# PRBonn/LiDiff

Hardware: NVIDIA B200
Metric: denoising_steps_per_sec_180k_pts_T50 (higher is better)
Workload: dtype fp16x3 split tensor-core MMA, fp32 accumulate (fp32 CUDA cores for the Cin=3 stem), fp64 DPM update

## Files before the change

### include/lidiff_b200.h

```cpp
#ifndef LIDIFF_B200_H_
#define LIDIFF_B200_H_

#include <stdint.h>
#include <stddef.h>

#ifdef __cplusplus
extern "C" {
#endif

#define LB2_OK            0
#define LB2_ERR_ARG      -1
#define LB2_ERR_CUDA     -2
#define LB2_ERR_UNSUP    -3

#define LB2_KEY_EMPTY 0xFFFFFFFFFFFFFFFFull

int         lb2_create(int device, void** handle);
void        lb2_destroy(void* handle);
const char* lb2_last_error(void* handle);
int         lb2_version(void);
int64_t     lb2_launch_count(void* handle);
#define LB2_OPT_TC_PAIR       0
#define LB2_OPT_TC_N256       1
#define LB2_OPT_TC_SMALL      2
#define LB2_OPT_TC_PERSISTENT 3
#define LB2_OPT_TC_FULL_LAG   4
#define LB2_OPT_TC_NSPLIT     5
#define LB2_OPT_COUNT         6
int         lb2_set_option(void* handle, int option, int value);
int         lb2_get_option(void* handle, int option);
int         lb2_read_status(void* handle, void* stream);

typedef struct {
    uint64_t* keys;
    int32_t*  vals;
    int32_t   cap_table;
} lb2_grid;

int lb2_quantize(void* h, void* stream, const float* x, int64_t n_elem, float resolution, int div_mode,
                 float* out_coord);

size_t lb2_unique_scratch_bytes(int64_t n_cap);
int lb2_unique_build(void* h, void* stream,
                     const float* in_f, const int32_t* in_i, const int32_t* d_nin, int32_t n_cap,
                     int32_t ts_floor, lb2_grid grid,
                     int32_t* out_coords, int32_t* inverse, int32_t* d_nout, void* scratch);

int lb2_voxel_mean(void* h, void* stream, const float* feats, const int32_t* inverse, int32_t n,
                   int32_t c, const int32_t* d_m, int32_t m_cap, float* out, int32_t* counts);

int lb2_kernel_map(void* h, void* stream, lb2_grid grid_in, const int32_t* out_coords,
                   const int32_t* d_nout, int32_t nout_cap, int32_t ks, int32_t step,
                   int32_t* nbr, int64_t nbr_stride, uint64_t* pair_count, uint32_t* row_mask);

int lb2_kernel_map_self(void* h, void* stream, lb2_grid grid, const int32_t* coords, const int32_t* d_n, int32_t n_cap,
                        int32_t step, int32_t* nbr, int64_t nbr_stride, uint64_t* pair_count, uint32_t* row_mask);

size_t lb2_row_order_scratch_bytes(int32_t n_cap);
int lb2_row_order(void* h, void* stream, const uint32_t* row_mask, const int32_t* d_n, int32_t n_cap,
                  int32_t kvol, int32_t* perm, void* scratch, const int32_t* coords, int32_t coord_shift);

int lb2_tile_order(void* h, void* stream, const uint32_t* row_mask, const int32_t* row_perm, const int32_t* d_n, int32_t n_cap,
                   int32_t* order128, int32_t* order256, void* scratch);

typedef struct {
    const float*   in1;
    const float*   in2;
    const float*   residual;
    float*         out;
    const float*   gate_table;
    const int32_t* gate_idx;
    float*         out_gated;
    const float*   pre_add;
    const void*    in1_h;
    const void*    in2_h;
    void*          out_h;
    void*          out_gated_h;
    const void*    residual_h;
} lb2_conv_io;

typedef struct {
    int32_t        c1, c2, cout, kvol;
    const float*   weight;
    const void*    weight_packed;
    const float*   scale;
    const float*   shift;
    int32_t        relu;
    const int32_t* nbr;
    int64_t        nbr_stride;
    const int32_t* d_mout;
    int32_t        mout_cap;
    const int32_t* row_perm;
    const uint32_t* row_mask;
    int32_t        npass;
    lb2_conv_io    io[2];
    const int32_t* tile_order128;
    const int32_t* tile_order256;
} lb2_conv_desc;

#define LB2_ALGO_AUTO  0
#define LB2_ALGO_FFMA  1
#define LB2_ALGO_TC    2
#define LB2_ALGO_TC_TILE 3
int lb2_spconv_forward(void* h, void* stream, const lb2_conv_desc* d, int algo);

typedef struct {
    int32_t        c1, c2, cout, kvol;
    const void*    weight_packed;
    const int32_t* pair_in;
    const int32_t* pair_out;
    const int32_t* koff;
    const int32_t* tile_off;
    int32_t        npass;
    const float*   in1[2];
    const float*   in2[2];
    const void*    in1_h[2];
    const void*    in2_h[2];
    float*         out[2];
    const int32_t* d_zero_rows;
    int32_t        zero_rows_cap;
} lb2_scatter_desc;
size_t lb2_pair_list_scratch_bytes(void);
int lb2_pair_list(void* h, void* stream, const int32_t* nbr, int64_t nbr_stride, const int32_t* d_nout,
                  int32_t nout_cap, int32_t kvol, int32_t skip_k, int32_t* pair_in, int32_t* pair_out,
                  int32_t* koff, int32_t* tile_off, void* scratch);
int lb2_spconv_scatter_supported(int32_t c1, int32_t c2, int32_t cout, int32_t kvol);
int lb2_spconv_scatter(void* h, void* stream, const lb2_scatter_desc* d);

size_t lb2_packed_weight_bytes(int32_t kvol, int32_t cin, int32_t cout);
int lb2_pack_weights(void* h, void* stream, const float* weight, int32_t kvol, int32_t cin, int32_t cout,
                     void* packed);

int lb2_nn_match(void* h, void* stream, const int32_t* q_coords, const int32_t* d_nq, int32_t nq_cap,
                 const int32_t* k_coords, const int32_t* d_nk, int32_t nk_cap, int32_t batch_scale,
                 int32_t* idx);

int lb2_nn_match_grid(void* h, void* stream, const int32_t* q_coords, const int32_t* d_nq, int32_t nq_cap,
                      const int32_t* k_coords, const int32_t* d_nk, int32_t nk_cap, lb2_grid key_grid,
                      int32_t key_stride, int32_t max_ring, int32_t* idx);

size_t lb2_nn_table_bytes(void);
int lb2_nn_table_build(void* h, void* stream, const int32_t* k_coords, const int32_t* d_nk, int32_t nk_cap, void* table);
int lb2_nn_match_table(void* h, void* stream, const int32_t* q_coords, const int32_t* d_nq, int32_t nq_cap,
                       const int32_t* k_coords, const int32_t* d_nk, int32_t nk_cap, const void* table,
                       int32_t key_stride, int32_t max_ring, int32_t* idx);

size_t lb2_nn_tree_bytes(int32_t nk_cap);
int lb2_nn_tree_build(void* h, void* stream, const int32_t* k_coords, const int32_t* d_nk, int32_t nk_cap, void* tree);
int lb2_nn_match_tree(void* h, void* stream, const int32_t* q_coords, const int32_t* d_nq, int32_t nq_cap,
                      const void* tree, int32_t nk_cap, const int32_t* k_coords, const int32_t* hint_of,
                      const int32_t* hint_idx, int32_t* idx);

int lb2_linear(void* h, void* stream, const float* x, int64_t ldx, const float* w, const float* b,
               const float* addend, int64_t ld_addend, int32_t m_cap, const int32_t* d_m,
               int32_t n_in, int32_t n_out, int32_t act, float* y, int64_t ldy,
               const float* prebias, int32_t pre_act);

int lb2_head_mlp(void* h, void* stream, const float* x, int64_t ldx, int64_t x_pass_stride, const float* w0, const float* b0,
                 const float* w1, const float* b1, int32_t m_cap, const int32_t* d_m, int32_t n_in, int32_t n_hid,
                 int32_t n_out, int32_t out_act, int32_t npass, float* y, int64_t ldy, int64_t y_pass_stride);

int lb2_gate_mul(void* h, void* stream, const float* x, const float* table, const int32_t* idx,
                 const int32_t* d_m, int32_t m_cap, int32_t c, float* out, void* out_h);

int lb2_gather_rows(void* h, void* stream, const float* src, const int32_t* idx, int32_t n, int32_t c,
                    float* out);

typedef struct {
    double c_sample, c_x0, c_noise, sigma_s, alpha_s, inv_r0;
    float  guidance_w, resolution;
    int32_t second_order, div_mode, f64_state;
} lb2_dpm_coef;
int lb2_guidance_dpm_step(void* h, void* stream, const float* eps_c, const float* eps_u,
                          const int32_t* inverse, const float* x_t, const double* x_init,
                          const float* noise, double* x0_state, int64_t n_points, lb2_dpm_coef coef,
                          float* eps_out, float* x_next, float* coord_next ,
                          const float* batch_col );

int lb2_farthest_point_sample(void* h, void* stream, const double* pts, int32_t n, int32_t n_samples,
                              int32_t* out_idx, double* dist_scratch);


size_t lb2_cloud_nn_scratch_bytes(int64_t nq, int64_t nr);
int lb2_cloud_nn_distance(void* h, void* stream, const double* query, int64_t nq, const double* ref, int64_t nr,
                          void* scratch, double* dist);

typedef struct {
    int64_t n_a, n_b;
    int64_t occ_a, occ_b, occ_ab;
    double  jsd_3d, jsd_bev;
} lb2_voxel_hist_result;
size_t lb2_voxel_hist_scratch_bytes(int64_t na, int64_t nb);
int lb2_voxel_hist_compare(void* h, void* stream, const double* a, int64_t na, const double* b, int64_t nb,
                           const double* edges, int32_t bins, void* scratch, lb2_voxel_hist_result* out);

int lb2_threshold_counts(void* h, void* stream, const double* d, int64_t n, const double* thr, int32_t nthr, int64_t* counts);

#ifdef __cplusplus
}
#endif
#endif
```

### lidiff_b200/_lib.py

```python
from __future__ import annotations

import ctypes as C
import os
import threading

import torch

_SO = os.path.join(os.path.dirname(os.path.abspath(__file__)), "_C", "liblidiff_b200.so")

ALGO_AUTO, ALGO_FFMA, ALGO_TC, ALGO_TC_TILE = 0, 1, 2, 3
OPT_TC_PAIR, OPT_TC_N256, OPT_TC_SMALL, OPT_TC_PERSISTENT, OPT_TC_FULL_LAG, OPT_TC_NSPLIT = range(6)


class Grid(C.Structure):
    _fields_ = [("keys", C.c_void_p), ("vals", C.c_void_p), ("cap_table", C.c_int32)]


class ConvIO(C.Structure):
    _fields_ = [("in1", C.c_void_p), ("in2", C.c_void_p), ("residual", C.c_void_p), ("out", C.c_void_p),
                ("gate_table", C.c_void_p), ("gate_idx", C.c_void_p), ("out_gated", C.c_void_p), ("pre_add", C.c_void_p),
                ("in1_h", C.c_void_p), ("in2_h", C.c_void_p), ("out_h", C.c_void_p), ("out_gated_h", C.c_void_p),
                ("residual_h", C.c_void_p)]


class ConvDesc(C.Structure):
    _fields_ = [("c1", C.c_int32), ("c2", C.c_int32), ("cout", C.c_int32), ("kvol", C.c_int32),
                ("weight", C.c_void_p), ("weight_packed", C.c_void_p),
                ("scale", C.c_void_p), ("shift", C.c_void_p), ("relu", C.c_int32),
                ("nbr", C.c_void_p), ("nbr_stride", C.c_int64),
                ("d_mout", C.c_void_p), ("mout_cap", C.c_int32), ("row_perm", C.c_void_p), ("row_mask", C.c_void_p),
                ("npass", C.c_int32),
                ("io", ConvIO * 2),
                ("tile_order128", C.c_void_p), ("tile_order256", C.c_void_p)]


class ScatterDesc(C.Structure):
    _fields_ = [("c1", C.c_int32), ("c2", C.c_int32), ("cout", C.c_int32), ("kvol", C.c_int32),
                ("weight_packed", C.c_void_p), ("pair_in", C.c_void_p), ("pair_out", C.c_void_p),
                ("koff", C.c_void_p), ("tile_off", C.c_void_p), ("npass", C.c_int32),
                ("in1", C.c_void_p * 2), ("in2", C.c_void_p * 2), ("in1_h", C.c_void_p * 2), ("in2_h", C.c_void_p * 2),
                ("out", C.c_void_p * 2),
                ("d_zero_rows", C.c_void_p), ("zero_rows_cap", C.c_int32)]


class VoxelHistResult(C.Structure):
    _fields_ = [("n_a", C.c_int64), ("n_b", C.c_int64), ("occ_a", C.c_int64), ("occ_b", C.c_int64), ("occ_ab", C.c_int64),
                ("jsd_3d", C.c_double), ("jsd_bev", C.c_double)]


class DpmCoef(C.Structure):
    _fields_ = [("c_sample", C.c_double), ("c_x0", C.c_double), ("c_noise", C.c_double),
                ("sigma_s", C.c_double), ("alpha_s", C.c_double), ("inv_r0", C.c_double),
                ("guidance_w", C.c_float), ("resolution", C.c_float),
                ("second_order", C.c_int32), ("div_mode", C.c_int32), ("f64_state", C.c_int32)]


EXPORTS = [
    "lb2_create", "lb2_destroy", "lb2_last_error", "lb2_version", "lb2_launch_count", "lb2_read_status",
    "lb2_set_option", "lb2_get_option", "lb2_tile_order",
    "lb2_quantize", "lb2_unique_scratch_bytes", "lb2_unique_build", "lb2_voxel_mean", "lb2_kernel_map",
    "lb2_spconv_forward", "lb2_packed_weight_bytes", "lb2_pack_weights", "lb2_nn_match", "lb2_linear",
    "lb2_gate_mul", "lb2_gather_rows", "lb2_head_mlp", "lb2_kernel_map_self", "lb2_guidance_dpm_step", "lb2_farthest_point_sample",
    "lb2_row_order", "lb2_row_order_scratch_bytes", "lb2_nn_match_grid",
    "lb2_nn_table_bytes", "lb2_nn_table_build", "lb2_nn_match_table",
    "lb2_nn_tree_bytes", "lb2_nn_tree_build", "lb2_nn_match_tree",
    "lb2_pair_list", "lb2_pair_list_scratch_bytes", "lb2_spconv_scatter", "lb2_spconv_scatter_supported",
    "lb2_cloud_nn_scratch_bytes", "lb2_cloud_nn_distance", "lb2_voxel_hist_scratch_bytes", "lb2_voxel_hist_compare",
    "lb2_threshold_counts",
]


def _ptr(t):
    if t is None:
        return None
    if isinstance(t, int):
        return t
    return t.data_ptr()


class Lib:

    def __init__(self, path: str = _SO):
        if not os.path.exists(path):
            raise RuntimeError(f"lidiff_b200: CUDA library not built ({path}); run `python -c 'import __graft_entry__ as g; g.build()'` "
                               "or lidiff_b200/csrc/build.sh — there is no CPU fallback")
        self.path = path
        self.dll = C.CDLL(path)
        d = self.dll
        d.lb2_create.argtypes = [C.c_int, C.POINTER(C.c_void_p)]
        d.lb2_destroy.argtypes = [C.c_void_p]
        d.lb2_destroy.restype = None
        d.lb2_last_error.argtypes = [C.c_void_p]
        d.lb2_last_error.restype = C.c_char_p
        d.lb2_launch_count.argtypes = [C.c_void_p]
        d.lb2_launch_count.restype = C.c_int64
        d.lb2_read_status.argtypes = [C.c_void_p, C.c_void_p]
        d.lb2_set_option.argtypes = [C.c_void_p, C.c_int, C.c_int]
        d.lb2_get_option.argtypes = [C.c_void_p, C.c_int]
        d.lb2_unique_scratch_bytes.argtypes = [C.c_int64]
        d.lb2_unique_scratch_bytes.restype = C.c_size_t
        d.lb2_packed_weight_bytes.argtypes = [C.c_int32] * 3
        d.lb2_packed_weight_bytes.restype = C.c_size_t
        vp, i32, i64, f32 = C.c_void_p, C.c_int32, C.c_int64, C.c_float
        d.lb2_quantize.argtypes = [vp, vp, vp, i64, f32, C.c_int, vp]
        d.lb2_unique_build.argtypes = [vp, vp, vp, vp, vp, i32, i32, Grid, vp, vp, vp, vp]
        d.lb2_voxel_mean.argtypes = [vp, vp, vp, vp, i32, i32, vp, i32, vp, vp]
        d.lb2_kernel_map.argtypes = [vp, vp, Grid, vp, vp, i32, i32, i32, vp, i64, vp, vp]
        d.lb2_kernel_map_self.argtypes = [vp, vp, Grid, vp, vp, i32, i32, vp, i64, vp, vp]
        d.lb2_row_order.argtypes = [vp, vp, vp, vp, i32, i32, vp, vp, vp, i32]
        d.lb2_tile_order.argtypes = [vp, vp, vp, vp, vp, i32, vp, vp, vp]
        d.lb2_row_order_scratch_bytes.restype = C.c_size_t
        d.lb2_row_order_scratch_bytes.argtypes = [i32]
        d.lb2_spconv_forward.argtypes = [vp, vp, C.POINTER(ConvDesc), C.c_int]
        d.lb2_pack_weights.argtypes = [vp, vp, vp, i32, i32, i32, vp]
        d.lb2_nn_match.argtypes = [vp, vp, vp, vp, i32, vp, vp, i32, i32, vp]
        d.lb2_pair_list.argtypes = [vp, vp, vp, i64, vp, i32, i32, i32, vp, vp, vp, vp, vp]
        d.lb2_pair_list_scratch_bytes.restype = C.c_size_t
        d.lb2_spconv_scatter.argtypes = [vp, vp, C.POINTER(ScatterDesc)]
        d.lb2_spconv_scatter_supported.argtypes = [i32, i32, i32, i32]
        d.lb2_nn_table_bytes.restype = C.c_size_t
        d.lb2_nn_tree_bytes.restype = C.c_size_t
        d.lb2_nn_tree_bytes.argtypes = [i32]
        d.lb2_nn_tree_build.argtypes = [vp, vp, vp, vp, i32, vp]
        d.lb2_nn_match_tree.argtypes = [vp, vp, vp, vp, i32, vp, i32, vp, vp, vp, vp]
        d.lb2_nn_table_build.argtypes = [vp, vp, vp, vp, i32, vp]
        d.lb2_nn_match_table.argtypes = [vp, vp, vp, vp, i32, vp, vp, i32, vp, i32, i32, vp]
        d.lb2_nn_match_grid.argtypes = [vp, vp, vp, vp, i32, vp, vp, i32, Grid, i32, i32, vp]
        d.lb2_linear.argtypes = [vp, vp, vp, i64, vp, vp, vp, i64, i32, vp, i32, i32, i32, vp, i64,
                                 vp, i32]
        d.lb2_gate_mul.argtypes = [vp, vp, vp, vp, vp, vp, i32, i32, vp, vp]
        d.lb2_gather_rows.argtypes = [vp, vp, vp, vp, i32, i32, vp]
        d.lb2_head_mlp.argtypes = [vp, vp, vp, i64, i64, vp, vp, vp, vp, i32, vp, i32, i32, i32, i32, i32, vp, i64, i64]
        d.lb2_guidance_dpm_step.argtypes = [vp, vp, vp, vp, vp, vp, vp, vp, vp, i64, DpmCoef, vp, vp, vp, vp]
        d.lb2_farthest_point_sample.argtypes = [vp, vp, vp, i32, i32, vp, vp]
        d.lb2_cloud_nn_scratch_bytes.argtypes = [i64, i64]
        d.lb2_cloud_nn_scratch_bytes.restype = C.c_size_t
        d.lb2_cloud_nn_distance.argtypes = [vp, vp, vp, i64, vp, i64, vp, vp]
        d.lb2_voxel_hist_scratch_bytes.argtypes = [i64, i64]
        d.lb2_voxel_hist_scratch_bytes.restype = C.c_size_t
        d.lb2_voxel_hist_compare.argtypes = [vp, vp, vp, i64, vp, i64, vp, i32, vp, vp]
        d.lb2_threshold_counts.argtypes = [vp, vp, vp, i64, vp, i32, vp]
        self._handles = {}
        self._lock = threading.Lock()

    def missing_symbols(self):
        return [s for s in EXPORTS if not hasattr(self.dll, s)]

    def handle(self, device) -> "Handle":
        dev = torch.device(device)
        if dev.type != "cuda":
            raise RuntimeError("lidiff_b200 runs on CUDA (B200, sm_100a) only; no CPU fallback")
        idx = dev.index if dev.index is not None else torch.cuda.current_device()
        with self._lock:
            if idx not in self._handles:
                hp = C.c_void_p()
                rc = self.dll.lb2_create(idx, C.byref(hp))
                if rc != 0:
                    raise RuntimeError(f"lb2_create(device={idx}) failed with {rc} (needs an sm_100 GPU)")
                self._handles[idx] = Handle(self, hp, idx)
            return self._handles[idx]


class Handle:
    def __init__(self, lib: Lib, hp, device_index: int):
        self.lib, self.dll, self.hp, self.device_index = lib, lib.dll, hp, device_index
        self.device = torch.device("cuda", device_index)

    def _stream(self):
        return torch.cuda.current_stream(self.device).cuda_stream

    def _check(self, rc, what):
        if rc != 0:
            msg = self.dll.lb2_last_error(self.hp)
            raise RuntimeError(f"{what} failed ({rc}): {msg.decode() if msg else ''}")

    def launch_count(self) -> int:
        return int(self.dll.lb2_launch_count(self.hp))

    def read_status(self) -> int:
        return int(self.dll.lb2_read_status(self.hp, self._stream()))

    def set_option(self, option: int, value: int):
        self._check(self.dll.lb2_set_option(self.hp, int(option), int(value)), "set_option")

    def get_option(self, option: int) -> int:
        return int(self.dll.lb2_get_option(self.hp, int(option)))

    def new_grid(self, n_cap: int):
        cap = 1 << max(4, (2 * n_cap - 1).bit_length())
        keys = torch.empty(cap, dtype=torch.int64, device=self.device)
        vals = torch.empty(2 * cap, dtype=torch.int32, device=self.device)
        return (keys, vals, cap)

    @staticmethod
    def _grid(g):
        return Grid(g[0].data_ptr(), g[1].data_ptr(), g[2])

    def unique_scratch(self, n_cap: int) -> torch.Tensor:
        nbytes = int(self.dll.lb2_unique_scratch_bytes(n_cap))
        return torch.empty(nbytes, dtype=torch.uint8, device=self.device)

    def quantize(self, x, resolution, div_mode, out):
        self._check(self.dll.lb2_quantize(self.hp, self._stream(), _ptr(x), x.numel(), float(resolution), int(div_mode), _ptr(out)), "lb2_quantize")

    def unique_build(self, in_f, in_i, d_nin, n_cap, ts_floor, grid, out_coords, inverse, d_nout, scratch):
        self._check(self.dll.lb2_unique_build(self.hp, self._stream(), _ptr(in_f), _ptr(in_i), _ptr(d_nin), int(n_cap), int(ts_floor),
                                              self._grid(grid), _ptr(out_coords), _ptr(inverse), _ptr(d_nout), _ptr(scratch)), "lb2_unique_build")

    def voxel_mean(self, feats, inverse, n, c, d_m, m_cap, out, counts):
        self._check(self.dll.lb2_voxel_mean(self.hp, self._stream(), _ptr(feats), _ptr(inverse), int(n), int(c), _ptr(d_m), int(m_cap),
                                            _ptr(out), _ptr(counts)), "lb2_voxel_mean")

    def kernel_map(self, grid_in, out_coords, d_nout, nout_cap, ks, step, nbr, nbr_stride, pair_count=None, row_mask=None):
        self._check(self.dll.lb2_kernel_map(self.hp, self._stream(), self._grid(grid_in), _ptr(out_coords), _ptr(d_nout), int(nout_cap),
                                            int(ks), int(step), _ptr(nbr), int(nbr_stride), _ptr(pair_count), _ptr(row_mask)), "lb2_kernel_map")

    def kernel_map_self(self, grid, coords, d_n, n_cap, step, nbr, nbr_stride, pair_count=None, row_mask=None):
        self._check(self.dll.lb2_kernel_map_self(self.hp, self._stream(), self._grid(grid), _ptr(coords), _ptr(d_n), int(n_cap), int(step),
                                                 _ptr(nbr), int(nbr_stride), _ptr(pair_count), _ptr(row_mask)), "lb2_kernel_map_self")

    def row_order_scratch_bytes(self, n_cap) -> int:
        return int(self.dll.lb2_row_order_scratch_bytes(int(n_cap)))

    def row_order(self, row_mask, d_n, n_cap, kvol, perm, scratch, coords=None, coord_shift=0):
        self._check(self.dll.lb2_row_order(self.hp, self._stream(), _ptr(row_mask), _ptr(d_n), int(n_cap), int(kvol), _ptr(perm), _ptr(scratch),
                                           _ptr(coords), int(coord_shift)), "lb2_row_order")

    def tile_order(self, row_mask, row_perm, d_n, n_cap, order128, order256, scratch):
        self._check(self.dll.lb2_tile_order(self.hp, self._stream(), _ptr(row_mask), _ptr(row_perm), _ptr(d_n), int(n_cap), _ptr(order128),
                                            _ptr(order256), _ptr(scratch)), "lb2_tile_order")

    def spconv(self, desc: ConvDesc, algo: int = ALGO_AUTO):
        self._check(self.dll.lb2_spconv_forward(self.hp, self._stream(), C.byref(desc), int(algo)), "lb2_spconv_forward")

    def pair_list(self, nbr, nbr_stride, d_nout, nout_cap, kvol, skip_k, pair_in, pair_out, koff, tile_off, scratch):
        self._check(self.dll.lb2_pair_list(self.hp, self._stream(), _ptr(nbr), int(nbr_stride), _ptr(d_nout), int(nout_cap), int(kvol), int(skip_k),
                                           _ptr(pair_in), _ptr(pair_out), _ptr(koff), _ptr(tile_off), _ptr(scratch)), "lb2_pair_list")

    def scatter_supported(self, c1, c2, cout, kvol) -> bool:
        return bool(self.dll.lb2_spconv_scatter_supported(int(c1), int(c2), int(cout), int(kvol)))

    def spconv_scatter(self, desc: "ScatterDesc"):
        self._check(self.dll.lb2_spconv_scatter(self.hp, self._stream(), C.byref(desc)), "lb2_spconv_scatter")

    def packed_weight_bytes(self, kvol, cin, cout) -> int:
        return int(self.dll.lb2_packed_weight_bytes(kvol, cin, cout))

    def pack_weights(self, w: torch.Tensor):
        kvol, cin, cout = w.shape
        nbytes = self.packed_weight_bytes(kvol, cin, cout)
        if nbytes == 0:
            return None
        out = torch.empty(nbytes, dtype=torch.uint8, device=self.device)
        self._check(self.dll.lb2_pack_weights(self.hp, self._stream(), _ptr(w), kvol, cin, cout, _ptr(out)), "lb2_pack_weights")
        return out

    def nn_match(self, q, d_nq, nq_cap, k, d_nk, nk_cap, batch_scale, idx):
        self._check(self.dll.lb2_nn_match(self.hp, self._stream(), _ptr(q), _ptr(d_nq), int(nq_cap), _ptr(k), _ptr(d_nk), int(nk_cap),
                                          int(batch_scale), _ptr(idx)), "lb2_nn_match")

    def nn_match_grid(self, q, d_nq, nq_cap, k, d_nk, nk_cap, key_grid, key_stride, max_ring, idx):
        self._check(self.dll.lb2_nn_match_grid(self.hp, self._stream(), _ptr(q), _ptr(d_nq), int(nq_cap), _ptr(k), _ptr(d_nk), int(nk_cap),
                                               self._grid(key_grid), int(key_stride), int(max_ring), _ptr(idx)), "lb2_nn_match_grid")

    def nn_table(self, k, d_nk, nk_cap):
        t = torch.empty(int(self.dll.lb2_nn_table_bytes()), dtype=torch.uint8, device=self.device)
        self._check(self.dll.lb2_nn_table_build(self.hp, self._stream(), _ptr(k), _ptr(d_nk), int(nk_cap), _ptr(t)), "lb2_nn_table_build")
        return t

    def nn_tree(self, k, d_nk, nk_cap, out=None):
        nbytes = int(self.dll.lb2_nn_tree_bytes(int(nk_cap)))
        t = out if (out is not None and out.numel() == nbytes) else torch.empty(nbytes, dtype=torch.uint8, device=self.device)
        self._check(self.dll.lb2_nn_tree_build(self.hp, self._stream(), _ptr(k), _ptr(d_nk), int(nk_cap), _ptr(t)), "lb2_nn_tree_build")
        return t

    def nn_match_tree(self, q, d_nq, nq_cap, tree, nk_cap, idx, k=None, hint_of=None, hint_idx=None):
        self._check(self.dll.lb2_nn_match_tree(self.hp, self._stream(), _ptr(q), _ptr(d_nq), int(nq_cap), _ptr(tree), int(nk_cap),
                                               _ptr(k), _ptr(hint_of), _ptr(hint_idx), _ptr(idx)), "lb2_nn_match_tree")

    def nn_match_table(self, q, d_nq, nq_cap, k, d_nk, nk_cap, table, key_stride, max_ring, idx):
        self._check(self.dll.lb2_nn_match_table(self.hp, self._stream(), _ptr(q), _ptr(d_nq), int(nq_cap), _ptr(k), _ptr(d_nk), int(nk_cap),
                                                _ptr(table), int(key_stride), int(max_ring), _ptr(idx)), "lb2_nn_match_table")

    def linear(self, x, ldx, w, b, addend, ld_add, m_cap, d_m, n_in, n_out, act, y, ldy, prebias=None, pre_act=0):
        self._check(self.dll.lb2_linear(self.hp, self._stream(), _ptr(x), int(ldx), _ptr(w), _ptr(b), _ptr(addend), int(ld_add), int(m_cap),
                                        _ptr(d_m), int(n_in), int(n_out), int(act), _ptr(y), int(ldy), _ptr(prebias), int(pre_act)), "lb2_linear")

    def head_mlp(self, x, ldx, x_pass_stride, w0, b0, w1, b1, m_cap, d_m, n_in, n_hid, n_out, out_act, npass, y, ldy, y_pass_stride):
        self._check(self.dll.lb2_head_mlp(self.hp, self._stream(), _ptr(x), int(ldx), int(x_pass_stride), _ptr(w0), _ptr(b0), _ptr(w1), _ptr(b1),
                                          int(m_cap), _ptr(d_m), int(n_in), int(n_hid), int(n_out), int(out_act), int(npass), _ptr(y), int(ldy),
                                          int(y_pass_stride)), "lb2_head_mlp")

    def gate_mul(self, x, table, idx, d_m, m_cap, c, out, out_h=None):
        self._check(self.dll.lb2_gate_mul(self.hp, self._stream(), _ptr(x), _ptr(table), _ptr(idx), _ptr(d_m), int(m_cap), int(c), _ptr(out),
                                          _ptr(out_h)), "lb2_gate_mul")

    def gather_rows(self, src, idx, n, c, out):
        self._check(self.dll.lb2_gather_rows(self.hp, self._stream(), _ptr(src), _ptr(idx), int(n), int(c), _ptr(out)), "lb2_gather_rows")

    def guidance_dpm_step(self, eps_c, eps_u, inverse, x_t, x_init, noise, x0_state, n_points, coef: DpmCoef,
                          eps_out, x_next, coord_next, batch_col=None):
        self._check(self.dll.lb2_guidance_dpm_step(self.hp, self._stream(), _ptr(eps_c), _ptr(eps_u), _ptr(inverse), _ptr(x_t), _ptr(x_init),
                                                   _ptr(noise), _ptr(x0_state), int(n_points), coef, _ptr(eps_out), _ptr(x_next),
                                                   _ptr(coord_next), _ptr(batch_col)), "lb2_guidance_dpm_step")

    def farthest_point_sample(self, pts, n, n_samples, out_idx, dist):
        self._check(self.dll.lb2_farthest_point_sample(self.hp, self._stream(), _ptr(pts), int(n), int(n_samples), _ptr(out_idx), _ptr(dist)),
                    "lb2_farthest_point_sample")

    def cloud_nn_scratch_bytes(self, nq, nr) -> int:
        return int(self.dll.lb2_cloud_nn_scratch_bytes(int(nq), int(nr)))

    def cloud_nn_distance(self, query, nq, ref, nr, scratch, dist):
        self._check(self.dll.lb2_cloud_nn_distance(self.hp, self._stream(), _ptr(query), int(nq), _ptr(ref), int(nr), _ptr(scratch),
                                                   _ptr(dist)), "lb2_cloud_nn_distance")

    def voxel_hist_scratch_bytes(self, na, nb) -> int:
        return int(self.dll.lb2_voxel_hist_scratch_bytes(int(na), int(nb)))

    def voxel_hist_compare(self, a, na, b, nb, edges, bins, scratch, out):
        self._check(self.dll.lb2_voxel_hist_compare(self.hp, self._stream(), _ptr(a), int(na), _ptr(b), int(nb), _ptr(edges), int(bins),
                                                    _ptr(scratch), _ptr(out)), "lb2_voxel_hist_compare")

    def threshold_counts(self, d, n, thr, nthr, counts):
        self._check(self.dll.lb2_threshold_counts(self.hp, self._stream(), _ptr(d), int(n), _ptr(thr), int(nthr), _ptr(counts)),
                    "lb2_threshold_counts")


_LIB = None


def get_lib() -> Lib:
    global _LIB
    if _LIB is None:
        _LIB = Lib()
    return _LIB


def get_handle(device) -> Handle:
    return get_lib().handle(device)
```

### lidiff_b200/csrc/coords.cu

```cuda
#include "common.cuh"
#include <stdlib.h>
#include <limits.h>
#include <algorithm>

extern "C" int lb2_version(void) { return 100; }

extern "C" int lb2_create(int device, void** handle) {
    if (!handle) return LB2_ERR_ARG;
    *handle = nullptr;
    int n = 0;
    if (cudaGetDeviceCount(&n) != cudaSuccess || n <= 0 || device < 0 || device >= n) return LB2_ERR_CUDA;
    if (cudaSetDevice(device) != cudaSuccess) return LB2_ERR_CUDA;
    cudaDeviceProp prop;
    if (cudaGetDeviceProperties(&prop, device) != cudaSuccess) return LB2_ERR_CUDA;
    if (prop.major != 10) return LB2_ERR_UNSUP;
    Lb2Handle* h = new Lb2Handle();
    h->device = device; h->num_sms = prop.multiProcessorCount; h->launches = 0; h->err[0] = 0; h->configured = 0;
    {
        auto env = [](const char* name, int dflt) { const char* e = getenv(name); return (e && e[0]) ? atoi(e) : dflt; };
        h->opt[LB2_OPT_TC_PAIR] = env("LB2_TC_PAIR", 2);
        h->opt[LB2_OPT_TC_N256] = env("LB2_TC_N256", 1);
        h->opt[LB2_OPT_TC_SMALL] = env("LB2_TC_SMALL", 1);
        h->opt[LB2_OPT_TC_PERSISTENT] = env("LB2_TC_PERSISTENT", 1);
        const char* lag = getenv("LB2_TC_LAG");
        h->opt[LB2_OPT_TC_FULL_LAG] = (lag && lag[0] == 'f') ? 1 : 0;
        h->opt[LB2_OPT_TC_NSPLIT] = env("LB2_TC_NSPLIT", 0);
    }
    if (cudaMalloc(&h->d_status, sizeof(int32_t)) != cudaSuccess) { delete h; return LB2_ERR_CUDA; }
    cudaMemset(h->d_status, 0, sizeof(int32_t));
    *handle = h;
    return LB2_OK;
}

extern "C" void lb2_destroy(void* handle) {
    Lb2Handle* h = (Lb2Handle*)handle;
    if (!h) return;
    cudaFree(h->d_status);
    delete h;
}

extern "C" int lb2_set_option(void* handle, int option, int value) {
    Lb2Handle* h = (Lb2Handle*)handle;
    LB2_REQUIRE(h, h && option >= 0 && option < LB2_OPT_COUNT, "set_option");
    h->opt[option] = value;
    return LB2_OK;
}

extern "C" int lb2_get_option(void* handle, int option) {
    Lb2Handle* h = (Lb2Handle*)handle;
    if (!h || option < 0 || option >= LB2_OPT_COUNT) return LB2_ERR_ARG;
    return h->opt[option];
}

extern "C" const char* lb2_last_error(void* handle) {
    return handle ? ((Lb2Handle*)handle)->err : "null handle";
}

extern "C" int64_t lb2_launch_count(void* handle) { return handle ? ((Lb2Handle*)handle)->launches : -1; }

extern "C" int lb2_read_status(void* handle, void* stream) {
    Lb2Handle* h = (Lb2Handle*)handle;
    if (!h) return LB2_ERR_ARG;
    int32_t v = 0;
    cudaStream_t s = (cudaStream_t)stream;
    if (cudaMemcpyAsync(&v, h->d_status, sizeof(v), cudaMemcpyDeviceToHost, s) != cudaSuccess) return LB2_ERR_CUDA;
    if (cudaMemsetAsync(h->d_status, 0, sizeof(v), s) != cudaSuccess) return LB2_ERR_CUDA;
    if (cudaStreamSynchronize(s) != cudaSuccess) return LB2_ERR_CUDA;
    return v;
}

__global__ void k_quantize(const float* __restrict__ x, long long n, float res, float inv_res, int div_mode,
                           float* __restrict__ out) {
    long long i = (long long)blockIdx.x * blockDim.x + threadIdx.x;
    if (i >= n) return;
    float v = x[i];
    float q = div_mode == 0 ? __fdiv_rn(v, res) : __fmul_rn(v, inv_res);
    out[i] = rintf(q);
}

extern "C" int lb2_quantize(void* handle, void* stream, const float* x, int64_t n_elem, float resolution,
                            int div_mode, float* out_coord) {
    Lb2Handle* h = (Lb2Handle*)handle;
    LB2_REQUIRE(h, h && x && out_coord && resolution > 0.f, "quantize");
    if (n_elem == 0) return LB2_OK;
    float inv = 1.0f / resolution;
    k_quantize<<<cdiv(n_elem, 256), 256, 0, (cudaStream_t)stream>>>(x, n_elem, resolution, inv, div_mode, out_coord);
    LB2_POST_LAUNCH(h, "k_quantize");
    return LB2_OK;
}

#define SCAN_THREADS 512
#define SCAN_ITEMS   4
#define SCAN_TILE    (SCAN_THREADS * SCAN_ITEMS)

struct UniqueScratch {
    int* slot_of;
    int* rank;
    int* bsum;
};

extern "C" size_t lb2_unique_scratch_bytes(int64_t n_cap) {
    size_t a = ((size_t)n_cap * sizeof(int) + 255) / 256 * 256;
    return 2 * a + SCAN_TILE * sizeof(int) + 256;
}

static UniqueScratch carve(void* scratch, int64_t n_cap) {
    size_t a = ((size_t)n_cap * sizeof(int) + 255) / 256 * 256;
    char* p = (char*)scratch;
    UniqueScratch s;
    s.slot_of = (int*)p; s.rank = (int*)(p + a); s.bsum = (int*)(p + 2 * a);
    return s;
}

__global__ void k_grid_clear(unsigned long long* keys, int* vals, int cap) {
    int i = blockIdx.x * blockDim.x + threadIdx.x;
    if (i < cap) { keys[i] = LB2_KEY_EMPTY; vals[i] = INT_MAX; vals[cap + i] = -1; }
}

__device__ __forceinline__ int4 load_row(const float* __restrict__ in_f, const int* __restrict__ in_i, int i, int ts) {
    int4 c;
    if (in_f) {
        float4 f = __ldg(reinterpret_cast<const float4*>(in_f) + i);
        c = make_int4((int)floorf(f.x), (int)floorf(f.y), (int)floorf(f.z), (int)floorf(f.w));
    } else {
        c = __ldg(reinterpret_cast<const int4*>(in_i) + i);
    }
    if (ts > 0) { c.y = floor_to_multiple(c.y, ts); c.z = floor_to_multiple(c.z, ts); c.w = floor_to_multiple(c.w, ts); }
    return c;
}

__global__ void k_grid_insert(const float* __restrict__ in_f, const int* __restrict__ in_i,
                              const int* __restrict__ d_n, int n_cap, int ts,
                              unsigned long long* keys, int* vals, unsigned mask,
                              int* __restrict__ slot_of, int* status) {
    int i = blockIdx.x * blockDim.x + threadIdx.x;
    int n = d_n ? min(*d_n, n_cap) : n_cap;
    if (i >= n) return;
    int4 c = load_row(in_f, in_i, i, ts);
    unsigned long long key;
    if (!lb2_pack_key(c.x, c.y, c.z, c.w, key)) atomicOr(status, 1);
    unsigned slot = lb2_hash(key) & mask;
    while (true) {
        unsigned long long prev = atomicCAS(keys + slot, (unsigned long long)LB2_KEY_EMPTY, key);
        if (prev == LB2_KEY_EMPTY || prev == key) break;
        slot = (slot + 1) & mask;
    }
    atomicMin(vals + slot, i);
    slot_of[i] = (int)slot;
}

__global__ void __launch_bounds__(SCAN_THREADS) k_scan_local(const int* __restrict__ slot_of, const int* __restrict__ vals,
                                                             const int* __restrict__ d_n, int n_cap,
                                                             int* __restrict__ rank, int* __restrict__ bsum) {
    __shared__ int warp_tot[SCAN_THREADS / 32];
    int n = d_n ? min(*d_n, n_cap) : n_cap;
    int base = blockIdx.x * SCAN_TILE + threadIdx.x * SCAN_ITEMS;
    int f[SCAN_ITEMS], tsum = 0;
#pragma unroll
    for (int j = 0; j < SCAN_ITEMS; ++j) {
        int i = base + j;
        f[j] = (i < n) ? (vals[slot_of[i]] == i) : 0;
        tsum += f[j];
    }
    int lane = threadIdx.x & 31, w = threadIdx.x >> 5;
    int incl = tsum;
#pragma unroll
    for (int d = 1; d < 32; d <<= 1) { int v = __shfl_up_sync(0xffffffffu, incl, d); if (lane >= d) incl += v; }
    if (lane == 31) warp_tot[w] = incl;
    __syncthreads();
    if (w == 0) {
        int v = (lane < SCAN_THREADS / 32) ? warp_tot[lane] : 0, inc2 = v;
#pragma unroll
        for (int d = 1; d < 32; d <<= 1) { int u = __shfl_up_sync(0xffffffffu, inc2, d); if (lane >= d) inc2 += u; }
        if (lane < SCAN_THREADS / 32) warp_tot[lane] = inc2 - v;
        if (lane == SCAN_THREADS / 32 - 1) bsum[blockIdx.x] = inc2;
    }
    __syncthreads();
    int excl = warp_tot[w] + incl - tsum;
#pragma unroll
    for (int j = 0; j < SCAN_ITEMS; ++j) {
        int i = base + j;
        if (i < n) rank[i] = f[j] ? excl : -1;
        excl += f[j];
    }
}

__global__ void __launch_bounds__(SCAN_THREADS) k_scan_bsum(int* __restrict__ bsum, int nblocks, int* __restrict__ d_total) {
    __shared__ int warp_tot[SCAN_THREADS / 32];
    int base = threadIdx.x * SCAN_ITEMS;
    int v[SCAN_ITEMS], tsum = 0;
#pragma unroll
    for (int j = 0; j < SCAN_ITEMS; ++j) { v[j] = (base + j < nblocks) ? bsum[base + j] : 0; tsum += v[j]; }
    int lane = threadIdx.x & 31, w = threadIdx.x >> 5;
    int incl = tsum;
#pragma unroll
    for (int d = 1; d < 32; d <<= 1) { int u = __shfl_up_sync(0xffffffffu, incl, d); if (lane >= d) incl += u; }
    if (lane == 31) warp_tot[w] = incl;
    __syncthreads();
    if (w == 0) {
        int x = (lane < SCAN_THREADS / 32) ? warp_tot[lane] : 0, inc2 = x;
#pragma unroll
        for (int d = 1; d < 32; d <<= 1) { int u = __shfl_up_sync(0xffffffffu, inc2, d); if (lane >= d) inc2 += u; }
        if (lane < SCAN_THREADS / 32) warp_tot[lane] = inc2 - x;
        if (lane == SCAN_THREADS / 32 - 1) *d_total = inc2;
    }
    __syncthreads();
    int excl = warp_tot[w] + incl - tsum;
#pragma unroll
    for (int j = 0; j < SCAN_ITEMS; ++j) { if (base + j < nblocks) bsum[base + j] = excl; excl += v[j]; }
}

__global__ void k_unique_emit(const float* __restrict__ in_f, const int* __restrict__ in_i,
                              const int* __restrict__ d_n, int n_cap, int ts,
                              const int* __restrict__ slot_of, const int* __restrict__ rank,
                              const int* __restrict__ bsum, int* __restrict__ vals, int cap,
                              int4* __restrict__ out_coords) {
    int i = blockIdx.x * blockDim.x + threadIdx.x;
    int n = d_n ? min(*d_n, n_cap) : n_cap;
    if (i >= n) return;
    int r = rank[i];
    if (r < 0) return;
    r += bsum[i / SCAN_TILE];
    vals[cap + slot_of[i]] = r;
    out_coords[r] = load_row(in_f, in_i, i, ts);
}

__global__ void k_unique_inverse(const int* __restrict__ d_n, int n_cap, const int* __restrict__ slot_of,
                                 const int* __restrict__ vals, int cap, int* __restrict__ inverse) {
    int i = blockIdx.x * blockDim.x + threadIdx.x;
    int n = d_n ? min(*d_n, n_cap) : n_cap;
    if (i < n) inverse[i] = vals[cap + slot_of[i]];
}

extern "C" int lb2_unique_build(void* handle, void* stream, const float* in_f, const int32_t* in_i,
                                const int32_t* d_nin, int32_t n_cap, int32_t ts_floor, lb2_grid grid,
                                int32_t* out_coords, int32_t* inverse, int32_t* d_nout, void* scratch) {
    Lb2Handle* h = (Lb2Handle*)handle;
    LB2_REQUIRE(h, h != nullptr, "handle");
    LB2_REQUIRE(h, (in_f != nullptr) != (in_i != nullptr), "exactly one of in_f / in_i");
    LB2_REQUIRE(h, grid.keys && grid.vals && out_coords && d_nout && scratch, "null buffer");
    LB2_REQUIRE(h, n_cap > 0 && n_cap <= SCAN_TILE * SCAN_TILE, "n_cap out of range (max 4M rows)");
    LB2_REQUIRE(h, grid.cap_table >= 2 && (grid.cap_table & (grid.cap_table - 1)) == 0, "cap_table must be a power of two");
    LB2_REQUIRE(h, (long long)grid.cap_table >= 2LL * n_cap, "cap_table must be >= 2 * n_cap");
    LB2_REQUIRE(h, ts_floor >= 0, "ts_floor");
    cudaStream_t s = (cudaStream_t)stream;
    UniqueScratch sc = carve(scratch, n_cap);
    unsigned long long* keys = (unsigned long long*)grid.keys;
    int cap = grid.cap_table;
    unsigned mask = (unsigned)cap - 1u;
    int nblk = (int)cdiv(n_cap, SCAN_TILE);

    k_grid_clear<<<cdiv(cap, 256), 256, 0, s>>>(keys, grid.vals, cap);
    LB2_POST_LAUNCH(h, "k_grid_clear");
    k_grid_insert<<<cdiv(n_cap, 256), 256, 0, s>>>(in_f, in_i, d_nin, n_cap, ts_floor, keys, grid.vals, mask, sc.slot_of, h->d_status);
    LB2_POST_LAUNCH(h, "k_grid_insert");
    k_scan_local<<<nblk, SCAN_THREADS, 0, s>>>(sc.slot_of, grid.vals, d_nin, n_cap, sc.rank, sc.bsum);
    LB2_POST_LAUNCH(h, "k_scan_local");
    k_scan_bsum<<<1, SCAN_THREADS, 0, s>>>(sc.bsum, nblk, d_nout);
    LB2_POST_LAUNCH(h, "k_scan_bsum");
    k_unique_emit<<<cdiv(n_cap, 256), 256, 0, s>>>(in_f, in_i, d_nin, n_cap, ts_floor, sc.slot_of, sc.rank, sc.bsum,
                                                  grid.vals, cap, (int4*)out_coords);
    LB2_POST_LAUNCH(h, "k_unique_emit");
    if (inverse) {
        k_unique_inverse<<<cdiv(n_cap, 256), 256, 0, s>>>(d_nin, n_cap, sc.slot_of, grid.vals, cap, inverse);
        LB2_POST_LAUNCH(h, "k_unique_inverse");
    }
    return LB2_OK;
}

__global__ void k_voxel_accum(const float* __restrict__ feats, const int* __restrict__ inverse, int n, int c,
                              float* __restrict__ out, int* __restrict__ counts) {
    long long t = (long long)blockIdx.x * blockDim.x + threadIdx.x;
    if (t >= (long long)n * c) return;
    int i = (int)(t / c), j = (int)(t % c);
    int r = inverse[i];
    atomicAdd(out + (long long)r * c + j, feats[t]);
    if (j == 0) atomicAdd(counts + r, 1);
}

__global__ void k_voxel_div(float* __restrict__ out, const int* __restrict__ counts, const int* __restrict__ d_m,
                            int m_cap, int c) {
    long long t = (long long)blockIdx.x * blockDim.x + threadIdx.x;
    int m = d_m ? min(*d_m, m_cap) : m_cap;
    if (t >= (long long)m * c) return;
    out[t] = __fdiv_rn(out[t], (float)counts[t / c]);
}

extern "C" int lb2_voxel_mean(void* handle, void* stream, const float* feats, const int32_t* inverse, int32_t n,
                              int32_t c, const int32_t* d_m, int32_t m_cap, float* out, int32_t* counts) {
    Lb2Handle* h = (Lb2Handle*)handle;
    LB2_REQUIRE(h, h && feats && inverse && out && counts && n > 0 && c > 0 && m_cap > 0, "voxel_mean");
    cudaStream_t s = (cudaStream_t)stream;
    if (cudaMemsetAsync(out, 0, (size_t)m_cap * c * sizeof(float), s) != cudaSuccess ||
        cudaMemsetAsync(counts, 0, (size_t)m_cap * sizeof(int), s) != cudaSuccess)
        return lb2_fail(h, LB2_ERR_CUDA, "voxel_mean memset%s", "");
    k_voxel_accum<<<cdiv((long long)n * c, 256), 256, 0, s>>>(feats, inverse, n, c, out, counts);
    LB2_POST_LAUNCH(h, "k_voxel_accum");
    k_voxel_div<<<cdiv((long long)m_cap * c, 256), 256, 0, s>>>(out, counts, d_m, m_cap, c);
    LB2_POST_LAUNCH(h, "k_voxel_div");
    return LB2_OK;
}

template <int KS>
__global__ void __launch_bounds__(128) k_kernel_map(const unsigned long long* __restrict__ keys, const int* __restrict__ rows, unsigned mask,
                                                    const int4* __restrict__ out_coords, const int* __restrict__ d_n, int n_cap,
                                                    int step, int* __restrict__ nbr, long long nbr_stride,
                                                    unsigned long long* __restrict__ pair_count, unsigned* __restrict__ row_mask) {
    constexpr int KV = KS * KS * KS;
    const int o = blockIdx.x * blockDim.x + threadIdx.x;
    const int n = d_n ? min(*d_n, n_cap) : n_cap;
    unsigned found = 0;
    if (o < n) {
        const int4 c = __ldg(out_coords + o);
        constexpr int cen = (KS & 1) ? KS / 2 : 0;
        int res[KV];
        unsigned long long key[KV], got[KV];
        unsigned slot[KV];
#pragma unroll
        for (int k = 0; k < KV; ++k) {
            const int kx = k % KS, ky = (k / KS) % KS, kz = k / (KS * KS);
            const int x = c.y + (kx - cen) * step, y = c.z + (ky - cen) * step, z = c.w + (kz - cen) * step;
            const bool ok = lb2_pack_key(c.x, x, y, z, key[k]);
            slot[k] = ok ? (lb2_hash(key[k]) & mask) : 0u;
            got[k] = ok ? __ldg(keys + slot[k]) : LB2_KEY_EMPTY;
            if (!ok) key[k] = ~LB2_KEY_EMPTY;
        }
#pragma unroll
        for (int k = 0; k < KV; ++k) {
            if (got[k] == key[k]) res[k] = __ldg(rows + slot[k]);
            else if (got[k] == LB2_KEY_EMPTY) res[k] = -1;
            else {
                unsigned sl = (slot[k] + 1) & mask;
                res[k] = -1;
                while (true) {
                    const unsigned long long kk = __ldg(keys + sl);
                    if (kk == key[k]) { res[k] = __ldg(rows + sl); break; }
                    if (kk == LB2_KEY_EMPTY) break;
                    sl = (sl + 1) & mask;
                }
            }
        }
#pragma unroll
        for (int k = 0; k < KV; ++k) {
            nbr[(long long)k * nbr_stride + o] = res[k];
            if (res[k] >= 0) found |= 1u << k;
        }
    } else if (o < n_cap) {
#pragma unroll
        for (int k = 0; k < KV; ++k) nbr[(long long)k * nbr_stride + o] = -1;
    }
    if (row_mask && o < n_cap) row_mask[o] = found;
    if (pair_count) {
        int cnt = __popc(found);
#pragma unroll
        for (int d = 16; d > 0; d >>= 1) cnt += __shfl_xor_sync(0xffffffffu, cnt, d);
        if ((threadIdx.x & 31) == 0 && cnt) atomicAdd(pair_count, (unsigned long long)cnt);
    }
}

extern "C" int lb2_kernel_map(void* handle, void* stream, lb2_grid grid_in, const int32_t* out_coords,
                              const int32_t* d_nout, int32_t nout_cap, int32_t ks, int32_t step,
                              int32_t* nbr, int64_t nbr_stride, uint64_t* pair_count, uint32_t* row_mask) {
    Lb2Handle* h = (Lb2Handle*)handle;
    LB2_REQUIRE(h, h && grid_in.keys && grid_in.vals && out_coords && nbr, "kernel_map null");
    LB2_REQUIRE(h, ks >= 1 && ks <= 3 && step != 0 && nout_cap > 0 && nbr_stride >= nout_cap, "kernel_map args");
    const unsigned long long* gk = (const unsigned long long*)grid_in.keys;
    const int* gr = grid_in.vals + grid_in.cap_table;
    const unsigned gm = (unsigned)grid_in.cap_table - 1u;
    const unsigned blocks = cdiv(nout_cap, 128);
    cudaStream_t s = (cudaStream_t)stream;
    if (ks == 3) k_kernel_map<3><<<blocks, 128, 0, s>>>(gk, gr, gm, (const int4*)out_coords, d_nout, nout_cap, step, nbr, nbr_stride, (unsigned long long*)pair_count, row_mask);
    else if (ks == 2) k_kernel_map<2><<<blocks, 128, 0, s>>>(gk, gr, gm, (const int4*)out_coords, d_nout, nout_cap, step, nbr, nbr_stride, (unsigned long long*)pair_count, row_mask);
    else k_kernel_map<1><<<blocks, 128, 0, s>>>(gk, gr, gm, (const int4*)out_coords, d_nout, nout_cap, step, nbr, nbr_stride, (unsigned long long*)pair_count, row_mask);
    LB2_POST_LAUNCH(h, "k_kernel_map");
    return LB2_OK;
}

__global__ void __launch_bounds__(128) k_kernel_map_self(const unsigned long long* __restrict__ keys, const int* __restrict__ rows, unsigned mask,
                                                         const int4* __restrict__ coords, const int* __restrict__ d_n, int n_cap, int step,
                                                         int* __restrict__ nbr, long long nbr_stride,
                                                         unsigned long long* __restrict__ pair_count, unsigned* __restrict__ row_mask) {
    constexpr int HALF = 13;
    const int o = blockIdx.x * blockDim.x + threadIdx.x;
    const int n = d_n ? min(*d_n, n_cap) : n_cap;
    unsigned found = 0;
    if (o < n) {
        const int4 c = __ldg(coords + o);
        int res[HALF];
        unsigned long long key[HALF], got[HALF];
        unsigned slot[HALF];
#pragma unroll
        for (int k = 0; k < HALF; ++k) {
            const int kx = k % 3, ky = (k / 3) % 3, kz = k / 9;
            const int x = c.y + (kx - 1) * step, y = c.z + (ky - 1) * step, z = c.w + (kz - 1) * step;
            const bool ok = lb2_pack_key(c.x, x, y, z, key[k]);
            slot[k] = ok ? (lb2_hash(key[k]) & mask) : 0u;
            got[k] = ok ? __ldg(keys + slot[k]) : LB2_KEY_EMPTY;
            if (!ok) key[k] = ~LB2_KEY_EMPTY;
        }
#pragma unroll
        for (int k = 0; k < HALF; ++k) {
            if (got[k] == key[k]) res[k] = __ldg(rows + slot[k]);
            else if (got[k] == LB2_KEY_EMPTY) res[k] = -1;
            else {
                unsigned sl = (slot[k] + 1) & mask;
                res[k] = -1;
                while (true) {
                    const unsigned long long kk = __ldg(keys + sl);
                    if (kk == key[k]) { res[k] = __ldg(rows + sl); break; }
                    if (kk == LB2_KEY_EMPTY) break;
                    sl = (sl + 1) & mask;
                }
            }
        }
#pragma unroll
        for (int k = 0; k < HALF; ++k) {
            nbr[(long long)k * nbr_stride + o] = res[k];
            if (res[k] >= 0) {
                found |= 1u << k;
                nbr[(long long)(26 - k) * nbr_stride + res[k]] = o;
                if (row_mask) atomicOr(row_mask + res[k], 1u << (26 - k));
            }
        }
        nbr[(long long)HALF * nbr_stride + o] = o;
        if (row_mask) atomicOr(row_mask + o, found | (1u << HALF));
    } else if (o < n_cap) {
#pragma unroll
        for (int k = 0; k <= HALF; ++k) nbr[(long long)k * nbr_stride + o] = -1;
    }
    if (pair_count) {
        int cnt = (o < n) ? 2 * __popc(found) + 1 : 0;
#pragma unroll
        for (int d = 16; d > 0; d >>= 1) cnt += __shfl_xor_sync(0xffffffffu, cnt, d);
        if ((threadIdx.x & 31) == 0 && cnt) atomicAdd(pair_count, (unsigned long long)cnt);
    }
}

extern "C" int lb2_kernel_map_self(void* handle, void* stream, lb2_grid grid, const int32_t* coords, const int32_t* d_n, int32_t n_cap,
                                   int32_t step, int32_t* nbr, int64_t nbr_stride, uint64_t* pair_count, uint32_t* row_mask) {
    Lb2Handle* h = (Lb2Handle*)handle;
    LB2_REQUIRE(h, h && grid.keys && grid.vals && coords && nbr, "kernel_map_self null");
    LB2_REQUIRE(h, step > 0 && n_cap > 0 && nbr_stride >= n_cap, "kernel_map_self args");
    cudaStream_t s = (cudaStream_t)stream;
    cudaError_t e = cudaMemsetAsync(nbr + 14 * nbr_stride, 0xff, (size_t)13 * nbr_stride * sizeof(int32_t), s);
    if (e == cudaSuccess && row_mask) e = cudaMemsetAsync(row_mask, 0, (size_t)n_cap * sizeof(uint32_t), s);
    if (e != cudaSuccess) return lb2_fail(h, LB2_ERR_CUDA, "kernel_map_self memset: %s", cudaGetErrorString(e));
    k_kernel_map_self<<<cdiv(n_cap, 128), 128, 0, s>>>((const unsigned long long*)grid.keys, grid.vals + grid.cap_table, (unsigned)grid.cap_table - 1u,
                                                       (const int4*)coords, d_n, n_cap, step, nbr, nbr_stride, (unsigned long long*)pair_count, row_mask);
    LB2_POST_LAUNCH(h, "k_kernel_map_self");
    return LB2_OK;
}

#define RO_BINS 256
#define RS_BITS 9
#define RS_BINS (1 << RS_BITS)
#define RS_CHUNK 2048
#define RS_WARPS 8

__device__ __forceinline__ unsigned ro_key27(unsigned mask) {
    const unsigned extras = mask & ~(1u << 13);
    const unsigned k26 = ((mask >> 14) << 13) | (mask & 0x1fffu);
    return ((__popc(extras) >= 2) ? (1u << 26) : 0u) | k26;
}

__device__ __forceinline__ unsigned ro_part9(unsigned v) {
    v &= 0x1ffu;
    v = (v | (v << 16)) & 0x030000ffu;
    v = (v | (v << 8)) & 0x0300f00fu;
    v = (v | (v << 4)) & 0x030c30c3u;
    v = (v | (v << 2)) & 0x09249249u;
    return v;
}
__device__ __forceinline__ unsigned ro_morton(const int4 c, int shift) {
    return ro_part9((unsigned)(c.y >> shift)) | (ro_part9((unsigned)(c.z >> shift)) << 1) | (ro_part9((unsigned)(c.w >> shift)) << 2);
}

struct RsSrc {
    const unsigned* keys;
    const unsigned* mask;
    const int4* coords;
    const int* vals;
    const unsigned long long* keys64;
    int mode, coord_shift, key_shift;
};
__device__ __forceinline__ unsigned rs_key(const RsSrc& s, int i) {
    switch (s.mode) {
        case 0: return s.keys[i];
        case 1: return ro_key27(s.mask[i]);
        case 2: return ro_morton(s.coords[i], s.coord_shift);
        case 4: return (unsigned)(s.keys64[s.vals ? s.vals[i] : i] >> s.key_shift);
        default: return ro_key27(s.mask[s.vals[i]]);
    }
}

__global__ void __launch_bounds__(256) k_rs_hist(const RsSrc src, const int* __restrict__ d_n, int n_cap, int shift, int* __restrict__ hist,
                                                 int* __restrict__ total) {
    __shared__ int sh[RS_BINS];
    for (int i = threadIdx.x; i < RS_BINS; i += blockDim.x) sh[i] = 0;
    __syncthreads();
    const int n = d_n ? min(*d_n, n_cap) : n_cap;
    const int lo = blockIdx.x * RS_CHUNK, hi = min(lo + RS_CHUNK, n);
    for (int i = lo + threadIdx.x; i < hi; i += blockDim.x) atomicAdd(&sh[(rs_key(src, i) >> shift) & (RS_BINS - 1)], 1);
    __syncthreads();
    for (int i = threadIdx.x; i < RS_BINS; i += blockDim.x) {
        hist[blockIdx.x * RS_BINS + i] = sh[i];
        if (sh[i]) atomicAdd(total + i, sh[i]);
    }
}

__global__ void __launch_bounds__(32 * RS_WARPS) k_rs_scatter(const RsSrc src, const int* __restrict__ d_n, int n_cap,
                                                              int shift, const int* __restrict__ hist, const int* __restrict__ total,
                                                              unsigned* __restrict__ keys_out, int* __restrict__ vals_out) {
    const int* __restrict__ vals_in = src.vals;
    __shared__ int cnt[RS_WARPS][RS_BINS];
    __shared__ int first[RS_BINS];
    const int warp = threadIdx.x >> 5, lane = threadIdx.x & 31;
    for (int i = threadIdx.x; i < RS_WARPS * RS_BINS; i += blockDim.x) (&cnt[0][0])[i] = 0;
    {
        const int t = threadIdx.x;
        const int t0 = total[2 * t], t1 = total[2 * t + 1];
        first[t] = t0 + t1;
        __syncthreads();
        for (int d = 1; d < RS_BINS / 2; d <<= 1) {
            const int u = (t >= d) ? first[t - d] : 0;
            __syncthreads();
            first[t] += u;
            __syncthreads();
        }
        const int excl = first[t] - (t0 + t1);
        int p0 = 0, p1 = 0;
#pragma unroll 8
        for (int b = 0; b < (int)blockIdx.x; ++b) {
            const int2 v = *reinterpret_cast<const int2*>(hist + b * RS_BINS + 2 * t);
            p0 += v.x; p1 += v.y;
        }
        __syncthreads();
        first[2 * t] = excl + p0;
        first[2 * t + 1] = excl + t0 + p1;
    }
    __syncthreads();
    const int n = d_n ? min(*d_n, n_cap) : n_cap;
    const int w0 = blockIdx.x * RS_CHUNK + warp * (RS_CHUNK / RS_WARPS);
    for (int g = 0; g < RS_CHUNK / RS_WARPS / 32; ++g) {
        const int i = w0 + g * 32 + lane;
        if (i < n) atomicAdd(&cnt[warp][(rs_key(src, i) >> shift) & (RS_BINS - 1)], 1);
    }
    __syncthreads();
    for (int bin = threadIdx.x; bin < RS_BINS; bin += blockDim.x) {
        int run = first[bin];
        for (int w = 0; w < RS_WARPS; ++w) { const int v = cnt[w][bin]; cnt[w][bin] = run; run += v; }
    }
    __syncthreads();
    for (int g = 0; g < RS_CHUNK / RS_WARPS / 32; ++g) {
        const int i = w0 + g * 32 + lane;
        const bool ok = i < n;
        const unsigned active = __ballot_sync(0xffffffffu, ok);
        if (ok) {
            const unsigned key = rs_key(src, i);
            const int val = vals_in ? vals_in[i] : i;
            const int d = (key >> shift) & (RS_BINS - 1);
            const unsigned peers = __match_any_sync(active, d);
            const int rank = __popc(peers & ((1u << lane) - 1u));
            const int pos = cnt[warp][d] + rank;
            __syncwarp(active);
            if (rank == 0) cnt[warp][d] += __popc(peers);
            __syncwarp(active);
            if (keys_out) keys_out[pos] = key;
            vals_out[pos] = val;
        }
    }
}

__device__ __forceinline__ int ro_bucket(unsigned mask, int kvol) {
    (void)kvol;
    return (int)(mask & 0xffu);
}

__global__ void k_ro_hist(const unsigned* __restrict__ mask, const int* __restrict__ d_n, int n_cap, int kvol, int* __restrict__ bins) {
    __shared__ int sh[RO_BINS];
    for (int i = threadIdx.x; i < RO_BINS; i += blockDim.x) sh[i] = 0;
    __syncthreads();
    const int n = d_n ? min(*d_n, n_cap) : n_cap;
    for (int i = blockIdx.x * blockDim.x + threadIdx.x; i < n; i += gridDim.x * blockDim.x) atomicAdd(&sh[ro_bucket(mask[i], kvol)], 1);
    __syncthreads();
    for (int i = threadIdx.x; i < RO_BINS; i += blockDim.x) if (sh[i]) atomicAdd(&bins[i], sh[i]);
}

__global__ void k_ro_scan(int* __restrict__ bins) {
    __shared__ int sh[RO_BINS];
    const int t = threadIdx.x;
    const int v = bins[t];
    sh[t] = v;
    __syncthreads();
    for (int d = 1; d < RO_BINS; d <<= 1) {
        const int u = (t >= d) ? sh[t - d] : 0;
        __syncthreads();
        sh[t] += u;
        __syncthreads();
    }
    bins[t] = sh[t] - v;
}

__global__ void k_ro_scatter(const unsigned* __restrict__ mask, const int* __restrict__ d_n, int n_cap, int kvol,
                             int* __restrict__ cursor, int* __restrict__ perm) {
    __shared__ int cnt[RO_BINS];
    __shared__ int base[RO_BINS];
    for (int i = threadIdx.x; i < RO_BINS; i += blockDim.x) cnt[i] = 0;
    __syncthreads();
    const int n = d_n ? min(*d_n, n_cap) : n_cap;
    const int i = blockIdx.x * blockDim.x + threadIdx.x;
    int b = -1, local = 0;
    if (i < n) { b = ro_bucket(mask[i], kvol); local = atomicAdd(&cnt[b], 1); }
    __syncthreads();
    for (int j = threadIdx.x; j < RO_BINS; j += blockDim.x) if (cnt[j]) base[j] = atomicAdd(&cursor[j], cnt[j]);
    __syncthreads();
    if (i < n) perm[base[b] + local] = i;
}

static int rs_blocks(int n_cap) { return cdiv(n_cap, RS_CHUNK); }

extern "C" size_t lb2_row_order_scratch_bytes(int32_t n_cap) {
    return ((size_t)RS_BINS * (rs_blocks(n_cap) + 6) + 3 * (size_t)n_cap) * sizeof(int);
}

extern "C" int lb2_row_order(void* handle, void* stream, const uint32_t* row_mask, const int32_t* d_n, int32_t n_cap,
                             int32_t kvol, int32_t* perm, void* scratch, const int32_t* coords, int32_t coord_shift) {
    Lb2Handle* h = (Lb2Handle*)handle;
    LB2_REQUIRE(h, h && row_mask && perm && scratch && n_cap > 0 && (kvol == 27 || (kvol >= 1 && kvol <= 8)), "row_order");
    LB2_REQUIRE(h, coord_shift >= 0 && coord_shift < 24, "row_order coord_shift");
    cudaStream_t s = (cudaStream_t)stream;
    if (kvol == 27) {
        const int nblk = rs_blocks(n_cap);
        int* hist = (int*)scratch;
        int* total = hist + (size_t)RS_BINS * nblk;
        unsigned* keys_a = (unsigned*)(total + 6 * RS_BINS);
        if (cudaMemsetAsync(total, 0, 6 * RS_BINS * sizeof(int), s) != cudaSuccess) return lb2_fail(h, LB2_ERR_CUDA, "row_order memset%s", "");
        unsigned* keys_b = keys_a + n_cap;
        int* vals_a = (int*)(keys_b + n_cap);
        const int npass = coords ? 6 : 3;
        for (int pass = 0; pass < npass; ++pass) {
            const int mp = coords ? pass - 3 : pass;
            const bool to_perm = coords ? (pass & 1) : !(pass & 1);
            RsSrc src;
            src.mask = row_mask; src.coords = (const int4*)coords; src.coord_shift = coord_shift;
            src.keys = (pass & 1) ? keys_a : keys_b;
            src.vals = (pass == 0) ? nullptr : (to_perm ? vals_a : perm);
            src.mode = (pass == 0) ? (coords ? 2 : 1) : ((coords && pass == 3) ? 3 : 0);
            unsigned* kout = (pass == npass - 1 || (coords && pass == 2)) ? nullptr : ((pass & 1) ? keys_b : keys_a);
            int* vout = to_perm ? perm : vals_a;
            const int shift = (mp >= 0 ? mp : pass) * RS_BITS;
            k_rs_hist<<<nblk, 256, 0, s>>>(src, d_n, n_cap, shift, hist, total + pass * RS_BINS);
            LB2_POST_LAUNCH(h, "k_rs_hist");
            k_rs_scatter<<<nblk, 32 * RS_WARPS, 0, s>>>(src, d_n, n_cap, shift, hist, total + pass * RS_BINS, kout, vout);
            LB2_POST_LAUNCH(h, "k_rs_scatter");
        }
        return LB2_OK;
    }
    int* bins = (int*)scratch;
    if (cudaMemsetAsync(bins, 0, RO_BINS * sizeof(int), s) != cudaSuccess) return lb2_fail(h, LB2_ERR_CUDA, "row_order memset%s", "");
    k_ro_hist<<<std::min<unsigned>(cdiv(n_cap, 256), 1024u), 256, 0, s>>>(row_mask, d_n, n_cap, kvol, bins);
    LB2_POST_LAUNCH(h, "k_ro_hist");
    k_ro_scan<<<1, RO_BINS, 0, s>>>(bins);
    LB2_POST_LAUNCH(h, "k_ro_scan");
    k_ro_scatter<<<cdiv(n_cap, 256), 256, 0, s>>>(row_mask, d_n, n_cap, kvol, bins, perm);
    LB2_POST_LAUNCH(h, "k_ro_scatter");
    return LB2_OK;
}

size_t lb2_sort_keys64_scratch_bytes(int n) {
    return ((size_t)RS_BINS * (rs_blocks(n) + 8) + (size_t)n) * sizeof(int);
}

int lb2_sort_keys64(Lb2Handle* h, cudaStream_t s, const unsigned long long* keys, int n, int key_bits, int* perm, void* scratch) {
    if (n <= 0) return LB2_OK;
    const int nblk = rs_blocks(n);
    const int npass = key_bits <= RS_BITS ? 1 : (key_bits + RS_BITS - 1) / RS_BITS;
    int* hist = (int*)scratch;
    int* total = hist + (size_t)RS_BINS * nblk;
    int* tmp = total + 8 * RS_BINS;
    if (cudaMemsetAsync(total, 0, (size_t)npass * RS_BINS * sizeof(int), s) != cudaSuccess) return lb2_fail(h, LB2_ERR_CUDA, "sort_keys64 memset%s", "");
    const int* vin = nullptr;
    for (int pass = 0; pass < npass; ++pass) {
        int* vout = ((npass - 1 - pass) & 1) ? tmp : perm;
        RsSrc src;
        src.keys = nullptr; src.mask = nullptr; src.coords = nullptr; src.vals = vin; src.keys64 = keys;
        src.mode = 4; src.coord_shift = 0; src.key_shift = pass * RS_BITS;
        k_rs_hist<<<nblk, 256, 0, s>>>(src, nullptr, n, 0, hist, total + pass * RS_BINS);
        LB2_POST_LAUNCH(h, "k_rs_hist");
        k_rs_scatter<<<nblk, 32 * RS_WARPS, 0, s>>>(src, nullptr, n, 0, hist, total + pass * RS_BINS, nullptr, vout);
        LB2_POST_LAUNCH(h, "k_rs_scatter");
        vin = vout;
    }
    return LB2_OK;
}

#define NT_LEAF 4
#define NT_HDR 16

static int nt_nleaf(int nk_cap) { int n = 1; while (n * NT_LEAF < nk_cap) n <<= 1; return n; }
static size_t nt_sort_ints(int nk_cap) { return (size_t)RS_BINS * (rs_blocks(nk_cap) + 3) + 4 * (size_t)nk_cap; }

extern "C" size_t lb2_nn_tree_bytes(int32_t nk_cap) {
    return (NT_HDR + (size_t)2 * nt_nleaf(nk_cap) * 8 + 5 * (size_t)nt_nleaf(nk_cap) * NT_LEAF + nt_sort_ints(nk_cap)) * sizeof(int) + 64;
}

__global__ void k_nt_init(int* __restrict__ hdr, int nleaf, int nk_cap) {
    if (threadIdx.x < 3) { hdr[threadIdx.x] = 0x7fffffff; hdr[3 + threadIdx.x] = (int)0x80000000; }
    if (threadIdx.x == 0) { hdr[6] = 0; hdr[7] = nleaf; hdr[8] = nk_cap; }
}

__global__ void k_nt_minmax(const int4* __restrict__ keys, const int* __restrict__ d_nk, int nk_cap, int* __restrict__ hdr) {
    const int nk = d_nk ? min(*d_nk, nk_cap) : nk_cap;
    int lo[3] = {0x7fffffff, 0x7fffffff, 0x7fffffff}, hi[3] = {(int)0x80000000, (int)0x80000000, (int)0x80000000};
    for (int i = blockIdx.x * blockDim.x + threadIdx.x; i < nk; i += gridDim.x * blockDim.x) {
        const int4 c = __ldg(keys + i);
        lo[0] = min(lo[0], c.y); lo[1] = min(lo[1], c.z); lo[2] = min(lo[2], c.w);
        hi[0] = max(hi[0], c.y); hi[1] = max(hi[1], c.z); hi[2] = max(hi[2], c.w);
    }
#pragma unroll
    for (int a = 0; a < 3; ++a) {
#pragma unroll
        for (int o = 16; o > 0; o >>= 1) { lo[a] = min(lo[a], __shfl_xor_sync(0xffffffffu, lo[a], o)); hi[a] = max(hi[a], __shfl_xor_sync(0xffffffffu, hi[a], o)); }
        if ((threadIdx.x & 31) == 0) { atomicMin(hdr + a, lo[a]); atomicMax(hdr + 3 + a, hi[a]); }
    }
}

__device__ __forceinline__ unsigned nt_spread9(unsigned v) {
    unsigned r = 0;
#pragma unroll
    for (int b = 0; b < 9; ++b) r |= ((v >> b) & 1u) << (3 * b);
    return r;
}

__global__ void k_nt_morton(const int4* __restrict__ keys, const int* __restrict__ d_nk, int nk_cap, const int* __restrict__ hdr,
                            unsigned* __restrict__ codes) {
    const int nk = d_nk ? min(*d_nk, nk_cap) : nk_cap;
    const int i = blockIdx.x * blockDim.x + threadIdx.x;
    if (i >= nk) return;
    long long ext = 0;
#pragma unroll
    for (int a = 0; a < 3; ++a) ext = max(ext, (long long)hdr[3 + a] - (long long)hdr[a]);
    int shift = 0;
    while ((ext >> shift) > 511) ++shift;
    const int4 c = __ldg(keys + i);
    const unsigned x = (unsigned)(((long long)c.y - hdr[0]) >> shift), y = (unsigned)(((long long)c.z - hdr[1]) >> shift),
                   z = (unsigned)(((long long)c.w - hdr[2]) >> shift);
    codes[i] = nt_spread9(x) | (nt_spread9(y) << 1) | (nt_spread9(z) << 2);
}

__global__ void k_nt_gather(const int4* __restrict__ keys, const int* __restrict__ d_nk, int nk_cap, const int* __restrict__ order,
                            int slots, int4* __restrict__ skeys, int* __restrict__ sbatch) {
    const int nk = d_nk ? min(*d_nk, nk_cap) : nk_cap;
    const int i = blockIdx.x * blockDim.x + threadIdx.x;
    if (i >= slots) return;
    if (i >= nk) { skeys[i] = make_int4(0, 0, 0, -1); sbatch[i] = 0; return; }
    const int j = order[i];
    const int4 c = __ldg(keys + j);
    skeys[i] = make_int4(c.y, c.z, c.w, j);
    sbatch[i] = c.x;
}

__global__ void k_nt_leaves(const int4* __restrict__ skeys, const int* __restrict__ sbatch, const int* __restrict__ d_nk, int nk_cap,
                            int nleaf, int* __restrict__ nodes) {
    const int nk = d_nk ? min(*d_nk, nk_cap) : nk_cap;
    const int l = blockIdx.x * blockDim.x + threadIdx.x;
    if (l >= nleaf) return;
    int v[8] = {0x7fffffff, 0x7fffffff, 0x7fffffff, (int)0x80000000, (int)0x80000000, (int)0x80000000, 0x7fffffff, (int)0x80000000};
    for (int t = 0; t < NT_LEAF; ++t) {
        const int i = l * NT_LEAF + t;
        if (i >= nk) break;
        const int4 c = skeys[i];
        const int b = sbatch[i];
        v[0] = min(v[0], c.x); v[1] = min(v[1], c.y); v[2] = min(v[2], c.z);
        v[3] = max(v[3], c.x); v[4] = max(v[4], c.y); v[5] = max(v[5], c.z);
        v[6] = min(v[6], b); v[7] = max(v[7], b);
    }
    int* n = nodes + (size_t)(nleaf + l) * 8;
#pragma unroll
    for (int a = 0; a < 8; ++a) n[a] = v[a];
}

__global__ void __launch_bounds__(1024) k_nt_internal(int nleaf, int* __restrict__ nodes) {
    for (int first = nleaf >> 1; first >= 1; first >>= 1) {
        for (int i = first + threadIdx.x; i < 2 * first; i += blockDim.x) {
            const int* a = nodes + (size_t)(2 * i) * 8;
            const int* b = a + 8;
            int* n = nodes + (size_t)i * 8;
#pragma unroll
            for (int c = 0; c < 3; ++c) { n[c] = min(a[c], b[c]); n[3 + c] = max(a[3 + c], b[3 + c]); }
            n[6] = min(a[6], b[6]); n[7] = max(a[7], b[7]);
        }
        __syncthreads();
    }
}

extern "C" int lb2_nn_tree_build(void* handle, void* stream, const int32_t* k_coords, const int32_t* d_nk, int32_t nk_cap, void* tree) {
    Lb2Handle* h = (Lb2Handle*)handle;
    LB2_REQUIRE(h, h && k_coords && tree && nk_cap > 0, "nn_tree_build");
    cudaStream_t s = (cudaStream_t)stream;
    const int nleaf = nt_nleaf(nk_cap);
    int* hdr = (int*)tree;
    int* nodes = hdr + NT_HDR;
    int4* skeys = (int4*)(nodes + (size_t)2 * nleaf * 8);
    const int slots = nleaf * NT_LEAF;
    int* sbatch = (int*)(skeys + slots);
    int* hist = sbatch + slots;
    const int nblk = rs_blocks(nk_cap);
    int* total = hist + (size_t)RS_BINS * nblk;
    unsigned* codes = (unsigned*)(total + 3 * RS_BINS);
    unsigned* keys_b = codes + nk_cap;
    int* vals_a = (int*)(keys_b + nk_cap);
    int* vals_b = vals_a + nk_cap;
    k_nt_init<<<1, 32, 0, s>>>(hdr, nleaf, nk_cap);
    LB2_POST_LAUNCH(h, "k_nt_init");
    k_nt_minmax<<<std::min<unsigned>(cdiv(nk_cap, 256), 256u), 256, 0, s>>>((const int4*)k_coords, d_nk, nk_cap, hdr);
    LB2_POST_LAUNCH(h, "k_nt_minmax");
    k_nt_morton<<<cdiv(nk_cap, 256), 256, 0, s>>>((const int4*)k_coords, d_nk, nk_cap, hdr, codes);
    LB2_POST_LAUNCH(h, "k_nt_morton");
    if (cudaMemsetAsync(total, 0, 3 * RS_BINS * sizeof(int), s) != cudaSuccess) return lb2_fail(h, LB2_ERR_CUDA, "nn_tree memset%s", "");
    const unsigned* kin[3] = {codes, keys_b, codes};
    const int* vin[3] = {nullptr, vals_a, vals_b};
    unsigned* kout[3] = {keys_b, codes, nullptr};
    int* vout[3] = {vals_a, vals_b, vals_a};
    for (int pass = 0; pass < 3; ++pass) {
        RsSrc src;
        src.keys = kin[pass]; src.mask = nullptr; src.coords = nullptr; src.vals = vin[pass]; src.mode = 0; src.coord_shift = 0;
        k_rs_hist<<<nblk, 256, 0, s>>>(src, d_nk, nk_cap, pass * RS_BITS, hist, total + pass * RS_BINS);
        LB2_POST_LAUNCH(h, "k_rs_hist");
        k_rs_scatter<<<nblk, 32 * RS_WARPS, 0, s>>>(src, d_nk, nk_cap, pass * RS_BITS, hist, total + pass * RS_BINS, kout[pass], vout[pass]);
        LB2_POST_LAUNCH(h, "k_rs_scatter");
    }
    k_nt_gather<<<cdiv(slots, 256), 256, 0, s>>>((const int4*)k_coords, d_nk, nk_cap, vals_a, slots, skeys, sbatch);
    LB2_POST_LAUNCH(h, "k_nt_gather");
    k_nt_leaves<<<cdiv(nleaf, 256), 256, 0, s>>>(skeys, sbatch, d_nk, nk_cap, nleaf, nodes);
    LB2_POST_LAUNCH(h, "k_nt_leaves");
    k_nt_internal<<<1, 1024, 0, s>>>(nleaf, nodes);
    LB2_POST_LAUNCH(h, "k_nt_internal");
    return LB2_OK;
}

__global__ void __launch_bounds__(256) k_tile_masks(const unsigned* __restrict__ mask, const int* __restrict__ perm, const int* __restrict__ d_n,
                                                    int n_cap, unsigned* __restrict__ tmask) {
    const int n = d_n ? min(*d_n, n_cap) : n_cap;
    const int nt = (n + 127) >> 7;
    const int warp = (blockIdx.x * blockDim.x + threadIdx.x) >> 5, lane = threadIdx.x & 31;
    if (warp >= nt) return;
    unsigned m = 0;
#pragma unroll
    for (int q = 0; q < 4; ++q) {
        const int slot = warp * 128 + q * 32 + lane;
        if (slot < n) m |= __ldg(mask + (perm ? __ldg(perm + slot) : slot));
    }
    m = __reduce_or_sync(0xffffffffu, m);
    if (lane == 0) tmask[warp] = m;
}

__global__ void __launch_bounds__(1024) k_tile_sort(const unsigned* __restrict__ tmask, const int* __restrict__ d_n, int n_cap,
                                                    int* __restrict__ order128, int* __restrict__ order256) {
    __shared__ int bins[2][33];
    const int n = d_n ? min(*d_n, n_cap) : n_cap;
    const int nt128 = (n + 127) >> 7, nt256 = (n + 255) >> 8;
    const int cap128 = (n_cap + 127) >> 7, cap256 = (n_cap + 255) >> 8;
    if (threadIdx.x < 66) (&bins[0][0])[threadIdx.x] = 0;
    __syncthreads();
    for (int t = threadIdx.x; t < nt128; t += blockDim.x) atomicAdd(&bins[0][32 - __popc(tmask[t])], 1);
    for (int u = threadIdx.x; u < nt256; u += blockDim.x) {
        const unsigned m = tmask[2 * u] | ((2 * u + 1 < nt128) ? tmask[2 * u + 1] : 0u);
        atomicAdd(&bins[1][32 - __popc(m)], 1);
    }
    __syncthreads();
    if (threadIdx.x < 2) {
        int run = 0;
        for (int b = 0; b < 33; ++b) { const int v = bins[threadIdx.x][b]; bins[threadIdx.x][b] = run; run += v; }
    }
    __syncthreads();
    for (int t = threadIdx.x; t < nt128; t += blockDim.x) order128[atomicAdd(&bins[0][32 - __popc(tmask[t])], 1)] = t;
    for (int u = threadIdx.x; u < nt256; u += blockDim.x) {
        const unsigned m = tmask[2 * u] | ((2 * u + 1 < nt128) ? tmask[2 * u + 1] : 0u);
        order256[atomicAdd(&bins[1][32 - __popc(m)], 1)] = u;
    }
    for (int t = nt128 + threadIdx.x; t < cap128; t += blockDim.x) order128[t] = -1;
    for (int u = nt256 + threadIdx.x; u < cap256; u += blockDim.x) order256[u] = -1;
}

extern "C" int lb2_tile_order(void* handle, void* stream, const uint32_t* row_mask, const int32_t* row_perm, const int32_t* d_n, int32_t n_cap,
                              int32_t* order128, int32_t* order256, void* scratch) {
    Lb2Handle* h = (Lb2Handle*)handle;
    LB2_REQUIRE(h, h && row_mask && order128 && order256 && scratch && n_cap > 0, "tile_order");
    cudaStream_t s = (cudaStream_t)stream;
    const int cap128 = cdiv(n_cap, 128);
    k_tile_masks<<<cdiv(cap128, 8), 256, 0, s>>>(row_mask, row_perm, d_n, n_cap, (unsigned*)scratch);
    LB2_POST_LAUNCH(h, "k_tile_masks");
    k_tile_sort<<<1, 1024, 0, s>>>((const unsigned*)scratch, d_n, n_cap, order128, order256);
    LB2_POST_LAUNCH(h, "k_tile_sort");
    return LB2_OK;
}
```

### lidiff_b200/csrc/spconv_ffma.cu

```cuda
#include "common.cuh"
#include "tc_common.cuh"

#define FF_BM 64
#define FF_BN 64
#define FF_BK 16
#define FF_THREADS 256

struct FfmaParams {
    int c1, c2, cout, kvol;
    const float* W;
    const float* scale;
    const float* shift;
    int relu;
    const int* nbr;
    long long nbr_stride;
    const int* d_mout;
    int mout_cap;
    const int* row_perm;
    lb2_conv_io io[2];
};

__global__ void __launch_bounds__(FF_THREADS) k_spconv_ffma(const FfmaParams p) {
    __shared__ int   idx_s[FF_BM];
    __shared__ int   row_s[FF_BM];
    __shared__ float As[FF_BK][FF_BM + 4];
    __shared__ float Bs[FF_BK][FF_BN + 4];

    const int M = p.d_mout ? min(*p.d_mout, p.mout_cap) : p.mout_cap;
    const int m0 = blockIdx.x * FF_BM;
    if (m0 >= M) return;
    const int n0 = blockIdx.y * FF_BN;
    const lb2_conv_io io = p.io[blockIdx.z];
    const int ctot = p.c1 + p.c2;
    const int t = threadIdx.x;
    const int ty = t >> 4, tx = t & 15;
    const int ar = t >> 2, ac = (t & 3) * 4;
    const int bk = t >> 4, bn = (t & 15) * 4;
    const bool vecA1 = (p.c1 % 4 == 0), vecA2 = (p.c2 % 4 == 0);
    const bool vecB = (p.cout % 4 == 0);

    float acc[4][4];
#pragma unroll
    for (int i = 0; i < 4; ++i)
#pragma unroll
        for (int j = 0; j < 4; ++j) acc[i][j] = 0.f;

    if (t < FF_BM) row_s[t] = (m0 + t < M) ? (p.row_perm ? __ldg(p.row_perm + m0 + t) : m0 + t) : -1;
    __syncthreads();
    for (int k = 0; k < p.kvol; ++k) {
        int my = -1;
        if (t < FF_BM) {
            const int row = row_s[t];
            if (row >= 0) my = p.nbr ? __ldg(p.nbr + (long long)k * p.nbr_stride + row) : row;
            idx_s[t] = my;
        }
        if (!__syncthreads_or(my >= 0)) continue;
        const float* Wk = p.W + (long long)k * ctot * p.cout;

        for (int c0 = 0; c0 < ctot; c0 += FF_BK) {
            {
                const int src = idx_s[ar];
                const int c = c0 + ac;
                float v[4] = {0.f, 0.f, 0.f, 0.f};
                if (src >= 0) {
                    if (c < p.c1) {
                        const float* rp = io.in1 + (long long)src * p.c1;
                        if (vecA1 && c + 3 < p.c1) {
                            float4 f = __ldg(reinterpret_cast<const float4*>(rp + c));
                            v[0] = f.x; v[1] = f.y; v[2] = f.z; v[3] = f.w;
                        } else {
#pragma unroll
                            for (int j = 0; j < 4; ++j) {
                                int cj = c + j;
                                if (cj < p.c1) v[j] = __ldg(rp + cj);
                                else if (cj < ctot) v[j] = __ldg(io.in2 + (long long)src * p.c2 + (cj - p.c1));
                            }
                        }
                    } else if (c < ctot) {
                        const float* rp = io.in2 + (long long)src * p.c2;
                        const int cc = c - p.c1;
                        if (vecA2 && cc + 3 < p.c2) {
                            float4 f = __ldg(reinterpret_cast<const float4*>(rp + cc));
                            v[0] = f.x; v[1] = f.y; v[2] = f.z; v[3] = f.w;
                        } else {
#pragma unroll
                            for (int j = 0; j < 4; ++j) if (cc + j < p.c2) v[j] = __ldg(rp + cc + j);
                        }
                    }
                }
#pragma unroll
                for (int j = 0; j < 4; ++j) As[ac + j][ar] = v[j];
            }
            {
                const int c = c0 + bk, n = n0 + bn;
                float v[4] = {0.f, 0.f, 0.f, 0.f};
                if (c < ctot) {
                    const float* wp = Wk + (long long)c * p.cout + n;
                    if (vecB && n + 3 < p.cout) {
                        float4 f = __ldg(reinterpret_cast<const float4*>(wp));
                        v[0] = f.x; v[1] = f.y; v[2] = f.z; v[3] = f.w;
                    } else {
#pragma unroll
                        for (int j = 0; j < 4; ++j) if (n + j < p.cout) v[j] = __ldg(wp + j);
                    }
                }
                *reinterpret_cast<float4*>(&Bs[bk][bn]) = make_float4(v[0], v[1], v[2], v[3]);
            }
            __syncthreads();
#pragma unroll
            for (int kk = 0; kk < FF_BK; ++kk) {
                const float4 a = *reinterpret_cast<const float4*>(&As[kk][ty * 4]);
                const float4 b = *reinterpret_cast<const float4*>(&Bs[kk][tx * 4]);
                const float av[4] = {a.x, a.y, a.z, a.w}, bv[4] = {b.x, b.y, b.z, b.w};
#pragma unroll
                for (int i = 0; i < 4; ++i)
#pragma unroll
                    for (int j = 0; j < 4; ++j) acc[i][j] = fmaf(av[i], bv[j], acc[i][j]);
            }
            __syncthreads();
        }
    }

#pragma unroll
    for (int i = 0; i < 4; ++i) {
        const int row = row_s[ty * 4 + i];
        if (row < 0) continue;
        const long long ro = (long long)row * p.cout;
        const float* gate_row = nullptr;
        if (io.gate_table) gate_row = io.gate_table + (long long)(io.gate_idx ? __ldg(io.gate_idx + row) : 0) * p.cout;
        float yv[4] = {0.f, 0.f, 0.f, 0.f}, gv[4] = {0.f, 0.f, 0.f, 0.f};
#pragma unroll
        for (int j = 0; j < 4; ++j) {
            const int col = n0 + tx * 4 + j;
            if (col >= p.cout) continue;
            float y = acc[i][j];
            if (io.pre_add) y += __ldg(io.pre_add + ro + col);
            if (p.scale) y = fmaf(y, __ldg(p.scale + col), __ldg(p.shift + col));
            if (io.residual) y += __ldg(io.residual + ro + col);
            else if (io.residual_h) {
                const __half* rp = reinterpret_cast<const __half*>(io.residual_h) + 2 * ro + col;
                y += __half2float(__ldg(rp)) + __half2float(__ldg(rp + p.cout));
            }
            if (p.relu) y = fmaxf(y, 0.f);
            yv[j] = y;
            gv[j] = gate_row ? y * __ldg(gate_row + col) : y;
            if (io.out) io.out[ro + col] = y;
            if (io.out_gated) io.out_gated[ro + col] = gv[j];
        }
        if (n0 + tx * 4 + 3 < p.cout) {
            if (io.out_h) tc::store_split4(io.out_h, row, p.cout, n0 + tx * 4, yv);
            if (io.out_gated_h) tc::store_split4(io.out_gated_h, row, p.cout, n0 + tx * 4, gv);
        }
    }
}

int lb2_spconv_ffma_launch(Lb2Handle* h, cudaStream_t s, const lb2_conv_desc* d) {
    FfmaParams p;
    p.c1 = d->c1; p.c2 = d->c2; p.cout = d->cout; p.kvol = d->kvol;
    p.W = d->weight; p.scale = d->scale; p.shift = d->shift; p.relu = d->relu;
    p.nbr = d->nbr; p.nbr_stride = d->nbr_stride; p.d_mout = d->d_mout; p.mout_cap = d->mout_cap; p.row_perm = d->row_perm;
    p.io[0] = d->io[0]; p.io[1] = d->io[d->npass > 1 ? 1 : 0];
    dim3 grid(cdiv(d->mout_cap, FF_BM), cdiv(d->cout, FF_BN), d->npass);
    k_spconv_ffma<<<grid, FF_THREADS, 0, s>>>(p);
    LB2_POST_LAUNCH(h, "k_spconv_ffma");
    return LB2_OK;
}
```

### lidiff_b200/csrc/spconv_scatter.cu

```cuda
#include "common.cuh"
#include <algorithm>
#include "tc_common.cuh"

namespace sc {
using namespace tc;

constexpr int THREADS = 320;
constexpr int MAX_STAGES = 4;
constexpr int MAX_KVOL = 27;
constexpr int SLAB_PITCH = 36;
constexpr int SLAB_BYTES = BM * SLAB_PITCH * 4;

struct Params {
    int c1, c2, cout, kvol, nchunks, stages, npass;
    const unsigned char* wpacked;
    const int* pair_in;
    const int* pair_out;
    const int* koff;
    const int* tile_off;
    const float* in1[2];
    const float* in2[2];
    const void* in1_h[2];
    const void* in2_h[2];
    float* out[2];
    int acc_stride, tmem_cols;
};

__global__ void __launch_bounds__(THREADS, 1) k_spconv_scatter(const Params p) {
    extern __shared__ unsigned char smem_raw[];
    __shared__ int s_koff[MAX_KVOL + 1];
    __shared__ int s_toff[MAX_KVOL + 1];
    const int warp = threadIdx.x >> 5, lane = threadIdx.x & 31;
    const int ctot = p.c1 + p.c2;
    if (threadIdx.x <= p.kvol) { s_koff[threadIdx.x] = p.koff[threadIdx.x]; s_toff[threadIdx.x] = p.tile_off[threadIdx.x]; }

    const uint32_t raw = smem_u32(smem_raw);
    const uint32_t base = (raw + 1023u) & ~1023u;
    unsigned char* gen = smem_raw + (base - raw);
    const uint32_t b_tile = (uint32_t)p.cout * 128u;
    const uint32_t w_bytes = (uint32_t)p.nchunks * 2u * b_tile;
    const uint32_t a_stage = 2u * A_TILE;
    unsigned char* a_gen = gen + w_bytes;
    const uint32_t a_base = base + w_bytes;
    float* slab = reinterpret_cast<float*>(a_gen + (size_t)p.stages * a_stage);
    uint64_t* bars = reinterpret_cast<uint64_t*>(reinterpret_cast<unsigned char*>(slab) + SLAB_BYTES);
    uint32_t* misc = reinterpret_cast<uint32_t*>(bars + 2 * MAX_STAGES + 6);
    const uint32_t bar0 = smem_u32(bars);
    auto full_a = [&](int s) { return bar0 + 8u * s; };
    auto empty_a = [&](int s) { return bar0 + 8u * (MAX_STAGES + s); };
    const uint32_t w_full = bar0 + 8u * (2 * MAX_STAGES), w_empty = bar0 + 8u * (2 * MAX_STAGES + 1);
    auto acc_full = [&](int b) { return bar0 + 8u * (2 * MAX_STAGES + 2 + b); };
    auto acc_empty = [&](int b) { return bar0 + 8u * (2 * MAX_STAGES + 4 + b); };

    if (threadIdx.x == 0) {
        for (int s = 0; s < p.stages; ++s) { mbar_init(full_a(s), 128); mbar_init(empty_a(s), 1); }
        mbar_init(w_full, 1); mbar_init(w_empty, 1);
        for (int b = 0; b < 2; ++b) { mbar_init(acc_full(b), 1); mbar_init(acc_empty(b), 128); }
        asm volatile("fence.mbarrier_init.release.cluster;" ::: "memory");
    }
    if (warp == 4) {
        asm volatile("tcgen05.alloc.cta_group::1.sync.aligned.shared::cta.b32 [%0], %1;" ::"r"(smem_u32(&misc[0])), "r"((uint32_t)p.tmem_cols) : "memory");
        asm volatile("tcgen05.relinquish_alloc_permit.cta_group::1.sync.aligned;" ::: "memory");
    }
    tc_fence_before();
    __syncthreads();
    tc_fence_after();
    const uint32_t tmem_d = misc[0];

    const int tiles_per_pass = s_toff[p.kvol];
    const long long total = (long long)tiles_per_pass * p.npass;
    const int t_begin = (int)(total * blockIdx.x / gridDim.x), t_end = (int)(total * (blockIdx.x + 1) / gridDim.x);

    auto decode = [&](int T, int& pass, int& k, int& pbase, int& cnt) {
        pass = T / tiles_per_pass;
        const int t = T - pass * tiles_per_pass;
        k = 0;
        while (k + 1 < p.kvol && s_toff[k + 1] <= t) ++k;
        pbase = s_koff[k] + (t - s_toff[k]) * BM;
        cnt = min(BM, s_koff[k + 1] - pbase);
    };

    if (warp < 4) {
        const int sub = threadIdx.x & 7, rbase = threadIdx.x >> 3;
        const int D = p.stages - 1;
        int it = 0, arrived = 0;
        bool any_h = false;
        for (int T = t_begin; T < t_end; ++T) {
            int pass, k, pbase, cnt;
            decode(T, pass, k, pbase, cnt);
            const bool use_h = (p.in1_h[pass] != nullptr) && (p.c2 == 0 || p.in2_h[pass] != nullptr);
            any_h |= use_h;
            int src[8];
#pragma unroll
            for (int j = 0; j < 8; ++j) { const int r = rbase + 16 * j; src[j] = r < cnt ? __ldg(p.pair_in + pbase + r) : -1; }
            for (int c = 0; c < p.nchunks; ++c, ++it) {
                const int s = it % p.stages;
                mbar_wait(empty_a(s), ((it / p.stages) & 1) ^ 1);
                unsigned char* a_hi = a_gen + (size_t)s * a_stage;
                const uint32_t a_hi_u = a_base + (uint32_t)s * a_stage;
                const int ch = c * KC + sub * 8;
                if (ch < ctot) {
                    const bool first = ch < p.c1;
                    const int cw = first ? p.c1 : p.c2;
                    const int co = first ? ch : ch - p.c1;
                    if (use_h) produce_a_split(reinterpret_cast<const __half*>(first ? p.in1_h[pass] : p.in2_h[pass]), cw, co, src, a_hi_u, a_hi_u + A_TILE, rbase, sub);
                    else produce_a_f32(first ? p.in1[pass] : p.in2[pass], cw, co, src, a_hi, a_hi + A_TILE, rbase, sub);
                }
                cp_async_commit();
                if (it >= D) {
                    cp_async_wait_dyn(D);
                    fence_proxy_async();
                    mbar_arrive(full_a(arrived % p.stages));
                    ++arrived;
                }
            }
        }
        cp_async_wait<0>();
        fence_proxy_async();
        for (; arrived < it; ++arrived) mbar_arrive(full_a(arrived % p.stages));
        (void)any_h;
    } else if (warp == 4) {
        if (lane == 0) {
            const uint32_t idesc = make_idesc(p.cout);
            int it = 0, j = 0, wrun = -1, cur_k = -1, cur_pass = -1;
            for (int T = t_begin; T < t_end; ++T, ++j) {
                int pass, k, pbase, cnt;
                decode(T, pass, k, pbase, cnt);
                if (k != cur_k || pass != cur_pass) {
                    ++wrun; cur_k = k; cur_pass = pass;
                    mbar_wait(w_full, wrun & 1);
                    tc_fence_after();
                }
                const int buf = j & 1;
                if (j >= 2) { mbar_wait(acc_empty(buf), ((j >> 1) - 1) & 1); tc_fence_after(); }
                const uint32_t tmem_acc = tmem_d + (uint32_t)(buf * p.acc_stride);
                for (int c = 0; c < p.nchunks; ++c, ++it) {
                    const int s = it % p.stages;
                    mbar_wait(full_a(s), (it / p.stages) & 1);
                    tc_fence_after();
                    const uint32_t a_hi = a_base + (uint32_t)s * a_stage, a_lo = a_hi + A_TILE;
                    const uint32_t b_hi = base + (uint32_t)c * 2u * b_tile, b_lo = b_hi + b_tile;
                    const int ksteps = min(KC, ctot - c * KC) >> 4;
                    for (int ks = 0; ks < ksteps; ++ks) {
                        const uint64_t dah = make_desc(a_hi + ks * 32), dal = make_desc(a_lo + ks * 32);
                        const uint64_t dbh = make_desc(b_hi + ks * 32), dbl = make_desc(b_lo + ks * 32);
                        umma(tmem_acc, dah, dbh, idesc, (c | ks) ? 1u : 0u);
                        umma(tmem_acc, dal, dbh, idesc, 1);
                        umma(tmem_acc, dah, dbl, idesc, 1);
                    }
                    umma_commit(empty_a(s));
                }
                umma_commit(acc_full(buf));
                bool run_ends = (T + 1 == t_end);
                if (!run_ends) {
                    int p2, k2, pb2, c2;
                    decode(T + 1, p2, k2, pb2, c2);
                    run_ends = (k2 != k) || (p2 != pass);
                }
                if (run_ends) umma_commit(w_empty);
            }
        }
        __syncwarp();
    } else if (warp == 5) {
        if (lane == 0) {
            int wrun = -1, cur_k = -1, cur_pass = -1;
            for (int T = t_begin; T < t_end; ++T) {
                int pass, k, pbase, cnt;
                decode(T, pass, k, pbase, cnt);
                if (k == cur_k && pass == cur_pass) continue;
                ++wrun; cur_k = k; cur_pass = pass;
                if (wrun >= 1) mbar_wait(w_empty, (wrun - 1) & 1);
                const unsigned char* src = p.wpacked + PACK_HEADER + (size_t)k * w_bytes;
                mbar_expect_tx(w_full, w_bytes);
                for (int c = 0; c < p.nchunks; ++c) bulk_g2s(base + (uint32_t)c * 2u * b_tile, src + (size_t)c * 2u * b_tile, 2u * b_tile, w_full);
            }
        }
        __syncwarp();
    } else {
        const int q4 = warp & 3;
        const float out_scale = __ldg(reinterpret_cast<const float*>(p.wpacked) + 1);
        const uint32_t lane_base = (uint32_t)(q4 * 32) << 16;
        float* myslab = slab + (size_t)q4 * 32 * SLAB_PITCH;
        int j = 0;
        for (int T = t_begin; T < t_end; ++T, ++j) {
            int pass, k, pbase, cnt;
            decode(T, pass, k, pbase, cnt);
            const int r = q4 * 32 + lane;
            const int orow = r < cnt ? __ldg(p.pair_out + pbase + r) : -1;
            const int buf = j & 1;
            mbar_wait(acc_full(buf), (j >> 1) & 1);
            tc_fence_after();
            for (int c0 = 0; c0 < p.cout; c0 += 32) {
                uint32_t v[32];
                tmem_ld32(tmem_d + lane_base + (uint32_t)(buf * p.acc_stride + c0), v);
                tmem_ld_wait();
                __syncwarp();
                float* srow = myslab + lane * SLAB_PITCH;
#pragma unroll
                for (int q = 0; q < 8; ++q)
                    *reinterpret_cast<float4*>(srow + q * 4) = make_float4(__uint_as_float(v[q * 4]) * out_scale, __uint_as_float(v[q * 4 + 1]) * out_scale,
                                                                           __uint_as_float(v[q * 4 + 2]) * out_scale, __uint_as_float(v[q * 4 + 3]) * out_scale);
                __syncwarp();
#pragma unroll
                for (int e = lane; e < 256; e += 32) {
                    const int rr = e >> 3, c4 = (e & 7) * 4;
                    const int dst_row = __shfl_sync(0xffffffffu, orow, rr);
                    if (dst_row >= 0) {
                        const float4 a4 = *reinterpret_cast<const float4*>(myslab + rr * SLAB_PITCH + c4);
                        asm volatile("red.global.add.v4.f32 [%0], {%1, %2, %3, %4};" ::"l"(p.out[pass] + (long long)dst_row * p.cout + c0 + c4),
                                     "f"(a4.x), "f"(a4.y), "f"(a4.z), "f"(a4.w) : "memory");
                    }
                }
            }
            tc_fence_before();
            mbar_arrive(acc_empty(buf));
        }
    }
    tc_fence_before();
    __syncthreads();
    if (warp == 4) asm volatile("tcgen05.dealloc.cta_group::1.sync.aligned.b32 %0, %1;" ::"r"(tmem_d), "r"((uint32_t)p.tmem_cols) : "memory");
}

__global__ void k_pair_count(const int* __restrict__ nbr, long long nbr_stride, const int* __restrict__ d_n, int n_cap, int skip_k,
                             int* __restrict__ cnt) {
    const int k = blockIdx.y;
    if (k == skip_k) return;
    const int n = d_n ? min(*d_n, n_cap) : n_cap;
    const int o = blockIdx.x * blockDim.x + threadIdx.x;
    const bool hit = o < n && nbr[(long long)k * nbr_stride + o] >= 0;
    const unsigned m = __ballot_sync(0xffffffffu, hit);
    if ((threadIdx.x & 31) == 0 && m) atomicAdd(cnt + k, __popc(m));
}

__global__ void k_pair_scan(const int* __restrict__ cnt, int kvol, int* __restrict__ koff, int* __restrict__ tile_off, int* __restrict__ cursor) {
    if (threadIdx.x == 0) {
        int a = 0, t = 0;
        for (int k = 0; k < kvol; ++k) { koff[k] = a; tile_off[k] = t; cursor[k] = 0; a += cnt[k]; t += (cnt[k] + tc::BM - 1) / tc::BM; }
        koff[kvol] = a; tile_off[kvol] = t;
    }
}

__global__ void k_pair_fill(const int* __restrict__ nbr, long long nbr_stride, const int* __restrict__ d_n, int n_cap, int skip_k,
                            const int* __restrict__ koff, int* __restrict__ cursor, int* __restrict__ pair_in, int* __restrict__ pair_out) {
    const int k = blockIdx.y;
    if (k == skip_k) return;
    const int n = d_n ? min(*d_n, n_cap) : n_cap;
    const int o = blockIdx.x * blockDim.x + threadIdx.x;
    const int v = o < n ? nbr[(long long)k * nbr_stride + o] : -1;
    const unsigned m = __ballot_sync(0xffffffffu, v >= 0);
    if (!m) return;
    const int lane = threadIdx.x & 31;
    int basep = 0;
    if (lane == __ffs(m) - 1) basep = atomicAdd(cursor + k, __popc(m));
    basep = __shfl_sync(0xffffffffu, basep, __ffs(m) - 1);
    if (v >= 0) {
        const int pos = koff[k] + basep + __popc(m & ((1u << lane) - 1));
        pair_in[pos] = v;
        pair_out[pos] = o;
    }
}

__global__ void k_zero_rows(float* __restrict__ buf, const int* __restrict__ d_n, int n_cap, int c) {
    const long long t = (long long)blockIdx.x * blockDim.x + threadIdx.x;
    const int n = d_n ? min(*d_n, n_cap) : n_cap;
    if (t < (long long)n * c / 4) reinterpret_cast<float4*>(buf)[t] = make_float4(0.f, 0.f, 0.f, 0.f);
}

static size_t smem_bytes(int cin, int cout, int stages) {
    const int nchunks = (cin + tc::KC - 1) / tc::KC;
    return 1024 + (size_t)nchunks * 2 * cout * 128 + (size_t)stages * 2 * tc::A_TILE + SLAB_BYTES + (2 * MAX_STAGES + 6) * 8 + 64;
}

static bool shape_ok(int c1, int c2, int cout, int kvol) {
    const int ctot = c1 + c2;
    if (kvol < 1 || kvol > MAX_KVOL || ctot % 16 || ctot < 16) return false;
    if (c2 > 0 && (c1 % 8 || c2 % 8)) return false;
    if (cout % 32 || cout < 32 || cout > 128) return false;
    return smem_bytes(ctot, cout, 2) <= 227 * 1024 - 256;
}

}

extern "C" size_t lb2_pair_list_scratch_bytes(void) { return 2 * 32 * sizeof(int); }

extern "C" int lb2_pair_list(void* handle, void* stream, const int32_t* nbr, int64_t nbr_stride, const int32_t* d_nout,
                             int32_t nout_cap, int32_t kvol, int32_t skip_k, int32_t* pair_in, int32_t* pair_out,
                             int32_t* koff, int32_t* tile_off, void* scratch) {
    Lb2Handle* h = (Lb2Handle*)handle;
    LB2_REQUIRE(h, h && nbr && pair_in && pair_out && koff && tile_off && scratch && nout_cap > 0 && kvol >= 1 && kvol <= sc::MAX_KVOL, "pair_list");
    cudaStream_t s = (cudaStream_t)stream;
    int* cnt = (int*)scratch;
    int* cursor = cnt + 32;
    if (cudaMemsetAsync(cnt, 0, 64 * sizeof(int), s) != cudaSuccess) return lb2_fail(h, LB2_ERR_CUDA, "pair_list memset%s", "");
    dim3 grid(cdiv(nout_cap, 256), kvol);
    sc::k_pair_count<<<grid, 256, 0, s>>>(nbr, nbr_stride, d_nout, nout_cap, skip_k, cnt);
    LB2_POST_LAUNCH(h, "k_pair_count");
    sc::k_pair_scan<<<1, 32, 0, s>>>(cnt, kvol, koff, tile_off, cursor);
    LB2_POST_LAUNCH(h, "k_pair_scan");
    sc::k_pair_fill<<<grid, 256, 0, s>>>(nbr, nbr_stride, d_nout, nout_cap, skip_k, koff, cursor, pair_in, pair_out);
    LB2_POST_LAUNCH(h, "k_pair_fill");
    return LB2_OK;
}

extern "C" int lb2_spconv_scatter_supported(int32_t c1, int32_t c2, int32_t cout, int32_t kvol) { return sc::shape_ok(c1, c2, cout, kvol) ? 1 : 0; }

extern "C" int lb2_spconv_scatter(void* handle, void* stream, const lb2_scatter_desc* d) {
    Lb2Handle* h = (Lb2Handle*)handle;
    LB2_REQUIRE(h, h && d && d->weight_packed && d->pair_in && d->pair_out && d->koff && d->tile_off, "spconv_scatter null");
    LB2_REQUIRE(h, d->npass == 1 || d->npass == 2, "npass");
    if (!sc::shape_ok(d->c1, d->c2, d->cout, d->kvol)) return lb2_fail(h, LB2_ERR_UNSUP, "spconv_scatter: shape not supported%s", "");
    cudaStream_t s = (cudaStream_t)stream;
    sc::Params p;
    p.c1 = d->c1; p.c2 = d->c2; p.cout = d->cout; p.kvol = d->kvol; p.npass = d->npass;
    p.nchunks = (d->c1 + d->c2 + tc::KC - 1) / tc::KC;
    p.wpacked = (const unsigned char*)d->weight_packed;
    p.pair_in = d->pair_in; p.pair_out = d->pair_out; p.koff = d->koff; p.tile_off = d->tile_off;
    for (int i = 0; i < 2; ++i) {
        const int j = d->npass > 1 ? i : 0;
        LB2_REQUIRE(h, d->in1[j] && d->out[j] && ((d->c2 > 0) == (d->in2[j] != nullptr)), "spconv_scatter io");
        p.in1[i] = d->in1[j]; p.in2[i] = d->in2[j]; p.out[i] = d->out[j];
        p.in1_h[i] = d->in1_h[j]; p.in2_h[i] = d->in2_h[j];
    }
    int stages = sc::MAX_STAGES;
    while (stages > 2 && sc::smem_bytes(d->c1 + d->c2, d->cout, stages) > 227 * 1024 - 256) --stages;
    p.stages = stages;
    const int half = d->cout <= 32 ? 32 : d->cout <= 64 ? 64 : 128;
    p.acc_stride = half; p.tmem_cols = 2 * half;
    if (d->zero_rows_cap > 0) {
        for (int i = 0; i < d->npass; ++i) {
            sc::k_zero_rows<<<cdiv((long long)d->zero_rows_cap * d->cout / 4, 256), 256, 0, s>>>(d->out[i], d->d_zero_rows, d->zero_rows_cap, d->cout);
            LB2_POST_LAUNCH(h, "k_zero_rows");
        }
    }
    {
        cudaError_t e = lb2_configure_smem(h, LB2_K_SCATTER, sc::k_spconv_scatter, (int)(227 * 1024 - 256));
        if (e != cudaSuccess) return lb2_fail(h, LB2_ERR_CUDA, "k_spconv_scatter smem attribute: %s", cudaGetErrorString(e));
    }
    sc::k_spconv_scatter<<<h->num_sms, sc::THREADS, sc::smem_bytes(d->c1 + d->c2, d->cout, stages), s>>>(p);
    LB2_POST_LAUNCH(h, "k_spconv_scatter");
    return LB2_OK;
}
```

### lidiff_b200/csrc/spconv_tc.cu

```cuda
#include "common.cuh"
#include <algorithm>
#include <stdlib.h>
#include "tc_common.cuh"

namespace tc {

constexpr int NUM_PRODUCER = 128;
constexpr int THREADS = 320;
constexpr int DRAIN_WARP0 = 6;
constexpr int STEP_BUDGET = 64;
constexpr int MAX_KVOL = 27;
constexpr int MAX_STAGES = 4;

struct Params {
    int c1, c2, cout, kvol;
    const unsigned char* wpacked;
    const float* scale;
    const float* shift;
    int relu;
    const int* nbr;
    long long nbr_stride;
    const int* d_mout;
    int mout_cap;
    const int* row_perm;
    int stages, nchunks, tmem_cols, tot_col, group;
    int nbuf, acc_stride;
    int ncta;
    lb2_conv_io io[2];
};

__global__ void __launch_bounds__(THREADS, 1) k_spconv_tc(const Params p) {
    extern __shared__ unsigned char smem_raw[];
    const int M = p.d_mout ? min(*p.d_mout, p.mout_cap) : p.mout_cap;
    const int m0 = blockIdx.x * BM;
    if (m0 >= M) return;
    const lb2_conv_io io = p.io[blockIdx.y];
    const int n0 = blockIdx.z * p.ncta;
    const int warp = threadIdx.x >> 5, lane = threadIdx.x & 31;
    const int ctot = p.c1 + p.c2;

    const uint32_t raw = smem_u32(smem_raw);
    const uint32_t base = (raw + 1023u) & ~1023u;
    unsigned char* gen = smem_raw + (base - raw);
    const uint32_t b_tile = (uint32_t)p.ncta * 128u;
    const uint32_t b_full = (uint32_t)p.cout * 128u;
    const float out_scale = __ldg(reinterpret_cast<const float*>(p.wpacked) + 1);
    const uint32_t stage_bytes = 2u * A_TILE + 2u * b_tile;
    unsigned char* tail = gen + (size_t)p.stages * stage_bytes;
    int* idx_s = reinterpret_cast<int*>(tail);
    uint64_t* bars = reinterpret_cast<uint64_t*>(tail + MAX_KVOL * BM * sizeof(int));
    uint32_t* misc = reinterpret_cast<uint32_t*>(bars + 3 * MAX_STAGES + 4);
    int* row_s = reinterpret_cast<int*>(misc + 4);
    const uint32_t bar0 = smem_u32(bars);
    auto full_a = [&](int s) { return bar0 + 8u * s; };
    auto full_b = [&](int s) { return bar0 + 8u * (MAX_STAGES + s); };
    auto empty = [&](int s) { return bar0 + 8u * (2 * MAX_STAGES + s); };
    auto acc_full = [&](int b) { return bar0 + 8u * (3 * MAX_STAGES + b); };
    auto acc_empty = [&](int b) { return bar0 + 8u * (3 * MAX_STAGES + 2 + b); };

    if (threadIdx.x == 0) {
        for (int s = 0; s < p.stages; ++s) { mbar_init(full_a(s), NUM_PRODUCER); mbar_init(full_b(s), 1); mbar_init(empty(s), 1); }
        for (int b = 0; b < 2; ++b) { mbar_init(acc_full(b), 1); mbar_init(acc_empty(b), 128); }
        misc[1] = 0;
        asm volatile("fence.mbarrier_init.release.cluster;" ::: "memory");
    }
    if (warp == 4) {
        asm volatile("tcgen05.alloc.cta_group::1.sync.aligned.shared::cta.b32 [%0], %1;" ::"r"(smem_u32(&misc[0])), "r"((uint32_t)p.tmem_cols) : "memory");
        asm volatile("tcgen05.relinquish_alloc_permit.cta_group::1.sync.aligned;" ::: "memory");
    }
    __syncthreads();
    if (threadIdx.x < BM) {
        const int slot = m0 + threadIdx.x;
        const int row = (slot < M) ? (p.row_perm ? __ldg(p.row_perm + slot) : slot) : -1;
        row_s[threadIdx.x] = row;
        uint32_t mymask = 0;
        for (int k0 = 0; k0 < p.kvol; k0 += 9) {
            int v[9];
#pragma unroll
            for (int q = 0; q < 9; ++q) {
                const int k = k0 + q;
                v[q] = -1;
                if (k < p.kvol && row >= 0) v[q] = p.nbr ? __ldg(p.nbr + (long long)k * p.nbr_stride + row) : row;
            }
#pragma unroll
            for (int q = 0; q < 9; ++q) {
                const int k = k0 + q;
                if (k < p.kvol) {
                    idx_s[k * BM + threadIdx.x] = v[q];
                    if (__any_sync(0xffffffffu, v[q] >= 0)) mymask |= 1u << k;
                }
            }
        }
        if (lane == 0 && mymask) atomicOr(&misc[1], mymask);
    }
    tc_fence_before();
    __syncthreads();
    tc_fence_after();
    const uint32_t tmem_d = misc[0];
    const uint32_t kmask = misc[1];
    const int n_off = __popc(kmask);
    const int n_groups = (n_off + p.group - 1) / p.group;

    if (warp < 4) {
        const int sub = threadIdx.x & 7;
        const int rbase = threadIdx.x >> 3;
        const bool use_h = (io.in1_h != nullptr) && (p.c2 == 0 || io.in2_h != nullptr);
        const int D = p.stages - 1;
        int it = 0, arrived = 0;
        for (uint32_t km = kmask; km; km &= km - 1) {
            const int k = __ffs(km) - 1;
            const int* idxk = idx_s + k * BM;
            int src[8];
#pragma unroll
            for (int j = 0; j < 8; ++j) src[j] = idxk[rbase + 16 * j];
            for (int c = 0; c < p.nchunks; ++c, ++it) {
                const int s = it % p.stages;
                mbar_wait(empty(s), ((it / p.stages) & 1) ^ 1);
                unsigned char* a_hi = gen + (size_t)s * stage_bytes;
                const uint32_t a_hi_u = base + (uint32_t)s * stage_bytes;
                const int ch = c * KC + sub * 8;
                if (ch < ctot) {
                    const bool first = ch < p.c1;
                    const int cw = first ? p.c1 : p.c2;
                    const int co = first ? ch : ch - p.c1;
                    if (use_h) produce_a_split(reinterpret_cast<const __half*>(first ? io.in1_h : io.in2_h), cw, co, src, a_hi_u, a_hi_u + A_TILE, rbase, sub);
                    else produce_a_f32(first ? io.in1 : io.in2, cw, co, src, a_hi, a_hi + A_TILE, rbase, sub);
                }
                if (use_h) {
                    cp_async_commit();
                    if (it >= D) {
                        cp_async_wait_dyn(D);
                        fence_proxy_async();
                        mbar_arrive(full_a(arrived % p.stages));
                        ++arrived;
                    }
                } else {
                    fence_proxy_async();
                    mbar_arrive(full_a(s));
                }
            }
        }
        if (use_h) {
            cp_async_wait<0>();
            fence_proxy_async();
            for (; arrived < it; ++arrived) mbar_arrive(full_a(arrived % p.stages));
        }
    } else if (warp == 4) {
        if (lane == 0) {
            const uint32_t idesc = make_idesc(p.ncta);
            int it = 0, in_group = 0, group_idx = 0, off_idx = 0;
            for (uint32_t km = kmask; km; km &= km - 1, ++off_idx) {
                const int buf = group_idx % p.nbuf;
                const uint32_t tmem_acc = tmem_d + (uint32_t)(buf * p.acc_stride);
                if (in_group == 0 && group_idx >= p.nbuf) {
                    mbar_wait(acc_empty(buf), ((group_idx / p.nbuf) - 1) & 1);
                    tc_fence_after();
                }
                for (int c = 0; c < p.nchunks; ++c, ++it) {
                    const int s = it % p.stages;
                    const uint32_t par = (it / p.stages) & 1;
                    mbar_wait(full_b(s), par);
                    mbar_wait(full_a(s), par);
                    tc_fence_after();
                    const uint32_t a_hi = base + (uint32_t)s * stage_bytes, a_lo = a_hi + A_TILE;
                    const uint32_t b_hi = a_lo + A_TILE, b_lo = b_hi + b_tile;
                    const int ksteps = min(KC, ctot - c * KC) >> 4;
                    for (int ks = 0; ks < ksteps; ++ks) {
                        const uint64_t dah = make_desc(a_hi + ks * 32), dal = make_desc(a_lo + ks * 32);
                        const uint64_t dbh = make_desc(b_hi + ks * 32), dbl = make_desc(b_lo + ks * 32);
                        umma(tmem_acc, dah, dbh, idesc, (in_group | c | ks) ? 1u : 0u);
                        umma(tmem_acc, dal, dbh, idesc, 1);
                        umma(tmem_acc, dah, dbl, idesc, 1);
                    }
                    umma_commit(empty(s));
                }
                if (++in_group == p.group || off_idx == n_off - 1) {
                    umma_commit(acc_full(buf));
                    in_group = 0;
                    ++group_idx;
                }
            }
        }
        __syncwarp();
    } else if (warp >= DRAIN_WARP0) {
        const int q4 = warp & 3;
        const uint32_t lane_base = (uint32_t)(q4 * 32) << 16;
        float* stage_c = reinterpret_cast<float*>(gen);
        const int pitch = p.ncta + 4;
        for (int g = 0; g < max(n_groups, 1); ++g) {
            const bool last = g >= n_groups - 1;
            const int buf = g % p.nbuf;
            const uint32_t acc_col = (uint32_t)(buf * p.acc_stride);
            if (n_groups > 0) {
                mbar_wait(acc_full(buf), (g / p.nbuf) & 1);
                tc_fence_after();
            }
            for (int c0 = 0; c0 < p.ncta; c0 += 32) {
                float acc[32];
                if (n_groups > 0) {
                    uint32_t r[32];
                    tmem_ld32(tmem_d + lane_base + acc_col + (uint32_t)c0, r);
                    if (g > 0) {
                        uint32_t t[32];
                        tmem_ld32(tmem_d + lane_base + (uint32_t)(p.tot_col + c0), t);
                        tmem_ld_wait();
#pragma unroll
                        for (int j = 0; j < 32; ++j) acc[j] = __fadd_rn(__uint_as_float(t[j]), __uint_as_float(r[j]));
                    } else {
                        tmem_ld_wait();
#pragma unroll
                        for (int j = 0; j < 32; ++j) acc[j] = __uint_as_float(r[j]);
                    }
                } else {
#pragma unroll
                    for (int j = 0; j < 32; ++j) acc[j] = 0.f;
                }
                if (!last) {
                    uint32_t t[32];
#pragma unroll
                    for (int j = 0; j < 32; ++j) t[j] = __float_as_uint(acc[j]);
                    tmem_st32(tmem_d + lane_base + (uint32_t)(p.tot_col + c0), t);
                } else {
                    float* srow = stage_c + (size_t)(q4 * 32 + lane) * pitch + c0;
#pragma unroll
                    for (int q = 0; q < 8; ++q)
                        *reinterpret_cast<float4*>(srow + q * 4) = make_float4(acc[q * 4] * out_scale, acc[q * 4 + 1] * out_scale,
                                                                               acc[q * 4 + 2] * out_scale, acc[q * 4 + 3] * out_scale);
                }
            }
            if (!last) {
                asm volatile("tcgen05.wait::st.sync.aligned;" ::: "memory");
                tc_fence_before();
                mbar_arrive(acc_empty(buf));
            }
        }
        asm volatile("bar.sync 1, 128;" ::: "memory");
        const int nv = p.ncta >> 2;
        for (int e = lane; e < 32 * nv; e += 32) {
            const int rr = q4 + 4 * (e / nv);
            const int lcol = (e % nv) * 4;
            const int col = n0 + lcol;
            const int orow = row_s[rr];
            if (orow < 0) continue;
            const long long ro = (long long)orow * p.cout;
            const float4 a4 = *reinterpret_cast<const float4*>(stage_c + (size_t)rr * pitch + lcol);
            float y[4] = {a4.x, a4.y, a4.z, a4.w};
            if (io.pre_add) {
                const float4 t4 = __ldg(reinterpret_cast<const float4*>(io.pre_add + ro + col));
                y[0] += t4.x; y[1] += t4.y; y[2] += t4.z; y[3] += t4.w;
            }
            if (p.scale) {
                const float4 s4 = __ldg(reinterpret_cast<const float4*>(p.scale + col));
                const float4 h4 = __ldg(reinterpret_cast<const float4*>(p.shift + col));
                y[0] = fmaf(y[0], s4.x, h4.x); y[1] = fmaf(y[1], s4.y, h4.y); y[2] = fmaf(y[2], s4.z, h4.z); y[3] = fmaf(y[3], s4.w, h4.w);
            }
            if (io.residual || io.residual_h) {
                const float4 t4 = load_residual4(io.residual, io.residual_h, orow, p.cout, col);
                y[0] += t4.x; y[1] += t4.y; y[2] += t4.z; y[3] += t4.w;
            }
            if (p.relu) {
#pragma unroll
                for (int j = 0; j < 4; ++j) y[j] = fmaxf(y[j], 0.f);
            }
            if (io.out) *reinterpret_cast<float4*>(io.out + ro + col) = make_float4(y[0], y[1], y[2], y[3]);
            if (io.out_h) store_split4(io.out_h, orow, p.cout, col, y);
            if (io.out_gated || io.out_gated_h) {
                if (io.gate_table) {
                    const long long g = io.gate_idx ? __ldg(io.gate_idx + orow) : 0;
                    const float4 g4 = __ldg(reinterpret_cast<const float4*>(io.gate_table + g * p.cout + col));
                    y[0] *= g4.x; y[1] *= g4.y; y[2] *= g4.z; y[3] *= g4.w;
                }
                if (io.out_gated) *reinterpret_cast<float4*>(io.out_gated + ro + col) = make_float4(y[0], y[1], y[2], y[3]);
                if (io.out_gated_h) store_split4(io.out_gated_h, orow, p.cout, col, y);
            }
        }
    } else if (warp == 5) {
        if (lane == 0) {
            int it = 0;
            for (uint32_t km = kmask; km; km &= km - 1) {
                const int k = __ffs(km) - 1;
                for (int c = 0; c < p.nchunks; ++c, ++it) {
                    const int s = it % p.stages;
                    mbar_wait(empty(s), ((it / p.stages) & 1) ^ 1);
                    const uint32_t dst = base + (uint32_t)s * stage_bytes + 2u * A_TILE;
                    const unsigned char* src = p.wpacked + PACK_HEADER + ((size_t)k * p.nchunks + c) * (2u * b_full) + (size_t)n0 * 128u;
                    mbar_expect_tx(full_b(s), 2u * b_tile);
                    bulk_g2s(dst, src, b_tile, full_b(s));
                    bulk_g2s(dst + b_tile, src + b_full, b_tile, full_b(s));
                }
            }
        }
        __syncwarp();
    }
    tc_fence_before();
    __syncthreads();
    if (warp == 4) {
        asm volatile("tcgen05.dealloc.cta_group::1.sync.aligned.b32 %0, %1;" ::"r"(tmem_d), "r"((uint32_t)p.tmem_cols) : "memory");
    }
}

__global__ void k_weight_absmax(const float* __restrict__ w, long long n, unsigned* __restrict__ header) {
    long long t = (long long)blockIdx.x * blockDim.x + threadIdx.x;
    float m = 0.f;
    for (; t < n; t += (long long)gridDim.x * blockDim.x) m = fmaxf(m, fabsf(w[t]));
#pragma unroll
    for (int o = 16; o > 0; o >>= 1) m = fmaxf(m, __shfl_xor_sync(0xffffffffu, m, o));
    if ((threadIdx.x & 31) == 0) atomicMax(header, __float_as_uint(m));
}

__device__ __forceinline__ float weight_scale(unsigned max_bits) {
    const float m = __uint_as_float(max_bits);
    if (!(m > 0.f) || !isfinite(m)) return 1.f;
    int e;
    frexpf(m, &e);
    return ldexpf(1.f, 14 - e);
}

__global__ void k_pack_weights(const float* __restrict__ w, int kvol, int cin, int cout, int nchunks, unsigned char* __restrict__ out) {
    const long long total = (long long)kvol * nchunks * cout * KC;
    long long t = (long long)blockIdx.x * blockDim.x + threadIdx.x;
    const float scale = weight_scale(*reinterpret_cast<const unsigned*>(out));
    if (t == 0) reinterpret_cast<float*>(out)[1] = 1.0f / scale;
    if (t >= total) return;
    const int kk = (int)(t % KC);
    const int n = (int)((t / KC) % cout);
    const int c = (int)((t / ((long long)KC * cout)) % nchunks);
    const int k = (int)(t / ((long long)KC * cout * nchunks));
    const int ch = c * KC + kk;
    const float v = ch < cin ? w[((long long)k * cin + ch) * cout + n] * scale : 0.f;
    const __half hi = __float2half_rn(v);
    const __half lo = __float2half_rn(v - __half2float(hi));
    const size_t tile = (size_t)cout * 128;
    unsigned char* blob = out + PACK_HEADER + ((size_t)k * nchunks + c) * 2 * tile;
    const uint32_t off = sw128(n, kk >> 3) + (uint32_t)(kk & 7) * 2u;
    *reinterpret_cast<__half*>(blob + off) = hi;
    *reinterpret_cast<__half*>(blob + tile + off) = lo;
}

static bool shape_ok(int c1, int c2, int cout, int kvol) {
    const int ctot = c1 + c2;
    if (kvol < 1 || kvol > MAX_KVOL) return false;
    if (ctot % 16 != 0 || ctot < 16) return false;
    if (c2 > 0 && (c1 % 8 != 0 || c2 % 8 != 0)) return false;
    if (cout % 32 != 0 || cout < 32 || cout > 256) return false;
    return true;
}

static size_t smem_bytes(int cout, int stages) {
    return 1024 + (size_t)stages * (2 * A_TILE + 2 * (size_t)cout * 128) + MAX_KVOL * BM * sizeof(int) + (3 * MAX_STAGES + 4) * 8 + 16 + BM * sizeof(int);
}

}

bool lb2_spconv_tc_supported(const lb2_conv_desc* d) { return tc::shape_ok(d->c1, d->c2, d->cout, d->kvol); }

extern "C" size_t lb2_packed_weight_bytes(int32_t kvol, int32_t cin, int32_t cout) {
    if (!tc::shape_ok(cin, 0, cout, kvol)) return 0;
    const int nchunks = (cin + tc::KC - 1) / tc::KC;
    return tc::PACK_HEADER + (size_t)kvol * nchunks * 2 * (size_t)cout * 128;
}

extern "C" int lb2_pack_weights(void* handle, void* stream, const float* weight, int32_t kvol, int32_t cin, int32_t cout, void* packed) {
    Lb2Handle* h = (Lb2Handle*)handle;
    LB2_REQUIRE(h, h && weight && packed, "pack_weights null");
    if (!tc::shape_ok(cin, 0, cout, kvol)) return lb2_fail(h, LB2_ERR_UNSUP, "pack_weights: shape not supported by the tensor-core variant%s", "");
    const int nchunks = (cin + tc::KC - 1) / tc::KC;
    const long long total = (long long)kvol * nchunks * cout * tc::KC;
    const long long nw = (long long)kvol * cin * cout;
    if (cudaMemsetAsync(packed, 0, tc::PACK_HEADER, (cudaStream_t)stream) != cudaSuccess) return lb2_fail(h, LB2_ERR_CUDA, "pack_weights memset%s", "");
    tc::k_weight_absmax<<<(unsigned)std::min<long long>(cdiv(nw, 256), 1024), 256, 0, (cudaStream_t)stream>>>(weight, nw, (unsigned*)packed);
    LB2_POST_LAUNCH(h, "k_weight_absmax");
    tc::k_pack_weights<<<cdiv(total, 256), 256, 0, (cudaStream_t)stream>>>(weight, kvol, cin, cout, nchunks, (unsigned char*)packed);
    LB2_POST_LAUNCH(h, "k_pack_weights");
    return LB2_OK;
}


int lb2_spconv_tc2_launch(Lb2Handle* h, cudaStream_t s, const lb2_conv_desc* d, int step_budget);

int lb2_spconv_tc_launch(Lb2Handle* h, cudaStream_t s, const lb2_conv_desc* d, bool persistent) {
    if (persistent && h->opt[LB2_OPT_TC_PERSISTENT]) return lb2_spconv_tc2_launch(h, s, d, tc::STEP_BUDGET);
    tc::Params p;
    p.c1 = d->c1; p.c2 = d->c2; p.cout = d->cout; p.kvol = d->kvol;
    p.wpacked = (const unsigned char*)d->weight_packed;
    p.scale = d->scale; p.shift = d->shift; p.relu = d->relu;
    p.nbr = d->nbr; p.nbr_stride = d->nbr_stride; p.d_mout = d->d_mout; p.mout_cap = d->mout_cap; p.row_perm = d->row_perm;
    p.nchunks = (d->c1 + d->c2 + tc::KC - 1) / tc::KC;
    const int nsplit = (d->cout == 256 && h->opt[LB2_OPT_TC_NSPLIT]) ? 2 : 1;
    p.ncta = d->cout / nsplit;
    int stages = tc::MAX_STAGES;
    while (stages > 1 && tc::smem_bytes(p.ncta, stages) > 227 * 1024) --stages;
    p.stages = stages;
    const int half = p.ncta <= 32 ? 32 : p.ncta <= 64 ? 64 : p.ncta <= 128 ? 128 : 256;
    p.nbuf = half <= 128 ? 2 : 1;
    p.acc_stride = half;
    p.tot_col = p.nbuf * half;
    { int need = (p.nbuf + 1) * half; p.tmem_cols = 32; while (p.tmem_cols < need) p.tmem_cols <<= 1; }
    const int steps_per_offset = 3 * ((d->c1 + d->c2 + 15) / 16);
    p.group = std::max(1, tc::STEP_BUDGET / steps_per_offset);
    p.io[0] = d->io[0]; p.io[1] = d->io[d->npass > 1 ? 1 : 0];
    const size_t smem = tc::smem_bytes(p.ncta, stages);
    {
        cudaError_t e = lb2_configure_smem(h, LB2_K_TC, tc::k_spconv_tc, (int)(227 * 1024));
        if (e != cudaSuccess) return lb2_fail(h, LB2_ERR_CUDA, "k_spconv_tc smem attribute: %s", cudaGetErrorString(e));
    }
    dim3 grid(cdiv(d->mout_cap, tc::BM), d->npass, nsplit);
    tc::k_spconv_tc<<<grid, tc::THREADS, smem, s>>>(p);
    LB2_POST_LAUNCH(h, "k_spconv_tc");
    return LB2_OK;
}
```

### lidiff_b200/engine.py

```python
from __future__ import annotations

import math
import os
from collections import ChainMap

import numpy as np
import torch

from . import _lib
from ._lib import ConvDesc, ConvIO, DpmCoef, ScatterDesc
from .scheduler import DPMSolverMultistepScheduler

GATE_NAMES = ("stage1", "stage2", "stage3", "stage4", "up1", "up2", "up3", "up4")
GATE_LEVEL = (0, 1, 2, 3, 4, 3, 2, 1)
BN_EPS = 1e-5


class ConvLayer:

    def __init__(self, h, sd, pconv, pbn, device):
        W = sd[f"{pconv}.kernel"].detach().to(device=device, dtype=torch.float32)
        if W.dim() == 2:
            W = W[None]
        self.W = W.contiguous()
        self.kvol, self.cin, self.cout = self.W.shape
        self.name = pconv
        if pbn is not None:
            g = lambda k: sd[f"{pbn}.bn.{k}"].detach().to(device=device, dtype=torch.float32)
            scale = g("weight") / torch.sqrt(g("running_var") + BN_EPS)
            self.scale = scale.contiguous()
            self.shift = (g("bias") - g("running_mean") * scale).contiguous()
        else:
            self.scale = self.shift = None
        self.Wp = h.pack_weights(self.W)
        self.Wc = self.Wpc = None
        if self.kvol == 27 and self.Wp is not None and h.scatter_supported(self.cin, 0, self.cout, 27):
            self.Wc = self.W[13:14].contiguous()
            self.Wpc = h.pack_weights(self.Wc)


class Linear:
    def __init__(self, sd, p, device, cols=None):
        w = sd[f"{p}.weight"].detach().to(device=device, dtype=torch.float32)
        self.w = (w if cols is None else w[:, cols[0]:cols[1]]).contiguous()
        self.b = sd[f"{p}.bias"].detach().to(device=device, dtype=torch.float32).contiguous()
        self.n_out, self.n_in = self.w.shape


class Act:
    __slots__ = ("f", "h", "P", "cap", "C")

    def __init__(self, P, cap, C, f, h):
        self.P, self.cap, self.C, self.f, self.h = P, cap, C, f, h


def _ptr(t, p):
    return None if t is None else t[min(p, t.shape[0] - 1)].data_ptr()


def _net_layers(h, sd, device, decoder: bool):
    L = {}

    def add(pconv, pbn):
        L[pconv] = ConvLayer(h, sd, pconv, pbn, device)

    def res(p):
        add(f"{p}.net.0", f"{p}.net.1")
        add(f"{p}.net.3", f"{p}.net.4")
        if f"{p}.downsample.0.kernel" in sd:
            add(f"{p}.downsample.0", f"{p}.downsample.1")

    add("stem.0", "stem.1")
    add("stem.3", "stem.4")
    for n in range(1, 5):
        add(f"stage{n}.0.net.0", f"stage{n}.0.net.1")
        res(f"stage{n}.1")
        res(f"stage{n}.2")
    if decoder:
        for n in range(1, 5):
            add(f"up{n}.0.net.0", f"up{n}.0.net.1")
            res(f"up{n}.1.0")
            res(f"up{n}.1.1")
    return L


class Geometry:

    def __init__(self, h, n_cap: int, with_up: bool = True, levels: int = 5, use_pairs: bool = True):
        dev = h.device
        self.h, self.n_cap, self.levels, self.use_pairs = h, n_cap, levels, use_pairs
        i32 = dict(dtype=torch.int32, device=dev)
        self.C = [torch.zeros((n_cap, 4), **i32) for _ in range(levels)]
        self.d_n = [torch.zeros(1, **i32) for _ in range(levels)]
        self.grid = [h.new_grid(n_cap) for _ in range(levels)]
        self.inv = [torch.zeros(n_cap, **i32) for _ in range(levels)]
        self.nbr3 = [torch.empty((27, n_cap), **i32) for _ in range(levels)]
        self.nbr_dn = [None] + [torch.empty((8, n_cap), **i32) for _ in range(levels - 1)]
        self.nbr_up = [torch.empty((8, n_cap), **i32) for _ in range(levels - 1)] + [None] if with_up else None
        self.scratch = h.unique_scratch(n_cap)
        self.counts = torch.empty(n_cap, **i32)
        self.pairs = torch.zeros(18, dtype=torch.int64, device=dev)
        self.map_id = {}
        self.mask_of = {}
        self.ro_scratch = torch.zeros((h.row_order_scratch_bytes(n_cap) + 3) // 4, **i32)
        self.ro_scratch_late = self.to_scratch_late = None
        self.perm3 = [torch.zeros(n_cap, **i32) for _ in range(levels)]
        self.perm_dn = [None] + [torch.zeros(n_cap, **i32) for _ in range(levels - 1)]
        self.perm_up = [torch.zeros(n_cap, **i32) for _ in range(levels - 1)] + [None] if with_up else None
        self.perm_of = {}
        self.use_tile_order = os.environ.get("LB2_TILE_ORDER", "1") != "0"
        self.map_self = os.environ.get("LB2_MAP_SELF", "1") != "0"
        self.tile_order_of = {}
        self.to_scratch = torch.zeros((n_cap + 127) // 128, **i32)
        self.morton_levels = set(int(c) for c in os.environ.get("LB2_MORTON_LEVELS", "") if c.isdigit())
        self.pair_levels = min(3, levels)
        self.pair_level_set = set(int(c) for c in os.environ.get("LB2_SCATTER_LEVELS", "") if c.isdigit())
        self.pairs_of = {}
        self.pl_scratch = torch.zeros(64, **i32)
        want = [use_pairs and l in self.pair_level_set for l in range(self.pair_levels)]
        self.pair_in = [torch.zeros(26 * n_cap, **i32) if w else None for w in want]
        self.pair_out = [torch.zeros(26 * n_cap, **i32) if w else None for w in want]
        self.koff = [torch.zeros(28, **i32) for _ in range(self.pair_levels)]
        self.tile_off = [torch.zeros(28, **i32) for _ in range(self.pair_levels)]

    def build(self, coords_f: torch.Tensor, n_points: int, after_levels=None, late_stream=None, late_done=None):
        h, N = self.h, self.n_cap
        h.unique_build(coords_f, None, None, n_points, 0, self.grid[0], self.C[0], self.inv[0], self.d_n[0], self.scratch)
        for l in range(1, self.levels):
            h.unique_build(None, self.C[l - 1], self.d_n[l - 1], N, 1 << l, self.grid[l], self.C[l], self.inv[l], self.d_n[l], self.scratch)
        if after_levels is not None:
            after_levels()
        self.pairs.zero_()

        def one(grid, l_out, ks, step, nbr, perm, slot, ro_scratch=None, to_scratch=None):
            ro_scratch = self.ro_scratch if ro_scratch is None else ro_scratch
            to_scratch = self.to_scratch if to_scratch is None else to_scratch
            mask = self.mask_of.get(nbr.data_ptr())
            if mask is None:
                mask = self.mask_of[nbr.data_ptr()] = torch.zeros(N, dtype=torch.int32, device=nbr.device)
            if ks == 3 and self.map_self:
                h.kernel_map_self(grid, self.C[l_out], self.d_n[l_out], N, step, nbr, N, self.pairs[slot:slot + 1], mask)
            else:
                h.kernel_map(grid, self.C[l_out], self.d_n[l_out], N, ks, step, nbr, N, self.pairs[slot:slot + 1], mask)
            morton = ks == 3 and l_out in self.morton_levels
            h.row_order(mask, self.d_n[l_out], N, ks ** 3, perm, ro_scratch, self.C[l_out] if morton else None, l_out)
            if self.use_tile_order:
                to = self.tile_order_of.get(nbr.data_ptr())
                if to is None:
                    to = self.tile_order_of[nbr.data_ptr()] = (torch.zeros((N + 127) // 128, dtype=torch.int32, device=nbr.device),
                                                               torch.zeros((N + 255) // 256, dtype=torch.int32, device=nbr.device))
                h.tile_order(mask, perm, self.d_n[l_out], N, to[0], to[1], to_scratch)
            self.map_id[nbr.data_ptr()] = slot
            self.perm_of[nbr.data_ptr()] = perm

        def map3(l, **kw):
            one(self.grid[l], l, 3, 1 << l, self.nbr3[l], self.perm3[l], l, **kw)
            if l < self.pair_levels and self.use_pairs and l in self.pair_level_set:
                h.pair_list(self.nbr3[l], N, self.d_n[l], N, 27, 13, self.pair_in[l], self.pair_out[l], self.koff[l], self.tile_off[l], self.pl_scratch)
                self.pairs_of[self.nbr3[l].data_ptr()] = l

        def map_dn(l, **kw):
            one(self.grid[l - 1], l, 2, 1 << (l - 1), self.nbr_dn[l], self.perm_dn[l], 4 + l, **kw)

        def map_up(l, **kw):
            one(self.grid[l + 1], l, 2, -(1 << l), self.nbr_up[l], self.perm_up[l], 9 + l, **kw)

        split = late_stream is not None and self.levels >= 3 and not (self.use_pairs and self.pair_level_set)
        early3 = (0, 1) if split else tuple(range(self.levels))
        early_dn = (1,) if split else tuple(range(1, self.levels))
        if split:
            if self.ro_scratch_late is None:
                self.ro_scratch_late, self.to_scratch_late = torch.zeros_like(self.ro_scratch), torch.zeros_like(self.to_scratch)
            kw = dict(ro_scratch=self.ro_scratch_late, to_scratch=self.to_scratch_late)
            late_stream.wait_stream(torch.cuda.current_stream())
            with torch.cuda.stream(late_stream):
                for l in range(2, self.levels):
                    map_dn(l, **kw)
                    map3(l, **kw)
                if self.nbr_up is not None:
                    for l in range(self.levels - 2, -1, -1):
                        map_up(l, **kw)
                late_done.record(late_stream)
        for l in early3:
            if l >= 1 and l in early_dn:
                map_dn(l)
            map3(l)
        for l in early_dn:
            if l not in early3:
                map_dn(l)
        if not split and self.nbr_up is not None:
            for l in range(self.levels - 1):
                map_up(l)

    def voxel_mean(self, feats, n_points, out):
        self.h.voxel_mean(feats, self.inv[0], n_points, feats.shape[1], self.d_n[0], self.n_cap, out, self.counts)

    def sizes(self):
        return [int(d.item()) for d in self.d_n]


class _PairLookup:

    def __init__(self, geom):
        self.geom = geom

    def get(self, ptr):
        l = self.geom.pairs_of.get(ptr)
        return None if l is None else (self.geom, l)


class DenoiseEngine:
    def __init__(self, sd_enc: dict, sd_diff: dict, *, device="cuda", n_points=180000, denoising_steps=50,
                 cond_weight=6.0, resolution=0.05, t_steps=1000, beta_start=3.5e-5, beta_end=0.007,
                 div_mode=1, conv_algo=_lib.ALGO_AUTO, batch_coord=0.0, sd_refine: dict | None = None, max_range=50.0):
        self.device = torch.device(device)
        self.h = _lib.get_handle(self.device)
        self.N = int(n_points)
        self.w = float(cond_weight)
        self.resolution = float(resolution)
        self.div_mode = int(div_mode)
        self.conv_algo = conv_algo
        h, dev = self.h, self.device
        self.enc = _net_layers(h, sd_enc, dev, decoder=False)
        self.diff = _net_layers(h, sd_diff, dev, decoder=True)
        self.refine = _net_layers(h, sd_refine, dev, decoder=True) if sd_refine is not None else None
        self.refine_head = (Linear(sd_refine, "last.0", dev), Linear(sd_refine, "last.2", dev)) if sd_refine is not None else None
        self.max_range = float(max_range)
        self.sched = DPMSolverMultistepScheduler(num_train_timesteps=t_steps, beta_start=beta_start, beta_end=beta_end,
                                                 beta_schedule="linear", algorithm_type="sde-dpmsolver++", solver_order=2)
        self.sched.set_timesteps(denoising_steps)
        self.T = len(self.sched.timesteps)
        self.latent = [(Linear(sd_diff, f"latent_{g}.0", dev), Linear(sd_diff, f"latent_{g}.2", dev)) for g in GATE_NAMES]
        self.temp = [(Linear(sd_diff, f"{g}_temp.0", dev), Linear(sd_diff, f"{g}_temp.2", dev)) for g in GATE_NAMES]
        self.lat_p, self.lat_t, self.lat_2 = [], [], []
        for g in GATE_NAMES:
            half = sd_diff[f"latemp_{g}.0.weight"].shape[1] // 2
            pc, tc = ((half, 2 * half), (0, half)) if g == "up1" else ((0, half), (half, 2 * half))
            self.lat_p.append(Linear(sd_diff, f"latemp_{g}.0", dev, cols=pc))
            self.lat_t.append(Linear(sd_diff, f"latemp_{g}.0", dev, cols=tc))
            self.lat_2.append(Linear(sd_diff, f"latemp_{g}.2", dev))
        self.head = (Linear(sd_diff, "last.0", dev), Linear(sd_diff, "last.2", dev))
        self._bufs = {}
        self._graphs = {}
        self.use_row_order = True
        self.use_scatter = True
        self.use_split = True
        self.lean = os.environ.get("LB2_LEAN", "1") != "0" and not os.environ.get("LB2_SCATTER_LEVELS")
        self._acts = {}
        self._perm_lookup = {}
        self._tile_order_lookup = {}
        self.geom = Geometry(h, self.N, with_up=True)
        self._perm_lookup = self.geom.perm_of
        self._mask_lookup = self.geom.mask_of
        self._tile_order_lookup = self.geom.tile_order_of
        self._pairs_lookup = _PairLookup(self.geom)
        self.geom_cond = None
        self.part_cap = 0
        self.nn_algo = os.environ.get("LB2_NN_ALGO", "tree")
        self.use_side_stream = os.environ.get("LB2_SIDE_STREAM", "1") != "0" and torch.cuda.is_available() and self.device.type == "cuda"
        if self.use_side_stream:
            self._side = torch.cuda.Stream(device=self.device)
            self._side_done = torch.cuda.Event()
            self._side2 = torch.cuda.Stream(device=self.device)
            self._side2_done = torch.cuda.Event()
            self._side3 = torch.cuda.Stream(device=self.device)
            self._side3_done = torch.cuda.Event()
        self.late_maps = self.use_side_stream and os.environ.get("LB2_LATE_MAPS", "1") != "0"
        self.conv_events = None
        self.layer_log = None
        self.pair_hist = None
        self._hist_row = 0
        self._conv_counter = 0
        self._have_x0 = False
        self.use_graphs = os.environ.get("LB2_GRAPHS", "1") != "0" and torch.cuda.is_available() and self.device.type == "cuda"
        self._graphs = {}
        self._eager_steps = 0
        self.graph_replays = 0
        self.replayed_launches = 0
        self._captured_launches = 0
        self._prepare_time_tables()
        self._prepare_uncond()

    @classmethod
    def from_modules(cls, pipe, **kw):
        sd_e = {k: v for k, v in pipe.partial_enc.state_dict().items()}
        sd_d = {k: v for k, v in pipe.model.state_dict().items()}
        hp = pipe.hparams
        if getattr(pipe, "model_refine", None) is not None:
            kw.setdefault("sd_refine", {k: v for k, v in pipe.model_refine.state_dict().items()})
        kw.setdefault("max_range", hp["data"].get("max_range", 50.0))
        return cls(sd_e, sd_d, device=pipe.device, n_points=hp["data"]["num_points"], denoising_steps=hp["diff"]["s_steps"],
                   cond_weight=pipe.w_uncond, resolution=hp["data"]["resolution"], t_steps=hp["diff"]["t_steps"],
                   beta_start=hp["diff"]["beta_start"], beta_end=hp["diff"]["beta_end"], **kw)

    def buf(self, name, shape, dtype=torch.float32):
        t = self._bufs.get(name)
        if t is None or tuple(t.shape) != tuple(shape) or t.dtype != dtype:
            if t is not None:
                self._graphs.clear()
            t = torch.zeros(shape, dtype=dtype, device=self.device)
            self._bufs[name] = t
        return t

    def act(self, name, P, cap, C, f32=True, split=True) -> Act:
        split = bool(split and self.use_split and self.conv_algo != _lib.ALGO_FFMA and C % 8 == 0)
        f32 = bool(f32 or not split)
        a = self._acts.get(name)
        if a is None or (a.P, a.cap, a.C) != (P, cap, C) or (a.f is not None) != f32 or (a.h is not None) != split:
            if a is not None:
                self._graphs.clear()
            f = torch.zeros((P, cap, C), dtype=torch.float32, device=self.device) if f32 else None
            hh = torch.zeros((P, cap, 2 * C), dtype=torch.float16, device=self.device) if split else None
            a = self._acts[name] = Act(P, cap, C, f, hh)
        return a

    def _linear(self, x, lin: Linear, out, act=0, m_cap=None, d_m=None, prebias=None, pre_act=0, bias=True):
        m_cap = x.shape[0] if m_cap is None else m_cap
        self.h.linear(x, x.stride(0), lin.w, lin.b if bias else None, None, 0, m_cap, d_m, lin.n_in, lin.n_out, act,
                      out, out.stride(0), prebias, pre_act)
        return out

    def _head(self, x, head, out, out_act, d_m):
        l0, l1 = head
        self.h.head_mlp(x, x.stride(1), x.stride(0), l0.w, l0.b, l1.w, l1.b, x.shape[1], d_m, l0.n_in, l0.n_out, l1.n_out, out_act,
                        x.shape[0], out, out.stride(1), out.stride(0))

    def _timestep_embedding(self, ts: torch.Tensor) -> torch.Tensor:
        half = 48
        freq = torch.from_numpy(np.exp(np.arange(0, half) * -(np.log(10000) / (half - 1)))).float().to(self.device)
        arg = ts.to(self.device)[:, None] * freq[None, :]
        return torch.cat([torch.sin(arg), torch.cos(arg)], dim=1).contiguous()

    def _prepare_time_tables(self):
        T, dev = self.T, self.device
        temb = self._timestep_embedding(self.sched.timesteps)
        self.bvec = []
        for g in range(8):
            l0, l2 = self.temp[g]
            u = self._linear(temb, l0, torch.empty((T, l0.n_out), device=dev), act=1)
            tv = self._linear(u, l2, torch.empty((T, l2.n_out), device=dev))
            self.bvec.append(self._linear(tv, self.lat_t[g], torch.empty((T, self.lat_t[g].n_out), device=dev)))

    def _gate_tables(self, A_list, rows_cap, d_rows, step, tag):
        out = []
        for g in range(8):
            t = self.buf(f"gate_{tag}_{g}", (rows_cap, self.lat_2[g].n_out))
            self._linear(A_list[g], self.lat_2[g], t, m_cap=rows_cap, d_m=d_rows, prebias=self.bvec[g][step], pre_act=1)
            out.append(t)
        return out

    def _part_A(self, part_F, rows_cap, d_rows, tag):
        A = []
        for g in range(8):
            l0, l2 = self.latent[g]
            h1 = self._linear(part_F, l0, self.buf(f"lat_h_{tag}", (rows_cap, l0.n_out)), act=1, m_cap=rows_cap, d_m=d_rows)
            p = self._linear(h1, l2, self.buf(f"lat_p_{tag}", (rows_cap, l2.n_out)), m_cap=rows_cap, d_m=d_rows)
            a = self.buf(f"lat_A_{tag}_{g}", (rows_cap, self.lat_p[g].n_out))
            A.append(self._linear(p, self.lat_p[g], a, m_cap=rows_cap, d_m=d_rows, bias=False))
        return A

    def _conv(self, lay: ConvLayer, nbr, d_m, cap, in1: Act, in2: Act = None, out: Act = None, residual: Act = None, relu=True,
              gate=None, out_gated: Act = None, npass=1):
        d = ConvDesc()
        d.c1 = in1.C
        d.c2 = in2.C if in2 is not None else 0
        assert d.c1 + d.c2 == lay.cin, (d.c1, d.c2, lay.cin)
        f = lambda a: None if a is None else a.f
        hh = lambda a: None if a is None else a.h
        pre = None
        geom_lvl = self._pairs_lookup.get(nbr.data_ptr()) if (nbr is not None and self.use_scatter and lay.Wpc is not None
                                                               and self.conv_algo != _lib.ALGO_FFMA) else None
        if geom_lvl is not None:
            g, l = geom_lvl
            pre = self.buf(f"scatter.{lay.cout}", (2, cap, lay.cout))
            sd = ScatterDesc()
            sd.c1, sd.c2, sd.cout, sd.kvol = d.c1, d.c2, lay.cout, 27
            sd.weight_packed = lay.Wp.data_ptr()
            sd.pair_in, sd.pair_out = g.pair_in[l].data_ptr(), g.pair_out[l].data_ptr()
            sd.koff, sd.tile_off = g.koff[l].data_ptr(), g.tile_off[l].data_ptr()
            sd.npass = npass
            for p in range(npass):
                sd.in1[p], sd.in2[p], sd.out[p] = _ptr(f(in1), p), _ptr(f(in2), p), pre[p].data_ptr()
                sd.in1_h[p], sd.in2_h[p] = _ptr(hh(in1), p), _ptr(hh(in2), p)
            sd.d_zero_rows, sd.zero_rows_cap = d_m.data_ptr(), cap
        else:
            sd = None
        map_ptr = nbr.data_ptr() if nbr is not None else None
        d.cout, d.kvol = lay.cout, (1 if pre is not None else lay.kvol)
        d.weight = (lay.Wc if pre is not None else lay.W).data_ptr()
        wp = lay.Wpc if pre is not None else lay.Wp
        d.weight_packed = wp.data_ptr() if wp is not None else None
        d.scale = lay.scale.data_ptr() if lay.scale is not None else None
        d.shift = lay.shift.data_ptr() if lay.shift is not None else None
        d.relu = 1 if relu else 0
        if pre is not None:
            nbr = None
        d.nbr = nbr.data_ptr() if nbr is not None else None
        d.nbr_stride = nbr.stride(0) if nbr is not None else cap
        d.d_mout = d_m.data_ptr() if d_m is not None else None
        d.mout_cap, d.npass = cap, npass
        perm = self._perm_lookup.get(nbr.data_ptr()) if (nbr is not None and self.use_row_order) else None
        d.row_perm = perm.data_ptr() if perm is not None else None
        mask = self._mask_lookup.get(nbr.data_ptr()) if nbr is not None else None
        d.row_mask = mask.data_ptr() if mask is not None else None
        to = self._tile_order_lookup.get(nbr.data_ptr()) if (nbr is not None and perm is not None) else None
        d.tile_order128 = to[0].data_ptr() if to is not None else None
        d.tile_order256 = to[1].data_ptr() if to is not None else None
        res_h = hh(residual) if (residual is not None and residual.f is None) else None
        for p in range(npass):
            gt = gi = None
            if gate is not None:
                gt = gate[p][0].data_ptr()
                gi = gate[p][1].data_ptr() if gate[p][1] is not None else None
            d.io[p] = ConvIO(_ptr(f(in1), p), _ptr(f(in2), p), _ptr(f(residual), p), _ptr(f(out), p), gt, gi, _ptr(f(out_gated), p),
                             pre[p].data_ptr() if pre is not None else None,
                             _ptr(hh(in1), p), _ptr(hh(in2), p), _ptr(hh(out), p), _ptr(hh(out_gated), p), _ptr(res_h, p))
        if self.layer_log is not None:
            self.layer_log.append(dict(name=lay.name, scatter=sd is not None, map=map_ptr, d_m=d_m.data_ptr() if d_m is not None else None,
                                       cin=lay.cin, cout=lay.cout, kvol=lay.kvol, npass=npass,
                                       tc=bool(lay.Wp is not None and self.conv_algo != _lib.ALGO_FFMA)))
        if self.conv_events is not None:
            e0, e1 = torch.cuda.Event(enable_timing=True), torch.cuda.Event(enable_timing=True)
            e0.record()
            if sd is not None:
                self.h.spconv_scatter(sd)
            self.h.spconv(d, self.conv_algo)
            e1.record()
            self.conv_events.append((e0, e1, self._conv_counter))
            self._conv_counter += 1
        else:
            if sd is not None:
                self.h.spconv_scatter(sd)
            self.h.spconv(d, self.conv_algo)

    def _res(self, L, p, geom, lvl, in1: Act, in2: Act, npass, tag, gate=None, want_plain=True, lean=False, out_f32=False):
        cap = geom.n_cap
        nbr, d_m = geom.nbr3[lvl], geom.d_n[lvl]
        cmid = L[f"{p}.net.0"].cout
        hbuf = self.act(f"{tag}.h", npass, cap, cmid, f32=not lean)
        self._conv(L[f"{p}.net.0"], nbr, d_m, cap, in1, in2, out=hbuf, npass=npass)
        if f"{p}.downsample.0" in L:
            sbuf = self.act(f"{tag}.s", npass, cap, cmid, split=not lean)
            self._conv(L[f"{p}.downsample.0"], None, d_m, cap, in1, in2, out=sbuf, relu=False, npass=npass)
        else:
            assert in2 is None
            sbuf = in1
        out = self.act(f"{tag}.o", npass, cap, cmid, f32=(not lean) or out_f32) if want_plain else None
        og = self.act(f"{tag}.g", npass, cap, cmid, f32=not lean) if gate is not None else None
        self._conv(L[f"{p}.net.3"], nbr, d_m, cap, hbuf, None, out=out, residual=sbuf, relu=True, gate=gate, out_gated=og, npass=npass)
        return out, og

    def _encoder(self, L, geom, F0: Act, npass, tag, gates=None, lean=False, before_gates=None, before_stage2=None):
        cap = geom.n_cap
        s0 = self.act(f"{tag}.stem0", 1, cap, 32, f32=not lean)
        self._conv(L["stem.0"], geom.nbr3[0], geom.d_n[0], cap, F0, out=s0, npass=1)
        x0 = self.act(f"{tag}.x0", 1, cap, 32, f32=(not lean) or gates is not None)
        self._conv(L["stem.3"], geom.nbr3[0], geom.d_n[0], cap, s0, out=x0, npass=1)
        skips = [x0]
        if gates is not None:
            if before_gates is not None:
                before_gates()
            cur = self.act(f"{tag}.x0g", npass, cap, 32, f32=not lean)
            for p in range(npass):
                tb, ix = gates[0][p]
                self.h.gate_mul(x0.f[0], tb, ix, geom.d_n[0], cap, 32, cur.f[p] if cur.f is not None else None,
                                cur.h[p] if cur.h is not None else None)
        else:
            cur = x0
        for n in range(1, 5):
            if n == 2 and before_stage2 is not None:
                before_stage2()
            a = self.act(f"{tag}.s{n}a", npass, cap, L[f"stage{n}.0.net.0"].cout, f32=not lean)
            self._conv(L[f"stage{n}.0.net.0"], geom.nbr_dn[n], geom.d_n[n], cap, cur, out=a, npass=npass)
            b, _ = self._res(L, f"stage{n}.1", geom, n, a, None, npass, f"{tag}.s{n}r1", lean=lean)
            g = gates[n] if gates is not None else None
            x, xg = self._res(L, f"stage{n}.2", geom, n, b, None, npass, f"{tag}.s{n}r2", gate=g, lean=lean)
            skips.append(x)
            cur = xg if gates is not None else x
        return skips, cur

    def _decoder(self, L, geom, skips, cur: Act, npass, tag, gates, lean=False):
        cap = geom.n_cap
        y = cur
        for n in range(1, 5):
            lvl = 4 - n
            d = self.act(f"{tag}.u{n}d", npass, cap, L[f"up{n}.0.net.0"].cout, f32=not lean)
            self._conv(L[f"up{n}.0.net.0"], geom.nbr_up[lvl], geom.d_n[lvl], cap, y, out=d, npass=npass)
            b, _ = self._res(L, f"up{n}.1.0", geom, lvl, d, skips[lvl], npass, f"{tag}.u{n}r1", lean=lean)
            g = gates[4 + n] if (gates is not None and n < 4) else None
            o, og = self._res(L, f"up{n}.1.1", geom, lvl, b, None, npass, f"{tag}.u{n}r2", gate=g, want_plain=(g is None), lean=lean,
                              out_f32=(n == 4))
            y = og if g is not None else o
        return y

    def _prepare_uncond(self):
        dev = self.device
        g1 = Geometry(self.h, 16, with_up=False, use_pairs=False)
        coords = torch.zeros((16, 4), dtype=torch.float32, device=dev)
        g1.build(coords, 16)
        F0 = self.act("uenc.F0", 1, 16, 3)
        F0.f.zero_()
        skips, _ = self._encoder(self.enc, g1, F0, 1, "uenc")
        part_u = skips[4].f[0][:1].clone()
        A = self._part_A(part_u, 1, None, "u")
        self.table_u = []
        for g in range(8):
            t = torch.empty((self.T, self.lat_2[g].n_out), device=dev)
            for s in range(self.T):
                self._linear(A[g], self.lat_2[g], t[s:s + 1], prebias=self.bvec[g][s], pre_act=1)
            self.table_u.append(t)
        for k in [k for k in self._acts if k.startswith("uenc")]:
            del self._acts[k]

    def set_condition(self, scan: torch.Tensor):
        dev, N = self.device, scan.shape[0]
        pts = scan.to(device=dev, dtype=torch.float32).contiguous()
        if self.geom_cond is None or self.geom_cond.n_cap != N:
            self._graphs.clear()
            self.geom_cond = Geometry(self.h, N, with_up=False, use_pairs=False)
            self._perm_lookup = ChainMap(self.geom.perm_of, self.geom_cond.perm_of)
            self._mask_lookup = ChainMap(self.geom.mask_of, self.geom_cond.mask_of)
            self._tile_order_lookup = ChainMap(self.geom.tile_order_of, self.geom_cond.tile_order_of)
        coords = self.buf("cond.coords", (N, 4))
        coords[:, 0] = 0
        self.h.quantize(pts, self.resolution, self.div_mode, self.buf("cond.q", (N, 3)))
        coords[:, 1:] = self._bufs["cond.q"]
        g = self.geom_cond
        g.build(coords, N)
        F0 = self.act("cond.F0", 1, N, 3)
        g.voxel_mean(pts, N, F0.f[0])
        skips, _ = self._encoder(self.enc, g, F0, 1, "cenc")
        self.part_F = skips[4].f[0]
        self.part_C, self.part_dn, self.part_grid = g.C[4], g.d_n[4], g.grid[4]
        self.part_cap = N
        self.part_tree = self.h.nn_tree(self.part_C, self.part_dn, N, out=getattr(self, "part_tree", None))
        self.A_cond = self._part_A(self.part_F, N, self.part_dn, "c")

    def step(self, i: int, x_t, x_next, coords, coords_next, x_init, noise_i, x0_state, eps_out=None):
        h, N, g = self.h, self.N, self.geom
        self._conv_counter = 0
        nn = [None] * 5
        tabs_box = []

        def gate_tables():
            tabs_box.append(self._gate_tables(self.A_cond, self.part_cap, self.part_dn, i, "c"))

        if self.use_side_stream:
            self._side2.wait_stream(torch.cuda.current_stream())
            with torch.cuda.stream(self._side2):
                gate_tables()
                self._side2_done.record(self._side2)
        else:
            gate_tables()

        def matches():
            for l in range(4, -1, -1):
                ix = self.buf(f"nn{l}", (N,), torch.int32)
                if self.nn_algo == "grid":
                    h.nn_match_grid(g.C[l], g.d_n[l], N, self.part_C, self.part_dn, self.part_cap, self.part_grid, 16, 4, ix)
                elif l == 4:
                    h.nn_match_tree(g.C[l], g.d_n[l], N, self.part_tree, self.part_cap, ix)
                else:
                    h.nn_match_tree(g.C[l], g.d_n[l], N, self.part_tree, self.part_cap, ix, self.part_C, g.inv[l + 1], nn[l + 1])
                nn[l] = ix

        def after_levels():
            if not self.use_side_stream:
                return matches()
            main = torch.cuda.current_stream()
            self._side.wait_stream(main)
            with torch.cuda.stream(self._side):
                matches()
                self._side_done.record(self._side)

        def join_sides():
            if self.use_side_stream:
                torch.cuda.current_stream().wait_event(self._side_done)
                torch.cuda.current_stream().wait_event(self._side2_done)

        def join_late_maps():
            if self.late_maps:
                torch.cuda.current_stream().wait_event(self._side3_done)

        if self.late_maps:
            g.build(coords, N, after_levels, late_stream=self._side3, late_done=self._side3_done)
        else:
            g.build(coords, N, after_levels)
        if self.pair_hist is not None:
            if self.late_maps:
                torch.cuda.current_stream().wait_event(self._side3_done)
            g.pairs[13:18] = torch.cat(g.d_n).long()
            self.pair_hist[self._hist_row % self.pair_hist.shape[0]] = g.pairs
            self._hist_row += 1
        F0 = self.act("F0", 1, N, 3)
        g.voxel_mean(x_t, N, F0.f[0])
        tabs_c = tabs_box[0]
        gates = [[(tabs_c[k], nn[GATE_LEVEL[k]]), (self.table_u[k][i:i + 1], None)] for k in range(8)]
        skips, cur = self._encoder(self.diff, g, F0, 2, "d", gates, lean=self.lean, before_gates=join_sides, before_stage2=join_late_maps)
        y4 = self._decoder(self.diff, g, skips, cur, 2, "d", gates, lean=self.lean)
        eps = self.buf("eps_vox", (2, N, 3))
        self._head(y4.f, self.head, eps, 0, g.d_n[0])
        c = self.sched.coefficients(i)
        second = self._have_x0 and not (i == self.T - 1 and self.T < 15)
        self._have_x0 = True
        cf = DpmCoef(c["c_sample"], c["c_x0"], c["c_noise"], c["sigma_s"], c["alpha_s"], c["inv_r0"] if second else 0.0,
                     self.w, self.resolution, 1 if second else 0, self.div_mode, 1)
        h.guidance_dpm_step(eps[0], eps[1], g.inv[0], x_t, x_init, noise_i, x0_state, N, cf, eps_out, x_next, coords_next)

    def start(self, x_init: torch.Tensor, x_feats: torch.Tensor, fresh: bool = True):
        dev, N = self.device, self.N
        if fresh:
            self._have_x0 = False
        x_src = x_init.reshape(-1, 3)
        assert x_src.shape[0] == N, f"engine built for {N} points, got {x_src.shape[0]}"
        x_init = self.buf("x_init", (N, 3), torch.float64)
        x_init.copy_(x_src)
        self.set_condition(x_init)
        st = dict(x_init=x_init, xa=self.buf("x_a", (N, 3)), xb=self.buf("x_b", (N, 3)), ca=self.buf("c_a", (N, 4)),
                  cb=self.buf("c_b", (N, 4)), x0s=self.buf("x0_state", (N, 3), torch.float64), i=0)
        st["xa"].copy_(x_feats.reshape(-1, 3).to(device=dev, dtype=torch.float32))
        st["ca"][:, 0] = 0
        self.h.quantize(st["xa"], self.resolution, self.div_mode, self.buf("q0", (N, 3)))
        st["ca"][:, 1:] = self._bufs["q0"]
        return st

    def advance(self, st, noise_i, host_noise=None, host_out=None):
        i = st["i"] % self.T
        graphed = self.use_graphs and self.conv_events is None and self.layer_log is None and self.pair_hist is None
        if host_noise is not None or graphed:
            nbuf = self.buf("noise_in", (self.N, 3))
            nbuf.copy_(host_noise if host_noise is not None else noise_i, non_blocking=True)
            noise_i = nbuf
        if not graphed or self._eager_steps < 1:
            self.step(i, st["xa"], st["xb"], st["ca"], st["cb"], st["x_init"], noise_i, st["x0s"])
            self._eager_steps += 1
        else:
            second = self._have_x0 and not (i == self.T - 1 and self.T < 15)
            key = (i, st["xa"].data_ptr(), bool(second))
            ent = self._graphs.get(key)
            if ent is None:
                have = self._have_x0
                l0 = self.h.launch_count()
                g = torch.cuda.CUDAGraph()
                with torch.cuda.graph(g):
                    self.step(i, st["xa"], st["xb"], st["ca"], st["cb"], st["x_init"], noise_i, st["x0s"])
                ent = self._graphs[key] = (g, self.h.launch_count() - l0)
                self._captured_launches += ent[1]
                self._have_x0 = have
            ent[0].replay()
            self._have_x0 = True
            self.graph_replays += 1
            self.replayed_launches += ent[1]
        st["xa"], st["xb"], st["ca"], st["cb"] = st["xb"], st["xa"], st["cb"], st["ca"]
        st["i"] += 1
        if host_out is not None:
            host_out.copy_(st["xa"], non_blocking=True)

    def launches(self) -> int:
        return self.h.launch_count() - self._captured_launches + self.replayed_launches

    def run(self, x_init: torch.Tensor, x_feats: torch.Tensor, step_noise=None, n_steps=None, return_device=False, fresh=True):
        dev, N = self.device, self.N
        st = self.start(x_init, x_feats, fresh=fresh)
        T = self.T if n_steps is None else n_steps
        if step_noise is not None:
            step_noise = step_noise.reshape(-1, N, 3).to(device=dev, dtype=torch.float32).contiguous()
        for i in range(T):
            nz = step_noise[i] if step_noise is not None else torch.randn((1, N, 3), device=dev, dtype=torch.float32)[0]
            self.advance(st, nz)
        if return_device:
            return st["xa"]
        out = st["xa"].cpu().numpy()
        if self.h.read_status() & 1:
            raise RuntimeError("lidiff_b200: a coordinate left the supported key range during sampling")
        return out

    def postprocess(self, completed: torch.Tensor, x_init: torch.Tensor) -> torch.Tensor:
        x, y, z = completed[:, 0], completed[:, 1], completed[:, 2]
        dist = torch.sqrt((x * x + y * y) + z * z)
        zi = x_init.reshape(-1, 3)[:, 2]
        max_z = zi.max().item()
        min_z = (zi.mean() - 2 * zi.std()).item()
        keep = (dist < self.max_range) & (z < max_z) & (z > min_z)
        return completed[keep].contiguous()

    def refine_offsets(self, pts: torch.Tensor) -> torch.Tensor:
        if self.refine is None:
            raise RuntimeError("DenoiseEngine was built without the refinement network (sd_refine)")
        h, g, N = self.h, self.geom, self.N
        pts = pts.to(device=self.device, dtype=torch.float32).contiguous()
        n = pts.shape[0]
        if n > N:
            raise RuntimeError(f"refine_offsets: {n} points exceed the engine capacity {N}")
        if n == 0:
            return torch.zeros((0, 18), device=self.device)
        coords = self.buf("r.coords", (N, 4))
        q = self.buf("r.q", (N, 3))
        h.quantize(pts, self.resolution, self.div_mode, q[:n])
        coords[:n, 0] = 0
        coords[:n, 1:] = q[:n]
        g.build(coords, n)
        F0 = self.act("r.F0", 1, N, 3)
        g.voxel_mean(pts, n, F0.f[0])
        skips, cur = self._encoder(self.refine, g, F0, 1, "r", lean=self.lean)
        y4 = self._decoder(self.refine, g, skips, cur, 1, "r", None, lean=self.lean)
        off_v = self.buf("r.off_v", (1, N, 18))
        self._head(y4.f, self.refine_head, off_v, 2, g.d_n[0])
        off_v = off_v[0]
        out = torch.empty((n, 18), device=self.device)
        h.gather_rows(off_v, g.inv[0], n, 18, out)
        return out

    def complete(self, x_init: torch.Tensor, x_feats: torch.Tensor, step_noise=None, fresh=True):
        x_t = self.run(x_init, x_feats, step_noise, return_device=True, fresh=fresh)
        post = self.postprocess(x_t, x_init.reshape(-1, 3).to(self.device))
        off = self.refine_offsets(post).reshape(-1, 6, 3)
        refined = (post[:, None, :] + off).reshape(-1, 3)
        if self.h.read_status() & 1:
            raise RuntimeError("lidiff_b200: a coordinate left the supported key range during sampling")
        return refined, post
```

Baseline: 60.76.

## Split level-3 sparse conv into dense-tile gather path plus residual scatter

```diff
diff --git a/include/lidiff_b200.h b/include/lidiff_b200.h
--- a/include/lidiff_b200.h
+++ b/include/lidiff_b200.h
@@ -62,6 +62,9 @@
 
 int lb2_tile_order(void* h, void* stream, const uint32_t* row_mask, const int32_t* row_perm, const int32_t* d_n, int32_t n_cap,
                    int32_t* order128, int32_t* order256, void* scratch);
+
+int lb2_tile_split(void* h, void* stream, const uint32_t* row_mask, const int32_t* row_perm, const int32_t* d_n, int32_t n_cap,
+                   int32_t kvol, int32_t min_rows, uint32_t* dense_mask, uint32_t* res_mask);
 
 typedef struct {
     const float*   in1;
@@ -123,7 +126,7 @@
 size_t lb2_pair_list_scratch_bytes(void);
 int lb2_pair_list(void* h, void* stream, const int32_t* nbr, int64_t nbr_stride, const int32_t* d_nout,
                   int32_t nout_cap, int32_t kvol, int32_t skip_k, int32_t* pair_in, int32_t* pair_out,
-                  int32_t* koff, int32_t* tile_off, void* scratch);
+                  int32_t* koff, int32_t* tile_off, void* scratch, const uint32_t* row_mask);
 int lb2_spconv_scatter_supported(int32_t c1, int32_t c2, int32_t cout, int32_t kvol);
 int lb2_spconv_scatter(void* h, void* stream, const lb2_scatter_desc* d);
 
diff --git a/lidiff_b200/_lib.py b/lidiff_b200/_lib.py
--- a/lidiff_b200/_lib.py
+++ b/lidiff_b200/_lib.py
@@ -57,7 +57,7 @@
 
 EXPORTS = [
     "lb2_create", "lb2_destroy", "lb2_last_error", "lb2_version", "lb2_launch_count", "lb2_read_status",
-    "lb2_set_option", "lb2_get_option", "lb2_tile_order",
+    "lb2_set_option", "lb2_get_option", "lb2_tile_order", "lb2_tile_split",
     "lb2_quantize", "lb2_unique_scratch_bytes", "lb2_unique_build", "lb2_voxel_mean", "lb2_kernel_map",
     "lb2_spconv_forward", "lb2_packed_weight_bytes", "lb2_pack_weights", "lb2_nn_match", "lb2_linear",
     "lb2_gate_mul", "lb2_gather_rows", "lb2_head_mlp", "lb2_kernel_map_self", "lb2_guidance_dpm_step", "lb2_farthest_point_sample",
@@ -109,12 +109,13 @@
         d.lb2_kernel_map_self.argtypes = [vp, vp, Grid, vp, vp, i32, i32, vp, i64, vp, vp]
         d.lb2_row_order.argtypes = [vp, vp, vp, vp, i32, i32, vp, vp, vp, i32]
         d.lb2_tile_order.argtypes = [vp, vp, vp, vp, vp, i32, vp, vp, vp]
+        d.lb2_tile_split.argtypes = [vp, vp, vp, vp, vp, i32, i32, i32, vp, vp]
         d.lb2_row_order_scratch_bytes.restype = C.c_size_t
         d.lb2_row_order_scratch_bytes.argtypes = [i32]
         d.lb2_spconv_forward.argtypes = [vp, vp, C.POINTER(ConvDesc), C.c_int]
         d.lb2_pack_weights.argtypes = [vp, vp, vp, i32, i32, i32, vp]
         d.lb2_nn_match.argtypes = [vp, vp, vp, vp, i32, vp, vp, i32, i32, vp]
-        d.lb2_pair_list.argtypes = [vp, vp, vp, i64, vp, i32, i32, i32, vp, vp, vp, vp, vp]
+        d.lb2_pair_list.argtypes = [vp, vp, vp, i64, vp, i32, i32, i32, vp, vp, vp, vp, vp, vp]
         d.lb2_pair_list_scratch_bytes.restype = C.c_size_t
         d.lb2_spconv_scatter.argtypes = [vp, vp, C.POINTER(ScatterDesc)]
         d.lb2_spconv_scatter_supported.argtypes = [i32, i32, i32, i32]
@@ -230,12 +231,16 @@
         self._check(self.dll.lb2_tile_order(self.hp, self._stream(), _ptr(row_mask), _ptr(row_perm), _ptr(d_n), int(n_cap), _ptr(order128),
                                             _ptr(order256), _ptr(scratch)), "lb2_tile_order")
 
+    def tile_split(self, row_mask, row_perm, d_n, n_cap, kvol, min_rows, dense_mask, res_mask):
+        self._check(self.dll.lb2_tile_split(self.hp, self._stream(), _ptr(row_mask), _ptr(row_perm), _ptr(d_n), int(n_cap), int(kvol), int(min_rows),
+                                            _ptr(dense_mask), _ptr(res_mask)), "lb2_tile_split")
+
     def spconv(self, desc: ConvDesc, algo: int = ALGO_AUTO):
         self._check(self.dll.lb2_spconv_forward(self.hp, self._stream(), C.byref(desc), int(algo)), "lb2_spconv_forward")
 
-    def pair_list(self, nbr, nbr_stride, d_nout, nout_cap, kvol, skip_k, pair_in, pair_out, koff, tile_off, scratch):
+    def pair_list(self, nbr, nbr_stride, d_nout, nout_cap, kvol, skip_k, pair_in, pair_out, koff, tile_off, scratch, row_mask=None):
         self._check(self.dll.lb2_pair_list(self.hp, self._stream(), _ptr(nbr), int(nbr_stride), _ptr(d_nout), int(nout_cap), int(kvol), int(skip_k),
-                                           _ptr(pair_in), _ptr(pair_out), _ptr(koff), _ptr(tile_off), _ptr(scratch)), "lb2_pair_list")
+                                           _ptr(pair_in), _ptr(pair_out), _ptr(koff), _ptr(tile_off), _ptr(scratch), _ptr(row_mask)), "lb2_pair_list")
 
     def scatter_supported(self, c1, c2, cout, kvol) -> bool:
         return bool(self.dll.lb2_spconv_scatter_supported(int(c1), int(c2), int(cout), int(kvol)))
diff --git a/lidiff_b200/csrc/coords.cu b/lidiff_b200/csrc/coords.cu
--- a/lidiff_b200/csrc/coords.cu
+++ b/lidiff_b200/csrc/coords.cu
@@ -883,6 +883,30 @@
     for (int u = nt256 + threadIdx.x; u < cap256; u += blockDim.x) order256[u] = -1;
 }
 
+__global__ void __launch_bounds__(256) k_tile_split(const unsigned* __restrict__ mask, const int* __restrict__ perm, const int* __restrict__ d_n,
+                                                    int n_cap, int kvol, int min_rows, unsigned* __restrict__ dense, unsigned* __restrict__ res) {
+    const int n = d_n ? min(*d_n, n_cap) : n_cap;
+    if (blockIdx.x * 256 >= n) return;
+    const int slot = blockIdx.x * 256 + threadIdx.x;
+    const int row = slot < n ? (perm ? __ldg(perm + slot) : slot) : -1;
+    const unsigned m = row >= 0 ? __ldg(mask + row) : 0u;
+    unsigned keep = 0;
+    for (int k = 0; k < kvol; ++k)
+        if (__syncthreads_count((m >> k) & 1u) >= min_rows) keep |= 1u << k;
+    if (row >= 0) { dense[row] = m & keep; res[row] = m & ~keep; }
+}
+
+extern "C" int lb2_tile_split(void* handle, void* stream, const uint32_t* row_mask, const int32_t* row_perm, const int32_t* d_n, int32_t n_cap,
+                              int32_t kvol, int32_t min_rows, uint32_t* dense_mask, uint32_t* res_mask) {
+    Lb2Handle* h = (Lb2Handle*)handle;
+    LB2_REQUIRE(h, h && row_mask && dense_mask && res_mask && n_cap > 0 && kvol >= 1 && kvol <= 32 && min_rows >= 0 && min_rows <= 256,
+                "tile_split");
+    cudaStream_t s = (cudaStream_t)stream;
+    k_tile_split<<<cdiv(n_cap, 256), 256, 0, s>>>(row_mask, row_perm, d_n, n_cap, kvol, min_rows, dense_mask, res_mask);
+    LB2_POST_LAUNCH(h, "k_tile_split");
+    return LB2_OK;
+}
+
 extern "C" int lb2_tile_order(void* handle, void* stream, const uint32_t* row_mask, const int32_t* row_perm, const int32_t* d_n, int32_t n_cap,
                               int32_t* order128, int32_t* order256, void* scratch) {
     Lb2Handle* h = (Lb2Handle*)handle;
diff --git a/lidiff_b200/csrc/spconv_ffma.cu b/lidiff_b200/csrc/spconv_ffma.cu
--- a/lidiff_b200/csrc/spconv_ffma.cu
+++ b/lidiff_b200/csrc/spconv_ffma.cu
@@ -17,12 +17,14 @@
     const int* d_mout;
     int mout_cap;
     const int* row_perm;
+    const unsigned* row_mask;
     lb2_conv_io io[2];
 };
 
 __global__ void __launch_bounds__(FF_THREADS) k_spconv_ffma(const FfmaParams p) {
     __shared__ int   idx_s[FF_BM];
     __shared__ int   row_s[FF_BM];
+    __shared__ unsigned mask_s[FF_BM];
     __shared__ float As[FF_BK][FF_BM + 4];
     __shared__ float Bs[FF_BK][FF_BN + 4];
 
@@ -45,13 +47,17 @@
 #pragma unroll
         for (int j = 0; j < 4; ++j) acc[i][j] = 0.f;
 
-    if (t < FF_BM) row_s[t] = (m0 + t < M) ? (p.row_perm ? __ldg(p.row_perm + m0 + t) : m0 + t) : -1;
+    if (t < FF_BM) {
+        const int row = (m0 + t < M) ? (p.row_perm ? __ldg(p.row_perm + m0 + t) : m0 + t) : -1;
+        row_s[t] = row;
+        mask_s[t] = (row >= 0 && p.row_mask) ? __ldg(p.row_mask + row) : 0xffffffffu;
+    }
     __syncthreads();
     for (int k = 0; k < p.kvol; ++k) {
         int my = -1;
         if (t < FF_BM) {
             const int row = row_s[t];
-            if (row >= 0) my = p.nbr ? __ldg(p.nbr + (long long)k * p.nbr_stride + row) : row;
+            if (row >= 0 && ((mask_s[t] >> k) & 1u)) my = p.nbr ? __ldg(p.nbr + (long long)k * p.nbr_stride + row) : row;
             idx_s[t] = my;
         }
         if (!__syncthreads_or(my >= 0)) continue;
@@ -158,7 +164,7 @@
     FfmaParams p;
     p.c1 = d->c1; p.c2 = d->c2; p.cout = d->cout; p.kvol = d->kvol;
     p.W = d->weight; p.scale = d->scale; p.shift = d->shift; p.relu = d->relu;
-    p.nbr = d->nbr; p.nbr_stride = d->nbr_stride; p.d_mout = d->d_mout; p.mout_cap = d->mout_cap; p.row_perm = d->row_perm;
+    p.nbr = d->nbr; p.nbr_stride = d->nbr_stride; p.d_mout = d->d_mout; p.mout_cap = d->mout_cap; p.row_perm = d->row_perm; p.row_mask = d->row_mask;
     p.io[0] = d->io[0]; p.io[1] = d->io[d->npass > 1 ? 1 : 0];
     dim3 grid(cdiv(d->mout_cap, FF_BM), cdiv(d->cout, FF_BN), d->npass);
     k_spconv_ffma<<<grid, FF_THREADS, 0, s>>>(p);
diff --git a/lidiff_b200/csrc/spconv_scatter.cu b/lidiff_b200/csrc/spconv_scatter.cu
--- a/lidiff_b200/csrc/spconv_scatter.cu
+++ b/lidiff_b200/csrc/spconv_scatter.cu
@@ -10,6 +10,7 @@
 constexpr int MAX_KVOL = 27;
 constexpr int SLAB_PITCH = 36;
 constexpr int SLAB_BYTES = BM * SLAB_PITCH * 4;
+constexpr int NBAR = 2 * MAX_STAGES + 8;
 
 struct Params {
     int c1, c2, cout, kvol, nchunks, stages, npass;
@@ -24,6 +25,7 @@
     const void* in2_h[2];
     float* out[2];
     int acc_stride, tmem_cols;
+    int stream_w;
 };
 
 __global__ void __launch_bounds__(THREADS, 1) k_spconv_scatter(const Params p) {
@@ -38,23 +40,24 @@
     const uint32_t base = (raw + 1023u) & ~1023u;
     unsigned char* gen = smem_raw + (base - raw);
     const uint32_t b_tile = (uint32_t)p.cout * 128u;
-    const uint32_t w_bytes = (uint32_t)p.nchunks * 2u * b_tile;
+    const uint32_t w_bytes = (uint32_t)(p.stream_w ? 2 : p.nchunks) * 2u * b_tile;
     const uint32_t a_stage = 2u * A_TILE;
     unsigned char* a_gen = gen + w_bytes;
     const uint32_t a_base = base + w_bytes;
     float* slab = reinterpret_cast<float*>(a_gen + (size_t)p.stages * a_stage);
     uint64_t* bars = reinterpret_cast<uint64_t*>(reinterpret_cast<unsigned char*>(slab) + SLAB_BYTES);
-    uint32_t* misc = reinterpret_cast<uint32_t*>(bars + 2 * MAX_STAGES + 6);
+    uint32_t* misc = reinterpret_cast<uint32_t*>(bars + NBAR);
     const uint32_t bar0 = smem_u32(bars);
     auto full_a = [&](int s) { return bar0 + 8u * s; };
     auto empty_a = [&](int s) { return bar0 + 8u * (MAX_STAGES + s); };
-    const uint32_t w_full = bar0 + 8u * (2 * MAX_STAGES), w_empty = bar0 + 8u * (2 * MAX_STAGES + 1);
-    auto acc_full = [&](int b) { return bar0 + 8u * (2 * MAX_STAGES + 2 + b); };
-    auto acc_empty = [&](int b) { return bar0 + 8u * (2 * MAX_STAGES + 4 + b); };
+    auto w_full = [&](int s) { return bar0 + 8u * (2 * MAX_STAGES + s); };
+    auto w_empty = [&](int s) { return bar0 + 8u * (2 * MAX_STAGES + 2 + s); };
+    auto acc_full = [&](int b) { return bar0 + 8u * (2 * MAX_STAGES + 4 + b); };
+    auto acc_empty = [&](int b) { return bar0 + 8u * (2 * MAX_STAGES + 6 + b); };
 
     if (threadIdx.x == 0) {
         for (int s = 0; s < p.stages; ++s) { mbar_init(full_a(s), 128); mbar_init(empty_a(s), 1); }
-        mbar_init(w_full, 1); mbar_init(w_empty, 1);
+        for (int s = 0; s < 2; ++s) { mbar_init(w_full(s), 1); mbar_init(w_empty(s), 1); }
         for (int b = 0; b < 2; ++b) { mbar_init(acc_full(b), 1); mbar_init(acc_empty(b), 128); }
         asm volatile("fence.mbarrier_init.release.cluster;" ::: "memory");
     }
@@ -126,9 +129,9 @@
             for (int T = t_begin; T < t_end; ++T, ++j) {
                 int pass, k, pbase, cnt;
                 decode(T, pass, k, pbase, cnt);
-                if (k != cur_k || pass != cur_pass) {
+                if (!p.stream_w && (k != cur_k || pass != cur_pass)) {
                     ++wrun; cur_k = k; cur_pass = pass;
-                    mbar_wait(w_full, wrun & 1);
+                    mbar_wait(w_full(0), wrun & 1);
                     tc_fence_after();
                 }
                 const int buf = j & 1;
@@ -138,8 +141,9 @@
                     const int s = it % p.stages;
                     mbar_wait(full_a(s), (it / p.stages) & 1);
                     tc_fence_after();
+                    if (p.stream_w) { mbar_wait(w_full(it & 1), (it >> 1) & 1); tc_fence_after(); }
                     const uint32_t a_hi = a_base + (uint32_t)s * a_stage, a_lo = a_hi + A_TILE;
-                    const uint32_t b_hi = base + (uint32_t)c * 2u * b_tile, b_lo = b_hi + b_tile;
+                    const uint32_t b_hi = base + (uint32_t)(p.stream_w ? (it & 1) : c) * 2u * b_tile, b_lo = b_hi + b_tile;
                     const int ksteps = min(KC, ctot - c * KC) >> 4;
                     for (int ks = 0; ks < ksteps; ++ks) {
                         const uint64_t dah = make_desc(a_hi + ks * 32), dal = make_desc(a_lo + ks * 32);
@@ -149,30 +153,45 @@
                         umma(tmem_acc, dah, dbl, idesc, 1);
                     }
                     umma_commit(empty_a(s));
+                    if (p.stream_w) umma_commit(w_empty(it & 1));
                 }
                 umma_commit(acc_full(buf));
+                if (p.stream_w) continue;
                 bool run_ends = (T + 1 == t_end);
                 if (!run_ends) {
                     int p2, k2, pb2, c2;
                     decode(T + 1, p2, k2, pb2, c2);
                     run_ends = (k2 != k) || (p2 != pass);
                 }
-                if (run_ends) umma_commit(w_empty);
+                if (run_ends) umma_commit(w_empty(0));
             }
         }
         __syncwarp();
     } else if (warp == 5) {
-        if (lane == 0) {
+        if (lane == 0 && p.stream_w) {
+            int it = 0;
+            for (int T = t_begin; T < t_end; ++T) {
+                int pass, k, pbase, cnt;
+                decode(T, pass, k, pbase, cnt);
+                const unsigned char* src = p.wpacked + PACK_HEADER + (size_t)k * p.nchunks * 2u * b_tile;
+                for (int c = 0; c < p.nchunks; ++c, ++it) {
+                    const int s = it & 1;
+                    if (it >= 2) mbar_wait(w_empty(s), ((it >> 1) - 1) & 1);
+                    mbar_expect_tx(w_full(s), 2u * b_tile);
+                    bulk_g2s(base + (uint32_t)s * 2u * b_tile, src + (size_t)c * 2u * b_tile, 2u * b_tile, w_full(s));
+                }
+            }
+        } else if (lane == 0) {
             int wrun = -1, cur_k = -1, cur_pass = -1;
             for (int T = t_begin; T < t_end; ++T) {
                 int pass, k, pbase, cnt;
                 decode(T, pass, k, pbase, cnt);
                 if (k == cur_k && pass == cur_pass) continue;
                 ++wrun; cur_k = k; cur_pass = pass;
-                if (wrun >= 1) mbar_wait(w_empty, (wrun - 1) & 1);
+                if (wrun >= 1) mbar_wait(w_empty(0), (wrun - 1) & 1);
                 const unsigned char* src = p.wpacked + PACK_HEADER + (size_t)k * w_bytes;
-                mbar_expect_tx(w_full, w_bytes);
-                for (int c = 0; c < p.nchunks; ++c) bulk_g2s(base + (uint32_t)c * 2u * b_tile, src + (size_t)c * 2u * b_tile, 2u * b_tile, w_full);
+                mbar_expect_tx(w_full(0), w_bytes);
+                for (int c = 0; c < p.nchunks; ++c) bulk_g2s(base + (uint32_t)c * 2u * b_tile, src + (size_t)c * 2u * b_tile, 2u * b_tile, w_full(0));
             }
         }
         __syncwarp();
@@ -222,12 +241,12 @@
 }
 
 __global__ void k_pair_count(const int* __restrict__ nbr, long long nbr_stride, const int* __restrict__ d_n, int n_cap, int skip_k,
-                             int* __restrict__ cnt) {
+                             const unsigned* __restrict__ row_mask, int* __restrict__ cnt) {
     const int k = blockIdx.y;
     if (k == skip_k) return;
     const int n = d_n ? min(*d_n, n_cap) : n_cap;
     const int o = blockIdx.x * blockDim.x + threadIdx.x;
-    const bool hit = o < n && nbr[(long long)k * nbr_stride + o] >= 0;
+    const bool hit = o < n && (!row_mask || ((row_mask[o] >> k) & 1u)) && nbr[(long long)k * nbr_stride + o] >= 0;
     const unsigned m = __ballot_sync(0xffffffffu, hit);
     if ((threadIdx.x & 31) == 0 && m) atomicAdd(cnt + k, __popc(m));
 }
@@ -241,12 +260,13 @@
 }
 
 __global__ void k_pair_fill(const int* __restrict__ nbr, long long nbr_stride, const int* __restrict__ d_n, int n_cap, int skip_k,
-                            const int* __restrict__ koff, int* __restrict__ cursor, int* __restrict__ pair_in, int* __restrict__ pair_out) {
+                            const unsigned* __restrict__ row_mask, const int* __restrict__ koff, int* __restrict__ cursor,
+                            int* __restrict__ pair_in, int* __restrict__ pair_out) {
     const int k = blockIdx.y;
     if (k == skip_k) return;
     const int n = d_n ? min(*d_n, n_cap) : n_cap;
     const int o = blockIdx.x * blockDim.x + threadIdx.x;
-    const int v = o < n ? nbr[(long long)k * nbr_stride + o] : -1;
+    const int v = (o < n && (!row_mask || ((row_mask[o] >> k) & 1u))) ? nbr[(long long)k * nbr_stride + o] : -1;
     const unsigned m = __ballot_sync(0xffffffffu, v >= 0);
     if (!m) return;
     const int lane = threadIdx.x & 31;
@@ -266,17 +286,22 @@
     if (t < (long long)n * c / 4) reinterpret_cast<float4*>(buf)[t] = make_float4(0.f, 0.f, 0.f, 0.f);
 }
 
-static size_t smem_bytes(int cin, int cout, int stages) {
-    const int nchunks = (cin + tc::KC - 1) / tc::KC;
-    return 1024 + (size_t)nchunks * 2 * cout * 128 + (size_t)stages * 2 * tc::A_TILE + SLAB_BYTES + (2 * MAX_STAGES + 6) * 8 + 64;
-}
+constexpr size_t SMEM_LIMIT = 227 * 1024 - 256;
+
+static size_t smem_bytes(int w_slots, int cout, int stages) {
+    return 1024 + (size_t)w_slots * 2 * cout * 128 + (size_t)stages * 2 * tc::A_TILE + SLAB_BYTES + NBAR * 8 + 64;
+}
+
+static int nchunks_of(int cin) { return (cin + tc::KC - 1) / tc::KC; }
+
+static bool stream_w(int cin, int cout) { return smem_bytes(nchunks_of(cin), cout, 2) > SMEM_LIMIT; }
 
 static bool shape_ok(int c1, int c2, int cout, int kvol) {
     const int ctot = c1 + c2;
     if (kvol < 1 || kvol > MAX_KVOL || ctot % 16 || ctot < 16) return false;
     if (c2 > 0 && (c1 % 8 || c2 % 8)) return false;
-    if (cout % 32 || cout < 32 || cout > 128) return false;
-    return smem_bytes(ctot, cout, 2) <= 227 * 1024 - 256;
+    if (cout % 32 || cout < 32 || cout > 256) return false;
+    return smem_bytes(stream_w(ctot, cout) ? 2 : nchunks_of(ctot), cout, 2) <= SMEM_LIMIT;
 }
 
 }
@@ -285,7 +310,7 @@
 
 extern "C" int lb2_pair_list(void* handle, void* stream, const int32_t* nbr, int64_t nbr_stride, const int32_t* d_nout,
                              int32_t nout_cap, int32_t kvol, int32_t skip_k, int32_t* pair_in, int32_t* pair_out,
-                             int32_t* koff, int32_t* tile_off, void* scratch) {
+                             int32_t* koff, int32_t* tile_off, void* scratch, const uint32_t* row_mask) {
     Lb2Handle* h = (Lb2Handle*)handle;
     LB2_REQUIRE(h, h && nbr && pair_in && pair_out && koff && tile_off && scratch && nout_cap > 0 && kvol >= 1 && kvol <= sc::MAX_KVOL, "pair_list");
     cudaStream_t s = (cudaStream_t)stream;
@@ -293,11 +318,11 @@
     int* cursor = cnt + 32;
     if (cudaMemsetAsync(cnt, 0, 64 * sizeof(int), s) != cudaSuccess) return lb2_fail(h, LB2_ERR_CUDA, "pair_list memset%s", "");
     dim3 grid(cdiv(nout_cap, 256), kvol);
-    sc::k_pair_count<<<grid, 256, 0, s>>>(nbr, nbr_stride, d_nout, nout_cap, skip_k, cnt);
+    sc::k_pair_count<<<grid, 256, 0, s>>>(nbr, nbr_stride, d_nout, nout_cap, skip_k, row_mask, cnt);
     LB2_POST_LAUNCH(h, "k_pair_count");
     sc::k_pair_scan<<<1, 32, 0, s>>>(cnt, kvol, koff, tile_off, cursor);
     LB2_POST_LAUNCH(h, "k_pair_scan");
-    sc::k_pair_fill<<<grid, 256, 0, s>>>(nbr, nbr_stride, d_nout, nout_cap, skip_k, koff, cursor, pair_in, pair_out);
+    sc::k_pair_fill<<<grid, 256, 0, s>>>(nbr, nbr_stride, d_nout, nout_cap, skip_k, row_mask, koff, cursor, pair_in, pair_out);
     LB2_POST_LAUNCH(h, "k_pair_fill");
     return LB2_OK;
 }
@@ -317,14 +342,18 @@
     p.pair_in = d->pair_in; p.pair_out = d->pair_out; p.koff = d->koff; p.tile_off = d->tile_off;
     for (int i = 0; i < 2; ++i) {
         const int j = d->npass > 1 ? i : 0;
-        LB2_REQUIRE(h, d->in1[j] && d->out[j] && ((d->c2 > 0) == (d->in2[j] != nullptr)), "spconv_scatter io");
+        const bool has_h = d->in1_h[j] && (d->c2 == 0 || d->in2_h[j]);
+        const bool has_f = d->in1[j] && (d->c2 == 0 || d->in2[j]);
+        LB2_REQUIRE(h, (has_h || has_f) && d->out[j] && (d->c2 > 0 || (!d->in2[j] && !d->in2_h[j])), "spconv_scatter io");
         p.in1[i] = d->in1[j]; p.in2[i] = d->in2[j]; p.out[i] = d->out[j];
         p.in1_h[i] = d->in1_h[j]; p.in2_h[i] = d->in2_h[j];
     }
+    p.stream_w = sc::stream_w(d->c1 + d->c2, d->cout) ? 1 : 0;
+    const int w_slots = p.stream_w ? 2 : p.nchunks;
     int stages = sc::MAX_STAGES;
-    while (stages > 2 && sc::smem_bytes(d->c1 + d->c2, d->cout, stages) > 227 * 1024 - 256) --stages;
+    while (stages > 2 && sc::smem_bytes(w_slots, d->cout, stages) > sc::SMEM_LIMIT) --stages;
     p.stages = stages;
-    const int half = d->cout <= 32 ? 32 : d->cout <= 64 ? 64 : 128;
+    const int half = d->cout <= 32 ? 32 : d->cout <= 64 ? 64 : d->cout <= 128 ? 128 : 256;
     p.acc_stride = half; p.tmem_cols = 2 * half;
     if (d->zero_rows_cap > 0) {
         for (int i = 0; i < d->npass; ++i) {
@@ -333,10 +362,10 @@
         }
     }
     {
-        cudaError_t e = lb2_configure_smem(h, LB2_K_SCATTER, sc::k_spconv_scatter, (int)(227 * 1024 - 256));
+        cudaError_t e = lb2_configure_smem(h, LB2_K_SCATTER, sc::k_spconv_scatter, (int)sc::SMEM_LIMIT);
         if (e != cudaSuccess) return lb2_fail(h, LB2_ERR_CUDA, "k_spconv_scatter smem attribute: %s", cudaGetErrorString(e));
     }
-    sc::k_spconv_scatter<<<h->num_sms, sc::THREADS, sc::smem_bytes(d->c1 + d->c2, d->cout, stages), s>>>(p);
+    sc::k_spconv_scatter<<<h->num_sms, sc::THREADS, sc::smem_bytes(w_slots, d->cout, stages), s>>>(p);
     LB2_POST_LAUNCH(h, "k_spconv_scatter");
     return LB2_OK;
 }
diff --git a/lidiff_b200/csrc/spconv_tc.cu b/lidiff_b200/csrc/spconv_tc.cu
--- a/lidiff_b200/csrc/spconv_tc.cu
+++ b/lidiff_b200/csrc/spconv_tc.cu
@@ -23,6 +23,7 @@
     const int* d_mout;
     int mout_cap;
     const int* row_perm;
+    const unsigned* row_mask;
     int stages, nchunks, tmem_cols, tot_col, group;
     int nbuf, acc_stride;
     int ncta;
@@ -73,6 +74,7 @@
         const int slot = m0 + threadIdx.x;
         const int row = (slot < M) ? (p.row_perm ? __ldg(p.row_perm + slot) : slot) : -1;
         row_s[threadIdx.x] = row;
+        const uint32_t rmask = (row >= 0 && p.row_mask) ? __ldg(p.row_mask + row) : 0xffffffffu;
         uint32_t mymask = 0;
         for (int k0 = 0; k0 < p.kvol; k0 += 9) {
             int v[9];
@@ -80,7 +82,7 @@
             for (int q = 0; q < 9; ++q) {
                 const int k = k0 + q;
                 v[q] = -1;
-                if (k < p.kvol && row >= 0) v[q] = p.nbr ? __ldg(p.nbr + (long long)k * p.nbr_stride + row) : row;
+                if (k < p.kvol && row >= 0 && ((rmask >> k) & 1u)) v[q] = p.nbr ? __ldg(p.nbr + (long long)k * p.nbr_stride + row) : row;
             }
 #pragma unroll
             for (int q = 0; q < 9; ++q) {
@@ -384,7 +386,7 @@
     p.c1 = d->c1; p.c2 = d->c2; p.cout = d->cout; p.kvol = d->kvol;
     p.wpacked = (const unsigned char*)d->weight_packed;
     p.scale = d->scale; p.shift = d->shift; p.relu = d->relu;
-    p.nbr = d->nbr; p.nbr_stride = d->nbr_stride; p.d_mout = d->d_mout; p.mout_cap = d->mout_cap; p.row_perm = d->row_perm;
+    p.nbr = d->nbr; p.nbr_stride = d->nbr_stride; p.d_mout = d->d_mout; p.mout_cap = d->mout_cap; p.row_perm = d->row_perm; p.row_mask = d->row_mask;
     p.nchunks = (d->c1 + d->c2 + tc::KC - 1) / tc::KC;
     const int nsplit = (d->cout == 256 && h->opt[LB2_OPT_TC_NSPLIT]) ? 2 : 1;
     p.ncta = d->cout / nsplit;
diff --git a/lidiff_b200/engine.py b/lidiff_b200/engine.py
--- a/lidiff_b200/engine.py
+++ b/lidiff_b200/engine.py
@@ -13,6 +13,7 @@
 
 GATE_NAMES = ("stage1", "stage2", "stage3", "stage4", "up1", "up2", "up3", "up4")
 GATE_LEVEL = (0, 1, 2, 3, 4, 3, 2, 1)
+SPLIT_TAU = {3: 0.5}
 BN_EPS = 1e-5
 
 
@@ -122,6 +123,16 @@
         self.pair_out = [torch.zeros(26 * n_cap, **i32) if w else None for w in want]
         self.koff = [torch.zeros(28, **i32) for _ in range(self.pair_levels)]
         self.tile_off = [torch.zeros(28, **i32) for _ in range(self.pair_levels)]
+        env = os.environ.get("LB2_SPLIT_TAU")
+        tau = dict(SPLIT_TAU) if env is None else {int(a): float(b) for a, b in (kv.split(":") for kv in env.split(",") if kv)}
+        ok = use_pairs and h.scatter_supported(256, 0, 256, 27)
+        self.split_min_rows = {l: math.ceil(t * 256) for l, t in tau.items() if ok and 0 < t and l < levels}
+        self.split_of = {}
+        self.split_bufs = {l: (torch.zeros(n_cap, **i32), torch.zeros(n_cap, **i32),
+                               (torch.zeros((n_cap + 127) // 128, **i32), torch.zeros((n_cap + 255) // 256, **i32)),
+                               torch.zeros(27 * n_cap, **i32), torch.zeros(27 * n_cap, **i32), torch.zeros(28, **i32), torch.zeros(28, **i32),
+                               torch.zeros(64, **i32))
+                           for l in self.split_min_rows}
 
     def build(self, coords_f: torch.Tensor, n_points: int, after_levels=None, late_stream=None, late_done=None):
         h, N = self.h, self.n_cap
@@ -155,6 +166,13 @@
 
         def map3(l, **kw):
             one(self.grid[l], l, 3, 1 << l, self.nbr3[l], self.perm3[l], l, **kw)
+            if l in self.split_min_rows:
+                dense, res, to, p_in, p_out, koff, toff, scratch = self.split_bufs[l]
+                mask, perm = self.mask_of[self.nbr3[l].data_ptr()], self.perm3[l]
+                h.tile_split(mask, perm, self.d_n[l], N, 27, self.split_min_rows[l], dense, res)
+                h.tile_order(dense, perm, self.d_n[l], N, to[0], to[1], kw.get("to_scratch", self.to_scratch))
+                h.pair_list(self.nbr3[l], N, self.d_n[l], N, 27, -1, p_in, p_out, koff, toff, scratch, row_mask=res)
+                self.split_of[self.nbr3[l].data_ptr()] = (dense, to, p_in, p_out, koff, toff)
             if l < self.pair_levels and self.use_pairs and l in self.pair_level_set:
                 h.pair_list(self.nbr3[l], N, self.d_n[l], N, 27, 13, self.pair_in[l], self.pair_out[l], self.koff[l], self.tile_off[l], self.pl_scratch)
                 self.pairs_of[self.nbr3[l].data_ptr()] = l
@@ -370,7 +388,23 @@
         pre = None
         geom_lvl = self._pairs_lookup.get(nbr.data_ptr()) if (nbr is not None and self.use_scatter and lay.Wpc is not None
                                                                and self.conv_algo != _lib.ALGO_FFMA) else None
-        if geom_lvl is not None:
+        split = None
+        if (geom_lvl is None and nbr is not None and lay.cout == 256 and lay.kvol == 27 and lay.Wp is not None
+                and self.conv_algo != _lib.ALGO_FFMA):
+            split = self.geom.split_of.get(nbr.data_ptr())
+        if split is not None:
+            dense, to_dense, p_in, p_out, koff, toff = split
+            pre = self.buf(f"split.{lay.cout}", (2, cap, lay.cout))
+            sd = ScatterDesc()
+            sd.c1, sd.c2, sd.cout, sd.kvol = d.c1, d.c2, lay.cout, 27
+            sd.weight_packed = lay.Wp.data_ptr()
+            sd.pair_in, sd.pair_out, sd.koff, sd.tile_off = p_in.data_ptr(), p_out.data_ptr(), koff.data_ptr(), toff.data_ptr()
+            sd.npass = npass
+            for p in range(npass):
+                sd.in1[p], sd.in2[p], sd.out[p] = _ptr(f(in1), p), _ptr(f(in2), p), pre[p].data_ptr()
+                sd.in1_h[p], sd.in2_h[p] = _ptr(hh(in1), p), _ptr(hh(in2), p)
+            sd.d_zero_rows, sd.zero_rows_cap = d_m.data_ptr(), cap
+        elif geom_lvl is not None:
             g, l = geom_lvl
             pre = self.buf(f"scatter.{lay.cout}", (2, cap, lay.cout))
             sd = ScatterDesc()
@@ -386,14 +420,15 @@
         else:
             sd = None
         map_ptr = nbr.data_ptr() if nbr is not None else None
-        d.cout, d.kvol = lay.cout, (1 if pre is not None else lay.kvol)
-        d.weight = (lay.Wc if pre is not None else lay.W).data_ptr()
-        wp = lay.Wpc if pre is not None else lay.Wp
+        centre = pre is not None and split is None
+        d.cout, d.kvol = lay.cout, (1 if centre else lay.kvol)
+        d.weight = (lay.Wc if centre else lay.W).data_ptr()
+        wp = lay.Wpc if centre else lay.Wp
         d.weight_packed = wp.data_ptr() if wp is not None else None
         d.scale = lay.scale.data_ptr() if lay.scale is not None else None
         d.shift = lay.shift.data_ptr() if lay.shift is not None else None
         d.relu = 1 if relu else 0
-        if pre is not None:
+        if centre:
             nbr = None
         d.nbr = nbr.data_ptr() if nbr is not None else None
         d.nbr_stride = nbr.stride(0) if nbr is not None else cap
@@ -402,8 +437,12 @@
         perm = self._perm_lookup.get(nbr.data_ptr()) if (nbr is not None and self.use_row_order) else None
         d.row_perm = perm.data_ptr() if perm is not None else None
         mask = self._mask_lookup.get(nbr.data_ptr()) if nbr is not None else None
+        if split is not None:
+            mask = split[0]
         d.row_mask = mask.data_ptr() if mask is not None else None
         to = self._tile_order_lookup.get(nbr.data_ptr()) if (nbr is not None and perm is not None) else None
+        if split is not None and to is not None:
+            to = split[1]
         d.tile_order128 = to[0].data_ptr() if to is not None else None
         d.tile_order256 = to[1].data_ptr() if to is not None else None
         res_h = hh(residual) if (residual is not None and residual.f is None) else None
```

After: 62.78 (median of 6 runs). 3.3% higher.
